# lisvulaczo/lodestar

Measured on AMD Instinct MI355X. Metric: BLS signature sets verified/sec (whole node) at 1/2/4/8 MI355X; p50 batch latency, higher is better.
Workload: dtype u32

## Files before the change

### include/lodestar_bls.h

```cpp
#ifndef LODESTAR_BLS_H
#define LODESTAR_BLS_H

#include <stddef.h>
#include <stdint.h>

#ifdef __cplusplus
extern "C" {
#endif

#define LSG_OK 0
#define LSG_ERR_INVALID_ARG 1
#define LSG_ERR_NO_DEVICE 2
#define LSG_ERR_DEVICE 3
#define LSG_ERR_NOMEM 4
#define LSG_ERR_CLOSED 5
#define LSG_ERR_BUSY 6
#define LSG_ERR_ENTROPY 7

#define LSG_BLST_SUCCESS 0
#define LSG_BLST_BAD_ENCODING 1
#define LSG_BLST_POINT_NOT_ON_CURVE 2
#define LSG_BLST_POINT_NOT_IN_GROUP 3
#define LSG_BLST_AGGR_TYPE_MISMATCH 4
#define LSG_BLST_VERIFY_FAIL 5
// ... 67 lines not shown
int lsg_submit_jobs(lsg_ctx* ctx, const lsg_job* jobs, size_t n_jobs, uint64_t seed, lsg_ticket* ticket);
int lsg_wait_jobs(lsg_ctx* ctx, lsg_ticket ticket, lsg_job_result* results , lsg_stats* stats);
int lsg_jobs_partial(lsg_ctx* ctx, lsg_ticket ticket, uint8_t* out576, int32_t* has_batch);
int lsg_jobs_partial_device(lsg_ctx* ctx, lsg_ticket ticket, void* dev_out576, int32_t* has_batch);
int lsg_wait_jobs_node(lsg_ctx* ctx, lsg_ticket ticket, int32_t node_valid, lsg_job_result* results,
                       lsg_stats* stats);
#define LSG_NO_GROUP 0xffffffffu
int lsg_submit_jobs_grouped(lsg_ctx* ctx, const lsg_job* jobs, size_t n_jobs, uint64_t seed,
                            const uint32_t* set_group, size_t n_groups, lsg_ticket* ticket);
int lsg_wait_jobs_grouped(lsg_ctx* ctx, lsg_ticket ticket, lsg_job_result* results, lsg_stats* stats,
                          uint8_t* agg96 , uint32_t* agg_n );
int lsg_set_coalesce(lsg_ctx* ctx, uint32_t max_sets, int32_t max_inflight);
int lsg_assign_jobs(const uint32_t* job_sets, size_t n_jobs, int32_t n_devices, int32_t* owner);
int lsg_pipeline_slots(lsg_ctx* ctx, int32_t* n);
int lsg_poll(lsg_ctx* ctx, lsg_ticket ticket, int32_t* done);
int lsg_verify_jobs(lsg_ctx* ctx, const lsg_job* jobs, size_t n_jobs, uint64_t seed, lsg_job_result* results,
                    lsg_stats* stats);

int lsg_verify_sets(lsg_ctx* ctx, const lsg_set* sets, size_t n_sets, uint64_t seed, lsg_job_result* result);

int lsg_aggregate_pubkeys(lsg_ctx* ctx, const uint8_t* pks, uint32_t pk_len, size_t n, uint8_t* out96,
                          int32_t* err_code);
int lsg_aggregate_pubkeys_multi(lsg_ctx* ctx, const lsg_set* sets, size_t n_sets, uint8_t* out96, int32_t* err);

int lsg_hash_to_g2(lsg_ctx* ctx, const uint8_t* msgs, uint32_t msg_len, size_t n, const uint8_t* dst,
                   uint32_t dst_len, uint8_t* out192);

int lsg_sig_decode(lsg_ctx* ctx, const uint8_t* sigs, uint32_t sig_len, size_t n, uint8_t* out192, int32_t* err);

int lsg_batch_partial(lsg_ctx* ctx, const lsg_set* sets, size_t n_sets, uint64_t seed, uint8_t* out576,
                      int32_t* set_err, int32_t* any_error);
int lsg_final_verify(lsg_ctx* ctx, const uint8_t* partials576, size_t n_partials, int32_t* valid);
int lsg_final_submit(lsg_ctx* ctx, const uint8_t* partials576, size_t n_partials, lsg_ticket* ticket);
int lsg_final_submit_device(lsg_ctx* ctx, const void* dev_partials576, size_t n_partials, lsg_ticket* ticket);
int lsg_final_wait(lsg_ctx* ctx, lsg_ticket ticket, int32_t* valid);
int lsg_final_submit_groups(lsg_ctx* ctx, const uint8_t* partials576, size_t n_groups, size_t per_group,
                            lsg_ticket* ticket);
int lsg_final_wait_groups(lsg_ctx* ctx, lsg_ticket ticket, int32_t* valid );

int lsg_pubkey_table_set(lsg_ctx* ctx, size_t first_index, const uint8_t* pks, uint32_t pk_len, size_t n,
                         int32_t* err);
int lsg_pubkey_table_size(lsg_ctx* ctx, size_t* n);

int lsg_committees_set(lsg_ctx* ctx, uint32_t first_id, const uint32_t* indices,
                       const uint32_t* offsets , size_t n_committees,
                       int32_t* err );
int lsg_committees_clear(lsg_ctx* ctx, uint32_t first_id, size_t n);
int lsg_committee_count(lsg_ctx* ctx, size_t* n);

typedef struct {
  uint64_t lookups, hits, pending, inserts, evictions, bypassed, full;
  uint32_t entries, capacity;
} lsg_msg_cache_stats;
int lsg_msg_cache_set(lsg_ctx* ctx, size_t capacity);
int lsg_msg_cache_clear(lsg_ctx* ctx);
int lsg_msg_cache_get_stats(lsg_ctx* ctx, lsg_msg_cache_stats* out);

int lsg_pubkey_validate(lsg_ctx* ctx, const uint8_t* pks, uint32_t pk_len, size_t n, uint8_t* out96, int32_t* err);

int lsg_aggregate_signatures(lsg_ctx* ctx, const uint8_t* sigs, uint32_t sig_len, const uint32_t* offsets,
                             size_t n_groups, uint8_t* out96, int32_t* err);

int lsg_signing_roots(lsg_ctx* ctx, const uint8_t* roots32, size_t n, const uint8_t* domain32, uint32_t domain_stride,
                      uint8_t* out32);
int lsg_attestation_signing_roots(lsg_ctx* ctx, const uint8_t* data128, size_t n, const uint8_t* domain32,
                                  uint32_t domain_stride, uint8_t* out32);
int lsg_deposit_signing_roots(lsg_ctx* ctx, const uint8_t* msgs88, size_t n, const uint8_t* domain32,
                              uint32_t domain_stride, uint8_t* out32);
int lsg_object_signing_roots(lsg_ctx* ctx, const uint8_t* objs, uint32_t obj_len, size_t n, const uint8_t* domain32,
                             uint32_t domain_stride, uint8_t* out32);

int lsg_verify_deposits(lsg_ctx* ctx, const uint8_t* data184, size_t n, const uint8_t* domain32, uint64_t seed,
                        uint8_t* valid, int32_t* err);

int lsg_sign(lsg_ctx* ctx, const uint8_t* sks32, const uint8_t* msgs, uint32_t msg_len, size_t n, uint8_t* out96);
int lsg_sk_to_pk(lsg_ctx* ctx, const uint8_t* sks32, size_t n, uint8_t* out96);

int lsg_check_fp2_mul(lsg_ctx* ctx, const uint32_t* in, size_t n, uint32_t* out);
int lsg_check_fp_sqr(lsg_ctx* ctx, const uint32_t* in, size_t n, uint32_t* out);
int lsg_check_fp2_sqr(lsg_ctx* ctx, const uint32_t* in, size_t n, uint32_t* out);
int lsg_check_sums(lsg_ctx* ctx, const uint32_t* in, size_t n, uint32_t* out);
int lsg_check_fp2_lanes(lsg_ctx* ctx, const uint32_t* in, size_t n, uint32_t* out);
int lsg_check_g2_lanes(lsg_ctx* ctx, const uint32_t* in, size_t n, uint32_t* out);
int lsg_check_canon(lsg_ctx* ctx, const uint32_t* in, size_t n, const uint8_t* bytes48, size_t nb, uint32_t* out,
                    uint32_t* out_limbs);
int lsg_check_fp2_roots(lsg_ctx* ctx, const uint32_t* in, size_t n, uint32_t* out);
int lsg_check_batch_inv(lsg_ctx* ctx, const uint32_t* in, size_t n, uint32_t* out);
int lsg_check_map_uniform(lsg_ctx* ctx, const uint8_t* ub256, size_t n, uint8_t* out192);
int lsg_check_batch_partial_rnd(lsg_ctx* ctx, const lsg_set* sets, size_t n_sets,
                                const uint64_t* rnd , uint8_t* out576,
                                int32_t* set_err, int32_t* any_error);

int lsg_probe_fp_mul_rate(lsg_ctx* ctx, double* fp_mul_per_s, double* mad_per_s);

int lsg_probe_mad_peak(lsg_ctx* ctx, double* mad_per_s);

int lsg_last_kernel_times(lsg_ctx* ctx, const char** names, double* ms, int max);

#ifdef __cplusplus
}
#endif
#endif
```

### lodestar_amd/_native.py

```python
import ctypes
import os
import struct
import threading

HERE = os.path.dirname(os.path.abspath(__file__))
LIB_PATH = os.environ.get("LSG_LIB", os.path.join(HERE, "liblodestar_bls.so"))
AB_LIB_PATH = os.path.join(HERE, "liblodestar_bls_ab.so")

LSG_OK = 0
LSG_ERR_INVALID_ARG = 1
LSG_ERR_NO_DEVICE = 2
LSG_ERR_BUSY = 6
LSG_ERR_ENTROPY = 7

LSG_INVALID = 0
LSG_VALID = 1
LSG_ERROR = 2

LSG_JOB_BATCHABLE = 1
LSG_JOB_PRIORITY = 2
LSG_JOB_VALIDATE_KEYS = 4

BLST_NAMES = {
    0: "BLST_SUCCESS", 1: "BLST_BAD_ENCODING", 2: "BLST_POINT_NOT_ON_CURVE", 3: "BLST_POINT_NOT_IN_GROUP",
# ... 66 lines not shown
        k = len(self.committees)
        return struct.pack("=I%dI" % k, k, *self.committees) + self.bits


def _key_form(pks):
    if isinstance(pks, PkBits):
        return LSG_PK_BITS, pks.n_bits, pks.tobytes()
    if isinstance(pks, PkBitsMulti):
        return LSG_PK_BITS_MULTI, pks.n_bits, pks.tobytes()
    if isinstance(pks, PkIndices):
        return LSG_PK_INDEX, len(pks), pks.tobytes()
    pk_len = len(pks[0]) if pks else 96
    if any(len(p) != pk_len for p in pks):
        raise ValueError("all pubkeys of one set must share one encoding length")
    if pk_len in (LSG_PK_BITS, LSG_PK_BITS_MULTI):
        pk_len = 0
    return pk_len, len(pks), b"".join(pks)


class MsgObject:

    def __init__(self, obj, domain):
        self.obj = bytes(obj)
        self.domain = bytes(domain)

    def __len__(self):
        return len(self.obj) + len(self.domain)

    def tobytes(self):
        return self.obj + self.domain


def _msg_form(msg):
    if isinstance(msg, MsgObject):
        b = msg.tobytes()
        return b, len(b) | LSG_MSG_OBJECT
    return msg, len(msg)


class LsgSet(ctypes.Structure):
    _fields_ = [
        ("pks", ctypes.c_void_p), ("pk_len", ctypes.c_uint32), ("n_pks", ctypes.c_uint32),
        ("msg", ctypes.c_void_p), ("msg_len", ctypes.c_uint32),
        ("sig", ctypes.c_void_p), ("sig_len", ctypes.c_uint32),
    ]


class LsgJob(ctypes.Structure):
    _fields_ = [("sets", ctypes.POINTER(LsgSet)), ("n_sets", ctypes.c_uint32), ("flags", ctypes.c_uint32)]


class LsgJobResult(ctypes.Structure):
    _fields_ = [("status", ctypes.c_int32), ("err_code", ctypes.c_int32)]


class LsgStats(ctypes.Structure):
    _fields_ = [
        ("batch_retries", ctypes.c_uint32), ("batch_sigs_success", ctypes.c_uint32),
        ("start_ns", ctypes.c_uint64), ("end_ns", ctypes.c_uint64),
        ("n_final_exps", ctypes.c_uint32), ("submit_us", ctypes.c_uint32),
        ("key_error", ctypes.c_int32), ("key_error_job", ctypes.c_uint32),
    ]


class LsgMsgCacheStats(ctypes.Structure):
    _fields_ = [(k, ctypes.c_uint64) for k in ("lookups", "hits", "pending", "inserts", "evictions", "bypassed",
                                                "full")] + [("entries", ctypes.c_uint32), ("capacity", ctypes.c_uint32)]


_lib = None
_lib_lock = threading.Lock()

EXPORTS = [
    "lsg_init", "lsg_init_devices", "lsg_destroy", "lsg_device_count", "lsg_last_error", "lsg_device_name",
    "lsg_reserve", "lsg_allocation_count", "lsg_verify_jobs", "lsg_verify_sets",
    "lsg_aggregate_pubkeys", "lsg_hash_to_g2", "lsg_sig_decode", "lsg_batch_partial", "lsg_final_verify",
    "lsg_probe_fp_mul_rate", "lsg_last_kernel_times", "lsg_sign", "lsg_sk_to_pk",
    "lsg_submit_jobs", "lsg_wait_jobs", "lsg_wait_jobs_node", "lsg_jobs_partial", "lsg_assign_jobs", "lsg_poll",
    "lsg_final_submit", "lsg_final_wait", "lsg_pipeline_slots", "lsg_probe_mad_peak",
    "lsg_pubkey_table_set", "lsg_pubkey_table_size", "lsg_pubkey_validate",
    "lsg_final_submit_groups", "lsg_final_wait_groups", "lsg_aggregate_signatures",
    "lsg_signing_roots", "lsg_attestation_signing_roots", "lsg_jobs_partial_device", "lsg_final_submit_device",
    "lsg_set_coalesce", "lsg_aggregate_pubkeys_multi", "lsg_check_fp2_mul",
    "lsg_check_fp_sqr", "lsg_check_fp2_sqr", "lsg_check_sums", "lsg_check_fp2_lanes", "lsg_check_g2_lanes",
    "lsg_check_canon", "lsg_check_fp2_roots", "lsg_check_batch_inv", "lsg_check_map_uniform",
    "lsg_check_batch_partial_rnd",
    "lsg_deposit_signing_roots", "lsg_verify_deposits",
    "lsg_committees_set", "lsg_committees_clear", "lsg_committee_count",
    "lsg_object_signing_roots",
    "lsg_submit_jobs_grouped", "lsg_wait_jobs_grouped",
    "lsg_msg_cache_set", "lsg_msg_cache_clear", "lsg_msg_cache_get_stats",
]


def load_library(path=LIB_PATH):
    global _lib
    with _lib_lock:
        if _lib is not None and path == LIB_PATH:
            return _lib
        if not os.path.exists(path):
            raise NativeUnavailable(f"{path} not built (run python -c 'import __graft_entry__; __graft_entry__.build()')")
        lib = ctypes.CDLL(path)
        vp, u32, u64, i32, sz = ctypes.c_void_p, ctypes.c_uint32, ctypes.c_uint64, ctypes.c_int32, ctypes.c_size_t
        pi32 = ctypes.POINTER(ctypes.c_int32)
        lib.lsg_init.argtypes = [ctypes.c_int, ctypes.POINTER(vp)]
        lib.lsg_init_devices.argtypes = [ctypes.POINTER(ctypes.c_int), ctypes.c_int, ctypes.POINTER(vp)]
        lib.lsg_device_count.argtypes = [vp, pi32]
        lib.lsg_reserve.argtypes = [vp, sz, sz, sz, i32]
        lib.lsg_allocation_count.argtypes = [vp, ctypes.POINTER(u64)]
        lib.lsg_wait_jobs_node.argtypes = [vp, u64, i32, ctypes.POINTER(LsgJobResult), ctypes.POINTER(LsgStats)]
        lib.lsg_jobs_partial.argtypes = [vp, u64, ctypes.c_char_p, pi32]
        lib.lsg_jobs_partial_device.argtypes = [vp, u64, vp, pi32]
        lib.lsg_final_submit_device.argtypes = [vp, vp, sz, ctypes.POINTER(u64)]
        lib.lsg_assign_jobs.argtypes = [ctypes.POINTER(u32), sz, i32, pi32]
        lib.lsg_destroy.argtypes = [vp]
        lib.lsg_last_error.argtypes = [vp]
        lib.lsg_last_error.restype = ctypes.c_char_p
        lib.lsg_device_name.argtypes = [vp, ctypes.c_char_p, sz]
        lib.lsg_verify_jobs.argtypes = [vp, ctypes.POINTER(LsgJob), sz, u64, ctypes.POINTER(LsgJobResult),
                                        ctypes.POINTER(LsgStats)]
        lib.lsg_verify_sets.argtypes = [vp, ctypes.POINTER(LsgSet), sz, u64, ctypes.POINTER(LsgJobResult)]
        lib.lsg_aggregate_pubkeys.argtypes = [vp, ctypes.c_char_p, u32, sz, ctypes.c_char_p, pi32]
        lib.lsg_aggregate_pubkeys_multi.argtypes = [vp, ctypes.POINTER(LsgSet), sz, ctypes.c_char_p, pi32]
        lib.lsg_hash_to_g2.argtypes = [vp, ctypes.c_char_p, u32, sz, ctypes.c_char_p, u32, ctypes.c_char_p]
        lib.lsg_sig_decode.argtypes = [vp, ctypes.c_char_p, u32, sz, ctypes.c_char_p, pi32]
        lib.lsg_batch_partial.argtypes = [vp, ctypes.POINTER(LsgSet), sz, u64, ctypes.c_char_p, pi32, pi32]
        lib.lsg_final_verify.argtypes = [vp, ctypes.c_char_p, sz, pi32]
        lib.lsg_probe_fp_mul_rate.argtypes = [vp, ctypes.POINTER(ctypes.c_double), ctypes.POINTER(ctypes.c_double)]
        lib.lsg_last_kernel_times.argtypes = [vp, ctypes.POINTER(ctypes.c_char_p), ctypes.POINTER(ctypes.c_double),
                                              ctypes.c_int]
        lib.lsg_sign.argtypes = [vp, ctypes.c_char_p, ctypes.c_char_p, u32, sz, ctypes.c_char_p]
        lib.lsg_sk_to_pk.argtypes = [vp, ctypes.c_char_p, sz, ctypes.c_char_p]
        pu64 = ctypes.POINTER(u64)
        lib.lsg_submit_jobs.argtypes = [vp, ctypes.POINTER(LsgJob), sz, u64, pu64]
        lib.lsg_wait_jobs.argtypes = [vp, u64, ctypes.POINTER(LsgJobResult), ctypes.POINTER(LsgStats)]
        lib.lsg_submit_jobs_grouped.argtypes = [vp, ctypes.POINTER(LsgJob), sz, u64, ctypes.POINTER(u32), sz, pu64]
        lib.lsg_wait_jobs_grouped.argtypes = [vp, u64, ctypes.POINTER(LsgJobResult), ctypes.POINTER(LsgStats),
                                              ctypes.c_char_p, ctypes.POINTER(u32)]
        lib.lsg_poll.argtypes = [vp, u64, pi32]
        lib.lsg_pubkey_table_set.argtypes = [vp, sz, ctypes.c_char_p, u32, sz, pi32]
        lib.lsg_pubkey_table_size.argtypes = [vp, ctypes.POINTER(sz)]
        lib.lsg_committees_set.argtypes = [vp, u32, ctypes.POINTER(u32), ctypes.POINTER(u32), sz, pi32]
        lib.lsg_committees_clear.argtypes = [vp, u32, sz]
        lib.lsg_committee_count.argtypes = [vp, ctypes.POINTER(sz)]
        lib.lsg_msg_cache_set.argtypes = [vp, sz]
        lib.lsg_msg_cache_clear.argtypes = [vp]
        lib.lsg_msg_cache_get_stats.argtypes = [vp, ctypes.POINTER(LsgMsgCacheStats)]
        lib.lsg_final_submit_groups.argtypes = [vp, ctypes.c_char_p, sz, sz, pu64]
        lib.lsg_final_wait_groups.argtypes = [vp, u64, pi32]
        lib.lsg_pubkey_validate.argtypes = [vp, ctypes.c_char_p, u32, sz, ctypes.c_char_p, pi32]
        lib.lsg_signing_roots.argtypes = [vp, ctypes.c_char_p, sz, ctypes.c_char_p, u32, ctypes.c_char_p]
        lib.lsg_attestation_signing_roots.argtypes = [vp, ctypes.c_char_p, sz, ctypes.c_char_p, u32, ctypes.c_char_p]
        lib.lsg_deposit_signing_roots.argtypes = [vp, ctypes.c_char_p, sz, ctypes.c_char_p, u32, ctypes.c_char_p]
        lib.lsg_object_signing_roots.argtypes = [vp, ctypes.c_char_p, u32, sz, ctypes.c_char_p, u32, ctypes.c_char_p]
        lib.lsg_verify_deposits.argtypes = [vp, ctypes.c_char_p, sz, ctypes.c_char_p, u64, ctypes.c_char_p, pi32]
        lib.lsg_aggregate_signatures.argtypes = [vp, ctypes.c_char_p, u32, ctypes.POINTER(u32), sz,
                                                 ctypes.c_char_p, pi32]
        lib.lsg_final_submit.argtypes = [vp, ctypes.c_char_p, sz, pu64]
        lib.lsg_final_wait.argtypes = [vp, u64, pi32]
        lib.lsg_pipeline_slots.argtypes = [vp, pi32]
        lib.lsg_set_coalesce.argtypes = [vp, u32, i32]
        lib.lsg_check_fp2_mul.argtypes = [vp, ctypes.c_char_p, sz, ctypes.c_char_p]
        lib.lsg_check_fp_sqr.argtypes = [vp, ctypes.c_char_p, sz, ctypes.c_char_p]
        lib.lsg_check_fp2_sqr.argtypes = [vp, ctypes.c_char_p, sz, ctypes.c_char_p]
        lib.lsg_check_sums.argtypes = [vp, ctypes.c_char_p, sz, ctypes.c_char_p]
        lib.lsg_check_fp2_lanes.argtypes = [vp, ctypes.c_char_p, sz, ctypes.c_char_p]
        lib.lsg_check_g2_lanes.argtypes = [vp, ctypes.c_char_p, sz, ctypes.c_char_p]
        lib.lsg_check_canon.argtypes = [vp, ctypes.c_char_p, sz, ctypes.c_char_p, sz, ctypes.c_char_p, ctypes.c_char_p]
        lib.lsg_check_fp2_roots.argtypes = [vp, ctypes.c_char_p, sz, ctypes.c_char_p]
        lib.lsg_check_batch_inv.argtypes = [vp, ctypes.c_char_p, sz, ctypes.c_char_p]
        lib.lsg_check_map_uniform.argtypes = [vp, ctypes.c_char_p, sz, ctypes.c_char_p]
        lib.lsg_check_batch_partial_rnd.argtypes = [vp, ctypes.POINTER(LsgSet), sz, ctypes.POINTER(u64),
                                                    ctypes.c_char_p, pi32, pi32]
        lib.lsg_probe_mad_peak.argtypes = [vp, ctypes.POINTER(ctypes.c_double)]
        for name in EXPORTS:
            if name != "lsg_last_error":
                getattr(lib, name).restype = ctypes.c_int
        if path == LIB_PATH:
            _lib = lib
        return lib


class SetBuffer:

    def __init__(self, sets):
        self._keep = []
        sets = list(sets)
        self.arr = (LsgSet * max(len(sets), 1))()
        for i, (pks, msg, sig) in enumerate(sets):
            pk_len, n_pks, pkb = _key_form(pks)
            msg, msg_len = _msg_form(msg)
            for b in (pkb, msg, sig):
                self._keep.append(b)
            s = self.arr[i]
            s.pks = ctypes.cast(ctypes.c_char_p(pkb), ctypes.c_void_p) if pkb else None
            s.pk_len = pk_len
            s.n_pks = n_pks
            s.msg = ctypes.cast(ctypes.c_char_p(msg), ctypes.c_void_p) if msg else None
            s.msg_len = msg_len
            s.sig = ctypes.cast(ctypes.c_char_p(sig), ctypes.c_void_p) if sig else None
            s.sig_len = len(sig)
        self.n = len(sets)


def assign_jobs(job_sizes, n_devices):
    lib = load_library()
    n = len(job_sizes)
    sizes = (ctypes.c_uint32 * max(n, 1))(*job_sizes)
    owner = (ctypes.c_int32 * max(n, 1))()
    rc = lib.lsg_assign_jobs(sizes, n, int(n_devices), owner)
    if rc != LSG_OK:
        raise ValueError(f"lsg_assign_jobs failed ({rc})")
    return list(owner[:n])


class PreparedJobs:

    def __init__(self, jobs):
        import numpy as np
        flat = [st for sets, _ in jobs for st in sets]
        n = len(flat)
        pk_parts, pk_len, n_pks = [], np.zeros(max(n, 1), np.uint32), np.zeros(max(n, 1), np.uint32)
        for i, (pks, _m, _s) in enumerate(flat):
            pk_len[i], n_pks[i], b = _key_form(pks)
            pk_parts.append(b)

        def pack(parts):
            lens = np.array([len(p) for p in parts] or [0], np.uint64)
            offs = np.zeros_like(lens)
            if len(parts) > 1:
                offs[1:] = np.cumsum(lens)[:-1]
            buf = np.frombuffer(b"".join(parts) + b"\0", dtype=np.uint8).copy()
            return buf, offs, lens

        self._pk, pk_off, _ = pack(pk_parts)
        forms = [_msg_form(m) for _, m, _ in flat]
        self._msg, msg_off, msg_len = pack([b for b, _ in forms])
        msg_word = np.array([w for _, w in forms] or [0], np.uint32)
        self._sig, sig_off, sig_len = pack([s for _, _, s in flat])
        self.sets = (LsgSet * max(n, 1))()
        dt = np.dtype({"names": ["pks", "pk_len", "n_pks", "msg", "msg_len", "sig", "sig_len"],
                       "formats": [np.uint64, np.uint32, np.uint32, np.uint64, np.uint32, np.uint64, np.uint32],
                       "offsets": [LsgSet.pks.offset, LsgSet.pk_len.offset, LsgSet.n_pks.offset, LsgSet.msg.offset,
                                   LsgSet.msg_len.offset, LsgSet.sig.offset, LsgSet.sig_len.offset],
                       "itemsize": ctypes.sizeof(LsgSet)})
        v = np.frombuffer(self.sets, dtype=dt)
        if n:
            has_keys = (n_pks[:n] > 0) | (pk_len[:n] == LSG_PK_BITS_MULTI)
            v["pks"][:n] = np.where(has_keys, self._pk.ctypes.data + pk_off[:n], 0)
            v["pk_len"][:n] = pk_len[:n]
# ... 384 lines not shown

    def final_submit_groups(self, groups):
        ng = len(groups)
        pg = len(groups[0]) if groups else 0
        if any(len(g) != pg for g in groups):
            raise ValueError("every group needs the same number of partials")
        t = ctypes.c_uint64()
        rc = self.lib.lsg_final_submit_groups(self.h, b"".join(b"".join(g) for g in groups), ng, pg, ctypes.byref(t))
        if rc == LSG_ERR_BUSY:
            return None
        self._check(rc, "lsg_final_submit_groups")
        t_ng = ng
        return (t.value, t_ng)

    def final_wait_groups(self, ticket):
        t, ng = ticket
        v = (ctypes.c_int32 * max(ng, 1))()
        self._check(self.lib.lsg_final_wait_groups(self.h, t, v), "lsg_final_wait_groups")
        return [bool(x) for x in v[:ng]]

    def sign(self, sks, msgs):
        if not sks:
            return []
        ml = len(msgs[0])
        out = ctypes.create_string_buffer(96 * len(sks))
        skb = b"".join(int(k).to_bytes(32, "big") for k in sks)
        self._check(self.lib.lsg_sign(self.h, skb, b"".join(msgs), ml, len(sks), out), "lsg_sign")
        raw = out.raw
        return [raw[96 * i:96 * i + 96] for i in range(len(sks))]

    def sk_to_pk(self, sks):
        if not sks:
            return []
        out = ctypes.create_string_buffer(96 * len(sks))
        skb = b"".join(int(k).to_bytes(32, "big") for k in sks)
        self._check(self.lib.lsg_sk_to_pk(self.h, skb, len(sks), out), "lsg_sk_to_pk")
        raw = out.raw
        return [raw[96 * i:96 * i + 96] for i in range(len(sks))]

    def check_fp2_mul(self, words):
        n = len(words) // 56
        assert len(words) == 56 * n
        out = ctypes.create_string_buffer(4 * 28 * n)
        src = struct.pack(f"<{len(words)}I", *words)
        self._check(self.lib.lsg_check_fp2_mul(self.h, src, n, out), "lsg_check_fp2_mul")
        return list(struct.unpack(f"<{28 * n}I", out.raw))

    def _check_sqr(self, fn, words, per_item):
        n = len(words) // per_item
        assert len(words) == per_item * n
        out = ctypes.create_string_buffer(4 * per_item * n)
        src = struct.pack(f"<{len(words)}I", *words)
        self._check(getattr(self.lib, fn)(self.h, src, n, out), fn)
        return list(struct.unpack(f"<{per_item * n}I", out.raw))

    def check_fp_sqr(self, words):
        return self._check_sqr("lsg_check_fp_sqr", words, 14)

    def check_fp2_sqr(self, words):
        return self._check_sqr("lsg_check_fp2_sqr", words, 28)

    def check_sums(self, words):
        n = len(words) // (12 * 14)
        assert len(words) == 12 * 14 * n
        out = ctypes.create_string_buffer(4 * 42 * 14 * n)
        src = struct.pack(f"<{len(words)}I", *words)
        self._check(self.lib.lsg_check_sums(self.h, src, n, out), "lsg_check_sums")
        return list(struct.unpack(f"<{42 * 14 * n}I", out.raw))

    def _check_lanes(self, fn, words):
        n = len(words) // (12 * 14)
        assert len(words) == 12 * 14 * n
        out = ctypes.create_string_buffer(4 * 24 * 14 * n)
        src = struct.pack(f"<{len(words)}I", *words)
        self._check(getattr(self.lib, fn)(self.h, src, n, out), fn)
        return list(struct.unpack(f"<{24 * 14 * n}I", out.raw))

    def check_fp2_lanes(self, words):
        return self._check_lanes("lsg_check_fp2_lanes", words)

    def check_g2_lanes(self, words):
        return self._check_lanes("lsg_check_g2_lanes", words)

    def check_canon(self, words, strings=()):
        n, nb = len(words) // 14, len(strings)
        assert len(words) == 14 * n and all(len(b) == 48 for b in strings)
        out = ctypes.create_string_buffer(4 * 54 * max(n, 1))
        limbs = ctypes.create_string_buffer(4 * 14 * max(nb, 1))
        src = struct.pack(f"<{len(words)}I", *words)
        self._check(self.lib.lsg_check_canon(self.h, src, n, b"".join(strings), nb, out, limbs), "lsg_check_canon")
        return (list(struct.unpack(f"<{54 * n}I", out.raw[:4 * 54 * n])),
                list(struct.unpack(f"<{14 * nb}I", limbs.raw[:4 * 14 * nb])))

    def check_fp2_roots(self, words):
        n = len(words) // 28
        assert len(words) == 28 * n
        out = ctypes.create_string_buffer(4 * 58 * n)
        src = struct.pack(f"<{len(words)}I", *words)
        self._check(self.lib.lsg_check_fp2_roots(self.h, src, n, out), "lsg_check_fp2_roots")
        return list(struct.unpack(f"<{58 * n}I", out.raw))

    def check_batch_inv(self, words):
        return self._check_sqr("lsg_check_batch_inv", words, 14)

    def check_map_uniform(self, items):
        n = len(items)
        assert all(len(b) == 256 for b in items)
        if not n:
            return []
        out = ctypes.create_string_buffer(192 * n)
        self._check(self.lib.lsg_check_map_uniform(self.h, b"".join(items), n, out), "lsg_check_map_uniform")
        raw = out.raw
        return [raw[192 * i:192 * i + 192] for i in range(n)]

    def batch_partial_rnd(self, sets, rnd):
        b = SetBuffer(sets)
        assert len(rnd) == b.n
        r = (ctypes.c_uint64 * max(b.n, 1))(*[int(x) for x in rnd])
        out = ctypes.create_string_buffer(576)
        errs = (ctypes.c_int32 * max(b.n, 1))()
        anyerr = ctypes.c_int32()
        self._check(self.lib.lsg_check_batch_partial_rnd(self.h, b.arr, b.n, r, out, errs, ctypes.byref(anyerr)),
                    "lsg_check_batch_partial_rnd")
        return out.raw, [errs[i] for i in range(b.n)], bool(anyerr.value)

    def probe_fp_mul_rate(self):
        a, b = ctypes.c_double(), ctypes.c_double()
        self._check(self.lib.lsg_probe_fp_mul_rate(self.h, ctypes.byref(a), ctypes.byref(b)), "lsg_probe_fp_mul_rate")
        return a.value, b.value

    def last_kernel_times(self, max_entries=1024):
        names = (ctypes.c_char_p * max_entries)()
        ms = (ctypes.c_double * max_entries)()
        n = self.lib.lsg_last_kernel_times(self.h, names, ms, max_entries)
        return [(names[i].decode(), ms[i]) for i in range(n)]
```

### lodestar_amd/csrc/lsg_curve.hpp

```cpp
#pragma once
#include "lsg_tower.hpp"

LSG_INL fp_t fadd(const fp_t& a, const fp_t& b) { return fp_add(a, b); }
LSG_INL fp2_t fadd(const fp2_t& a, const fp2_t& b) { return fp2_add(a, b); }
LSG_INL fp_t fsub(const fp_t& a, const fp_t& b) { return fp_sub(a, b); }
LSG_INL fp2_t fsub(const fp2_t& a, const fp2_t& b) { return fp2_sub(a, b); }
LSG_INL fp_t fmul(const fp_t& a, const fp_t& b) { return fp_mul(a, b); }
LSG_INL fp2_t fmul(const fp2_t& a, const fp2_t& b) { return fp2_mul(a, b); }
LSG_INL fp_t fsqr(const fp_t& a) { return fp_sqr(a); }
LSG_INL fp2_t fsqr(const fp2_t& a) { return fp2_sqr(a); }
LSG_INL fp_t fneg(const fp_t& a) { return fp_neg(a); }
LSG_INL fp2_t fneg(const fp2_t& a) { return fp2_neg(a); }
LSG_INL fps_t<1, 0> fsum(const fp_t& a) { return fps(a); }
LSG_INL fp2s_t<1, 0> fsum(const fp2_t& a) { return fp2s(a); }
template <int K, int P, int N>
LSG_INL fps_t<K * P, K * N> fsum_mulk(const fps_t<P, N>& a) { return fps_mulk<K>(a); }
template <int K, int P0, int N0, int P1, int N1>
LSG_INL fp2s_t<K * P0, K * N0, K * P1, K * N1> fsum_mulk(const fp2s_t<P0, N0, P1, N1>& a) { return fp2s_mulk<K>(a); }
template <int K> LSG_INL fp_t fmulk(const fp_t& a) { return fp_mulk<K>(a); }
template <int K> LSG_INL fp2_t fmulk(const fp2_t& a) { return fp2_mulk<K>(a); }
template <class F> LSG_INL F fsub2(const F& a, const F& b, const F& c) { return (fsum(a) - b - c).carry(); }
LSG_INL fp_t fmul_b3(const fp_t& a) { return fp_mul12(a); }
LSG_INL fp2_t fmul_b3(const fp2_t& a) { return fp2_mul_b3(a); }
LSG_INL bool fis_zero(const fp_t& a) { return fp_is_zero(a); }
LSG_INL bool fis_zero(const fp2_t& a) { return fp2_is_zero(a); }
LSG_INL bool feq(const fp_t& a, const fp_t& b) { return fp_eq(a, b); }
LSG_INL bool feq(const fp2_t& a, const fp2_t& b) { return fp2_eq(a, b); }
LSG_INL fp_t fselect(bool c, const fp_t& a, const fp_t& b) { return fp_select(c, a, b); }
LSG_INL fp2_t fselect(bool c, const fp2_t& a, const fp2_t& b) { return fp2_select(c, a, b); }
LSG_INL fp_t finv(const fp_t& a) { return fp_inv(a); }
LSG_INL fp2_t finv(const fp2_t& a) { return fp2_inv(a); }
template <class F> LSG_INL F fzero();
template <> LSG_INL fp_t fzero<fp_t>() { return fp_zero(); }
template <> LSG_INL fp2_t fzero<fp2_t>() { return fp2_zero(); }
template <class F> LSG_INL F fone();
template <> LSG_INL fp_t fone<fp_t>() { return FP_ONE; }
template <> LSG_INL fp2_t fone<fp2_t>() { return fp2_one(); }
#ifdef LSG_PAIR_MODE
#include "lsg_fp2_lanes.hpp"
#endif
#ifdef LSG_FP2_LANES
template <> LSG_INL fp2v_t fzero<fp2v_t>() { return fp2v_from_const(fpc_t{}, fpc_t{}); }
template <> LSG_INL fp2v_t fone<fp2v_t>() { return fp2v_from_const(FP_ONE, fpc_t{}); }
#endif

template <class F>
struct aff_t {
  F x, y;
};
template <class F>
struct proj_t {
  F X, Y, Z;
};
typedef aff_t<fp_t> g1a_t;
typedef aff_t<fp2_t> g2a_t;
typedef proj_t<fp_t> g1p_t;
typedef proj_t<fp2_t> g2p_t;

template <class F>
LSG_INL proj_t<F> proj_inf() {
  proj_t<F> r;
  r.X = fzero<F>();
  r.Y = fone<F>();
  r.Z = fzero<F>();
  return r;
}

template <class F>
LSG_INL proj_t<F> proj_from_aff(const aff_t<F>& a) {
  proj_t<F> r;
  r.X = a.x;
  r.Y = a.y;
  r.Z = fone<F>();
  return r;
}

template <class F>
LSG_INL bool proj_is_inf(const proj_t<F>& a) {
  return fis_zero(a.Z);
}

template <class F>
LSG_INL proj_t<F> proj_neg(const proj_t<F>& a) {
  proj_t<F> r = a;
  r.Y = fneg(a.Y);
  return r;
}

template <class F>
LSG_INL proj_t<F> proj_add(const proj_t<F>& p, const proj_t<F>& q) {
  F t0 = fmul(p.X, q.X);
  F t1 = fmul(p.Y, q.Y);
  F t2 = fmul(p.Z, q.Z);
  F t3 = fsub2(fmul(fadd(p.X, p.Y), fadd(q.X, q.Y)), t0, t1);
  F t4 = fsub2(fmul(fadd(p.Y, p.Z), fadd(q.Y, q.Z)), t1, t2);
  F Y3 = fsub2(fmul(fadd(p.X, p.Z), fadd(q.X, q.Z)), t0, t2);
  F X3;
  t0 = fmulk<3>(t0);
  t2 = fmul_b3(t2);
  F Z3 = fadd(t1, t2);
  t1 = fsub(t1, t2);
  Y3 = fmul_b3(Y3);
  X3 = fmul(t4, Y3);
  t2 = fmul(t3, t1);
  X3 = fsub(t2, X3);
  Y3 = fmul(Y3, t0);
// ... 535 lines not shown
```

### lodestar_amd/csrc/lsg_fp2_lanes.hpp

```cpp
#pragma once

constexpr int LSG_VL = 14;

#if LSG_PAIR_G == 2
#define LSG_LANES_HIDE(x) asm volatile("" : "+v"(x))
#else
#define LSG_LANES_HIDE(x) ((void)0)
#endif

LSG_PFN void lanes_carry64(int64_t* t) {
#pragma unroll
  for (int j = 0; j < LSG_VL - 1; j++) {
    t[j + 1] += t[j] >> 29;
    t[j] &= (int64_t)LSG_M29;
  }
}
LSG_PFN void lanes_reduce_step(int64_t* t, const uint32_t* p, int i) {
  uint32_t m = ((uint32_t)t[0] * LSG_N0P) & LSG_M29;
  LSG_LANES_HIDE(m);
#pragma unroll
  for (int j = 0; j < LSG_VL; j++) t[j] += (int64_t)(int32_t)m * (int32_t)p[j];
  const int64_t c = t[0] >> 29;
#pragma unroll
  for (int j = 0; j < LSG_VL - 1; j++) t[j] = t[j + 1];
  t[0] += c;
  t[LSG_VL - 1] = 0;
  if (i == 6) lanes_carry64(t);
}
LSG_PFN void lanes_tail(int64_t* t, uint32_t* r) {
  lanes_carry64(t);
#pragma unroll
  for (int j = 0; j < LSG_VL; j++) r[j] = (uint32_t)t[j];
}
template <class OTHER>
LSG_PFN void lanes_sop_pass(uint32_t* r, const uint32_t* P, const uint32_t* Q, const uint32_t* b, const OTHER& other) {
  uint32_t p[LSG_VL];
#pragma unroll
  for (int j = 0; j < LSG_VL; j++) p[j] = LSG_P[j];
  int64_t t[LSG_VL];
#pragma unroll
  for (int j = 0; j < LSG_VL; j++) t[j] = 0;
#pragma unroll
  for (int i = 0; i < LSG_VL; i++) {
    uint32_t bo = b[i], bs = other(i, b[i]);
    LSG_LANES_HIDE(bo);
    LSG_LANES_HIDE(bs);
#pragma unroll
    for (int j = 0; j < LSG_VL; j++) t[j] += (int64_t)(int32_t)P[j] * (int32_t)bo;
#pragma unroll
    for (int j = 0; j < LSG_VL; j++) t[j] += (int64_t)(int32_t)Q[j] * (int32_t)bs;
    lanes_reduce_step(t, p, i);
  }
  lanes_tail(t, r);
}
LSG_PFN void lanes_mul_pass(uint32_t* r, const uint32_t* V, const uint32_t* s) {
  uint32_t p[LSG_VL];
#pragma unroll
  for (int j = 0; j < LSG_VL; j++) p[j] = LSG_P[j];
  int64_t t[LSG_VL];
#pragma unroll
  for (int j = 0; j < LSG_VL; j++) t[j] = 0;
#pragma unroll
  for (int i = 0; i < LSG_VL; i++) {
    uint32_t si = s[i];
    LSG_LANES_HIDE(si);
#pragma unroll
    for (int j = 0; j < LSG_VL; j++) t[j] += (int64_t)(int32_t)V[j] * (int32_t)si;
    lanes_reduce_step(t, p, i);
  }
  lanes_tail(t, r);
}
LSG_PFN void lanes_mul_operand(uint32_t& P, uint32_t& Q, uint32_t own, uint32_t partner, bool odd) {
  P = odd ? partner : own;
  Q = odd ? own : 0u - partner;
}
LSG_PFN void lanes_sqr_operand(uint32_t& V, uint32_t& s, uint32_t own, uint32_t partner, bool odd) {
  V = odd ? own : own + partner;
  s = odd ? partner + partner : own - partner;
}

#if LSG_PAIR_G == 2 && !defined(LSG_NO_FP2_LANES)
#define LSG_FP2_LANES 1
struct fp2v_t {
  uint32_t l[LSG_VL];
};
LSG_PFN bool lanes_odd() { return pair_h() != 0u; }
LSG_PFN uint32_t lanes_swap(uint32_t x) {
  return (uint32_t)__builtin_amdgcn_update_dpp(0, (int)x, 0xB1, 0xf, 0xf, true);
}

typedef uint32_t lanes8_t __attribute__((ext_vector_type(8)));
typedef uint32_t lanes4_t __attribute__((ext_vector_type(4)));
typedef uint32_t lanes2_t __attribute__((ext_vector_type(2)));
#define LSG_LANES_PARAMS(x) lanes8_t x##_a, lanes4_t x##_b, lanes2_t x##_c
#define LSG_LANES_ARGS(v) lanes_pack8(v), lanes_pack4(v), lanes_pack2(v)
#define LSG_LANES_UNPACK(x) lanes_unpack(x##_a, x##_b, x##_c)
LSG_PFN lanes8_t lanes_pack8(const fp2v_t& a) {
  return lanes8_t{a.l[0], a.l[1], a.l[2], a.l[3], a.l[4], a.l[5], a.l[6], a.l[7]};
}
LSG_PFN lanes4_t lanes_pack4(const fp2v_t& a) { return lanes4_t{a.l[8], a.l[9], a.l[10], a.l[11]}; }
LSG_PFN lanes2_t lanes_pack2(const fp2v_t& a) { return lanes2_t{a.l[12], a.l[13]}; }
LSG_PFN fp2v_t lanes_unpack(const lanes8_t& a, const lanes4_t& b, const lanes2_t& c) {
  fp2v_t r;
#pragma unroll
  for (int k = 0; k < 8; k++) r.l[k] = a[k];
#pragma unroll
  for (int k = 0; k < 4; k++) r.l[8 + k] = b[k];
  r.l[12] = c[0];
  r.l[13] = c[1];
  return r;
}

LSG_PLEAF fp2v_t lanes_fp2_mul_v(LSG_LANES_PARAMS(va), LSG_LANES_PARAMS(vb)) {
  const fp2v_t a = LSG_LANES_UNPACK(va), b = LSG_LANES_UNPACK(vb);
  const bool odd = lanes_odd();
  uint32_t P[LSG_VL], Q[LSG_VL];
#pragma unroll
  for (int k = 0; k < LSG_VL; k++) {
    lanes_mul_operand(P[k], Q[k], a.l[k], lanes_swap(a.l[k]), odd);
    LSG_LANES_HIDE(P[k]);
    LSG_LANES_HIDE(Q[k]);
  }
  fp2v_t r;
  lanes_sop_pass(r.l, P, Q, b.l, [](int, uint32_t x) { return lanes_swap(x); });
  return r;
}
LSG_PLEAF fp2v_t lanes_fp2_sqr_v(LSG_LANES_PARAMS(va)) {
  const fp2v_t a = LSG_LANES_UNPACK(va);
  const bool odd = lanes_odd();
  uint32_t V[LSG_VL], s[LSG_VL];
#pragma unroll
  for (int k = 0; k < LSG_VL; k++) {
    lanes_sqr_operand(V[k], s[k], a.l[k], lanes_swap(a.l[k]), odd);
    LSG_LANES_HIDE(V[k]);
    LSG_LANES_HIDE(s[k]);
  }
  fp2v_t r;
  lanes_mul_pass(r.l, V, s);
  return r;
}

LSG_PFN fp2v_t fp2v_from_pair(const fp2_t& a) {
  const bool odd = lanes_odd();
  fp2v_t r;
#pragma unroll
  for (int k = 0; k < LSG_PL; k++) {
    const uint32_t s = lanes_swap(odd ? a.c0.l[k] : a.c1.l[k]);
    r.l[k] = odd ? s : a.c0.l[k];
    r.l[LSG_PL + k] = odd ? a.c1.l[k] : s;
  }
  return r;
}
LSG_PFN fp2_t fp2v_to_pair(const fp2v_t& a) {
  const bool odd = lanes_odd();
  fp2_t r;
#pragma unroll
  for (int k = 0; k < LSG_PL; k++) {
    const uint32_t s = lanes_swap(odd ? a.l[k] : a.l[LSG_PL + k]);
    r.c0.l[k] = odd ? s : a.l[k];
    r.c1.l[k] = odd ? a.l[LSG_PL + k] : s;
  }
  return r;
}
LSG_PFN fp2v_t fp2v_from_const(const fpc_t& c0, const fpc_t& c1) {
  const bool odd = lanes_odd();
  fp2v_t r;
#pragma unroll
  for (int k = 0; k < LSG_VL; k++) r.l[k] = odd ? c1.l[k] : c0.l[k];
  return r;
}

LSG_PFN fp2v_t lanes_carry(const fp2v_t& a) {
  fp2v_t o;
  o.l[0] = a.l[0] & LSG_M29;
#pragma unroll
  for (int k = 1; k < LSG_VL - 1; k++) o.l[k] = (a.l[k] & LSG_M29) + (uint32_t)((int32_t)a.l[k - 1] >> 29);
  o.l[LSG_VL - 1] = a.l[LSG_VL - 1] + (uint32_t)((int32_t)a.l[LSG_VL - 2] >> 29);
  return o;
}
template <int P, int N>
struct fp2vs_t {
  uint32_t l[LSG_VL];
  LSG_PFN fp2v_t carry() const {
    static_assert(fps_carry_ok(P, N), "lazy sum too long for one carry round: carry a group first (P <= 3, N <= 3)");
    fp2v_t a;
#pragma unroll
    for (int k = 0; k < LSG_VL; k++) a.l[k] = l[k];
    return lanes_carry(a);
  }
  template <int K>
  LSG_PFN fp2v_t carry_mul() const {
    static_assert(fps_carry_mul_ok(K, P, N), "small multiple of this sum does not come out carried: carry() first");
    constexpr int m = fps_mulk_m(K), s = fps_mulk_s(K), sh = 29 - s;
    constexpr uint32_t lowm = (1u << sh) - 1;
    uint32_t t[LSG_VL];
#pragma unroll
    for (int k = 0; k < LSG_VL; k++) t[k] = m == 3 ? l[k] + (l[k] << 1) : l[k];
    fp2v_t o;
    o.l[0] = (t[0] & lowm) << s;
#pragma unroll
    for (int k = 1; k < LSG_VL - 1; k++) o.l[k] = ((t[k] & lowm) << s) + (uint32_t)((int32_t)t[k - 1] >> sh);
    o.l[LSG_VL - 1] = (t[LSG_VL - 1] << s) + (uint32_t)((int32_t)t[LSG_VL - 2] >> sh);
    return o;
  }
};
LSG_PFN fp2vs_t<1, 0> fsum(const fp2v_t& a) {
  fp2vs_t<1, 0> r;
#pragma unroll
  for (int k = 0; k < LSG_VL; k++) r.l[k] = a.l[k];
  return r;
}
template <int P, int N, int Q, int M>
LSG_PFN fp2vs_t<P + Q, N + M> operator+(const fp2vs_t<P, N>& a, const fp2vs_t<Q, M>& b) {
  fp2vs_t<P + Q, N + M> r;
#pragma unroll
  for (int k = 0; k < LSG_VL; k++) r.l[k] = a.l[k] + b.l[k];
  return r;
}
template <int P, int N, int Q, int M>
LSG_PFN fp2vs_t<P + M, N + Q> operator-(const fp2vs_t<P, N>& a, const fp2vs_t<Q, M>& b) {
  fp2vs_t<P + M, N + Q> r;
#pragma unroll
  for (int k = 0; k < LSG_VL; k++) r.l[k] = a.l[k] - b.l[k];
  return r;
}
template <int P, int N>
LSG_PFN fp2vs_t<N, P> operator-(const fp2vs_t<P, N>& a) {
  fp2vs_t<N, P> r;
#pragma unroll
  for (int k = 0; k < LSG_VL; k++) r.l[k] = 0u - a.l[k];
  return r;
}
template <int P, int N>
LSG_PFN fp2vs_t<P + 1, N> operator+(const fp2vs_t<P, N>& a, const fp2v_t& b) { return a + fsum(b); }
template <int P, int N>
LSG_PFN fp2vs_t<P, N + 1> operator-(const fp2vs_t<P, N>& a, const fp2v_t& b) { return a - fsum(b); }
template <int K, int P, int N>
LSG_PFN fp2vs_t<K * P, K * N> fsum_mulk(const fp2vs_t<P, N>& a) {
  static_assert(K >= 1 && K <= 3, "uncarried small multiples up to 3");
  fp2vs_t<K * P, K * N> r;
#pragma unroll
  for (int k = 0; k < LSG_VL; k++) r.l[k] = a.l[k] * (uint32_t)K;
  return r;
}

LSG_PFN fp2v_t fmul(const fp2v_t& a, const fp2v_t& b) { return lanes_fp2_mul_v(LSG_LANES_ARGS(a), LSG_LANES_ARGS(b)); }
LSG_PFN fp2v_t fsqr(const fp2v_t& a) { return lanes_fp2_sqr_v(LSG_LANES_ARGS(a)); }
LSG_PFN fp2v_t fadd(const fp2v_t& a, const fp2v_t& b) { return (fsum(a) + b).carry(); }
LSG_PFN fp2v_t fsub(const fp2v_t& a, const fp2v_t& b) { return (fsum(a) - b).carry(); }
LSG_PFN fp2v_t fneg(const fp2v_t& a) { return (-fsum(a)).carry(); }
template <int K>
LSG_PFN fp2v_t fmulk(const fp2v_t& a) { return fsum(a).template carry_mul<K>(); }
LSG_PFN fp2v_t fmul_b3(const fp2v_t& a) {
  const bool odd = lanes_odd();
  fp2vs_t<2, 1> x;
#pragma unroll
  for (int k = 0; k < LSG_VL; k++) {
    const uint32_t o = lanes_swap(a.l[k]);
    x.l[k] = odd ? a.l[k] + o : a.l[k] - o;
  }
  return fmulk<12>(x.carry());
}
LSG_PFN fp2v_t fselect(bool c, const fp2v_t& a, const fp2v_t& b) {
  fp2v_t r;
#pragma unroll
  for (int k = 0; k < LSG_VL; k++) r.l[k] = c ? a.l[k] : b.l[k];
  return r;
}
LSG_PFN bool fis_zero(const fp2v_t& a) { return fp2_is_zero(fp2v_to_pair(a)); }
#endif
```

### lodestar_amd/csrc/lsg_host.hip

```cpp
#include <hip/hip_runtime.h>
#include <rccl/rccl.h>
#include <stdio.h>
#include <stdlib.h>
#include <errno.h>
#include <string.h>
#include <sys/random.h>
#include <time.h>

#include <algorithm>
#include <atomic>
#include <condition_variable>
#include <chrono>
#include <mutex>
#include <shared_mutex>
#include <thread>
#include <unordered_map>
#include <string>
#include <vector>

#include "../../include/lodestar_bls.h"
#include "lsg_launch.h"
#include "lsg_layout.h"
#include "lsg_serial.h"
#include "lsg_ab.h"
// ... 403 lines not shown
    s->own_streams = false;
  } else {
    for (int k = 0; k < 2; k++) LSG_HIP(s, hipStreamCreateWithFlags(&s->st_norm[k], hipStreamNonBlocking));
    s->st[0] = s->st_norm[0];
    s->st[1] = s->st_norm[1];
  }
  hipEvent_t* evs[] = {&s->ev_in, &s->ev_sig, &s->ev_grp, &s->ev_part, &s->ev_done, &s->ev_node, &s->ev_xp};
  for (hipEvent_t* e : evs) LSG_HIP(s, hipEventCreateWithFlags(e, hipEventDisableTiming));
  if (blocking_waits()) {
    for (hipEvent_t* e : {&s->ev_part, &s->ev_done}) {
      LSG_HIP(s, hipEventDestroy(*e));
      LSG_HIP(s, hipEventCreateWithFlags(e, hipEventDisableTiming | hipEventBlockingSync));
    }
  }
  LSG_RC(ensure(s, s->d_dst, 256));
  LSG_HIP(s, hipMemcpy(s->d_dst.p, DST_POP, DST_POP_LEN, hipMemcpyHostToDevice));
  return LSG_OK;
}

void slot_destroy(Slot* s) {
  if (!s->d) return;
  for (int k = 0; k < 2; k++)
    if (s->st[k]) (void)hipStreamSynchronize(s->st[k]);
  DevBuf* bufs[] = {&s->d_sig,  &s->d_siglen, &s->d_msg,  &s->d_msgoff, &s->d_msglen, &s->d_pk,    &s->d_pklen,
                    &s->d_rnd,  &s->d_mode,   &s->d_dst,  &s->d_ub,     &s->d_sigaff, &s->d_siginf, &s->d_seterr,
                    &s->d_pkp,  &s->d_pkerr,  &s->d_agg,  &s->d_P,      &s->d_pinf,   &s->d_H,     &s->d_hinf,
                    &s->d_rs,   &s->d_rs2,    &s->d_fall, &s->d_fall2,  &s->d_Pp,     &s->d_zP,    &s->d_zPi,
                    &s->d_U,    &s->d_nrm,    &s->d_nrmi, &s->d_Hp,     &s->d_zN,     &s->d_zNi,   &s->binv_lv[0],
                    &s->binv_lv[1], &s->binv_iv[0], &s->binv_iv[1], &s->d_lines, &s->d_S, &s->d_F, &s->d_verdict,
                    &s->d_Sb,   &s->d_fgb,    &s->d_Fb,   &s->d_bkt,    &s->d_bits,   &s->d_aux,   &s->d_gath,
                    &s->d_nodeF, &s->d_nodeV, &s->d_plan, &s->d_mid, &s->d_Hm, &s->d_hinfm,
                    &s->d_mmask, &s->d_PmP, &s->d_Pm, &s->d_pinfm, &s->d_errm, &s->d_xport,
                    &s->d_agga, &s->d_aggi, &s->d_aggpre, &s->d_aggtot, &s->d_aggflag, &s->d_cbits,
                    &s->d_gplan, &s->d_gsum, &s->d_gagg, &s->d_gtmp[0], &s->d_gtmp[1], &s->d_Hx, &s->d_hinfx};
  for (DevBuf* b : bufs) free_dev(*b);
  for (auto& u : s->seg_tmp)
    for (DevBuf& b : u) free_dev(b);
  HostBuf* hb[] = {&s->h_arena, &s->h_err, &s->h_pinf, &s->h_pkerr, &s->h_verdict, &s->h_blob, &s->h_plan, &s->h_nodeV,
                   &s->h_xport, &s->h_cbits, &s->h_gplan, &s->h_gagg};
  for (HostBuf* b : hb) free_host(*b);
  for (Timer& t : s->timers) {
    (void)hipEventDestroy(t.a);
    (void)hipEventDestroy(t.b);
  }
  s->timers.clear();
  hipEvent_t evs[] = {s->ev_in, s->ev_sig, s->ev_grp, s->ev_part, s->ev_done, s->ev_node, s->ev_xp};
  for (hipEvent_t e : evs)
    if (e) (void)hipEventDestroy(e);
  if (s->own_streams) {
    for (int k = 0; k < 2; k++) {
      if (s->st_prio[k]) (void)hipStreamSynchronize(s->st_prio[k]);
      if (s->st_norm[k]) (void)hipStreamSynchronize(s->st_norm[k]);
    }
    for (int k = 0; k < 2; k++) {
      if (s->st_norm[k]) (void)hipStreamDestroy(s->st_norm[k]);
      s->st_norm[k] = s->st_prio[k] = s->st[k] = nullptr;
    }
  }
  s->d = nullptr;
}

int slot_streams(Slot* s, bool prio) {
  if (!s->own_streams) return LSG_OK;
  if (prio && !s->st_prio[0]) {
    Dev* d = s->d;
    for (int k = 0; k < 2; k++) LSG_RC(prio_stream(d->c, d, &d->s_pp[k]));
    s->st_prio[0] = d->s_pp[0];
    s->st_prio[1] = d->s_pp[1];
  }
  hipStream_t* p = prio ? s->st_prio : s->st_norm;
  s->st[0] = p[0];
  s->st[1] = p[1];
  return LSG_OK;
}

int slot_ready(Dev* d, Slot* s, int index) {
  if (s->d) return LSG_OK;
  const int rc = slot_create(d, s, index, nullptr);
  if (rc) slot_destroy(s);
  return rc;
}

bool miller_fused() { return lsg_ab_long("LSG_MILLER_FUSED", 1) != 0; }

size_t slp_items_max();
int miller_k_for(size_t n_sets) {
  if (miller_fused()) return n_sets <= slp_items_max() ? 1 : 4;
  const long v = lsg_ab_long("LSG_MILLER_K", 0);
  if (v == 1 || v == 2 || v == 4) return (int)v;
  return n_sets >= 8192 ? 4 : (n_sets >= 1024 ? 2 : 1);
}

bool agg_tree_on() { return lsg_ab_long("LSG_AGG_TREE", 0) != 0; }

Switches read_switches() {
  Switches w;
  w.package_group = lsg_ab_long("LSG_PACKAGE_GROUP", 1) != 0;
  w.sub_groups = lsg_ab_long("LSG_SUB_GROUPS", 1) != 0;
  w.nb_merge = lsg_ab_long("LSG_NB_MERGE", 1) != 0;
  w.msg_agg = lsg_ab_long("LSG_MSG_AGG", 1) != 0;
  w.msm_min_group = (size_t)std::max(1L, lsg_ab_long("LSG_MSM_MIN_GROUP", 256));
  w.b0_min = (size_t)std::max(0L, lsg_ab_long("LSG_B0_MIN", 64));
  w.b0_run = (size_t)std::max(2L, lsg_ab_long("LSG_B0_RUN", 4));
  w.seg_fold_wide = (int)lsg_ab_long("LSG_SEG_FOLD_WIDE", SEG_FOLD_WIDE);
  w.slp_items = slp_items_max();
  return w;
}
SegPlan slot_seg(Slot* s, int op, const std::vector<int32_t>& seg_off, const std::vector<int32_t>& seg_len, bool has_idx,
                 size_t idx_off, int32_t dst_base) {
  return plan_seg(s->plan, op, seg_off, seg_len, has_idx, idx_off, dst_base,
                  (int)lsg_ab_long("LSG_SEG_FOLD_WIDE", SEG_FOLD_WIDE));
}

void binv_sizes(size_t n, size_t* lv, size_t* iv);
size_t binv_lv_words(size_t n) {
  size_t a, b;
  binv_sizes(n, &a, &b);
  return a;
}
size_t binv_iv_words(size_t n) {
  size_t a, b;
  binv_sizes(n, &a, &b);
  return b;
}

int size_inputs(Slot* s, size_t n, size_t np, size_t mb) {
  const size_t nn = std::max(n, (size_t)1), pp = std::max(np, (size_t)1);
  auto al = [](size_t x) { return (x + 7) & ~(size_t)7; };
  const size_t arena = al(192 * nn) + al(4 * nn) * 4 + al(4 * pp) + al(8 * nn) + al(96 * pp) + al(std::max(mb, (size_t)1)) + nn;
  LSG_RC(ensure_host(s, s->h_arena, arena));
  LSG_RC(ensure(s, s->d_sig, 192 * nn));
  LSG_RC(ensure(s, s->d_siglen, 4 * nn));
  LSG_RC(ensure(s, s->d_msg, std::max(mb, (size_t)1)));
  LSG_RC(ensure(s, s->d_msgoff, 4 * nn));
  LSG_RC(ensure(s, s->d_msglen, 4 * nn));
  LSG_RC(ensure(s, s->d_pk, 96 * pp));
  LSG_RC(ensure(s, s->d_pklen, 4 * pp));
  LSG_RC(ensure(s, s->d_rnd, 8 * nn));
  LSG_RC(ensure(s, s->d_mode, nn));
  LSG_RC(ensure(s, s->d_mid, 4 * nn));
  return LSG_OK;
}

int size_state(Slot* s, size_t n, size_t np, size_t ng, size_t n_msm, int pkg = 0) {
  const size_t nn = std::max(n, (size_t)1), pp = std::max(np, (size_t)1), gg = std::max(ng, (size_t)1);
  const size_t g_msm = std::max(n_msm, (size_t)1);
  struct {
    DevBuf* b;
    size_t bytes;
  } dev[] = {{&s->d_ub, 256 * nn},
             {&s->d_sigaff, 4 * W_G2A * nn},
             {&s->d_siginf, nn},
             {&s->d_seterr, 4 * nn},
             {&s->d_pkp, 4 * W_G1P * pp},
             {&s->d_pkerr, 4 * pp},
             {&s->d_agg, 4 * W_G1P * nn},
             {&s->d_P, 4 * W_G1A * nn},
             {&s->d_pinf, nn},
             {&s->d_H, 4 * W_G2A * nn},
             {&s->d_hinf, nn},
             {&s->d_rs, 4 * W_G2P * nn},
             {&s->d_Pp, 4 * W_G1P * nn},
             {&s->d_zP, 4 * W_FP * nn},
             {&s->d_zPi, 4 * W_FP * nn},
             {&s->d_U, 4 * W_H2CU * nn},
             {&s->d_nrm, 4 * W_FP * 2 * nn},
// ... 475 lines not shown
  if (s->msg_dedup) s->msg_id.assign(mid, mid + n);
  if (scale && n) {
    if (rnd_in) {
      memcpy(rnd, rnd_in, 8 * n);
    } else if (seed == 0) {
      if (!os_random(rnd, 8 * n)) {
        set_err(s->d->c, "no entropy for the RLC randomizers (getrandom failed)");
        return LSG_ERR_ENTROPY;
      }
      for (size_t i = 0; i < n; i++)
        while (rnd[i] == 0)
          if (!os_random(&rnd[i], 8)) {
            set_err(s->d->c, "no entropy for the RLC randomizers (getrandom failed)");
            return LSG_ERR_ENTROPY;
          }
    } else {
      uint64_t sd = seed;
      for (size_t i = 0; i < n; i++) {
        uint64_t r;
        do r = splitmix64(sd);
        while (r == 0);
        rnd[i] = r;
      }
    }
  } else if (n) {
    memset(rnd, 0, 8 * n);
  }
  if (scale && noscale)
    for (size_t i = 0; i < n; i++)
      if ((*noscale)[i]) rnd[i] = 0;
  memcpy(s->rnd.data(), rnd, 8 * n);
  hipStream_t S = s->st[0];
  struct {
    DevBuf* d;
    size_t off, len;
  } cp[] = {{&s->d_sig, o_sig, 192 * nn},      {&s->d_siglen, o_siglen, 4 * nn}, {&s->d_msg, o_msg, std::max(mc ? mo : msg_total, (size_t)1)},
            {&s->d_msgoff, o_msgoff, 4 * nn}, {&s->d_msglen, o_msglen, 4 * nn}, {&s->d_pk, o_pk, ks * np},
            {&s->d_pklen, o_pklen, 4 * np},   {&s->d_rnd, o_rnd, 8 * nn}};
  for (auto& x : cp) LSG_HIP(s, hipMemcpyAsync(x.d->p, A + x.off, x.len, hipMemcpyHostToDevice, S));
  if (s->msg_dedup) LSG_HIP(s, hipMemcpyAsync(s->d_mid.p, A + o_mid, 4 * n, hipMemcpyHostToDevice, S));
  if (bw) LSG_HIP(s, hipMemcpyAsync(s->d_cbits.p, cbits, 4 * bw, hipMemcpyHostToDevice, S));
  return LSG_OK;
}

int run_pk_bits(Slot* s, uint32_t* dst) {
  if (s->bits_sets.empty()) return LSG_OK;
  Dev* d = s->d;
  KL(s, "k_pk_agg_bits", lsgk::pk_agg_bits(S_(s), (int)s->bplan.n_pairs, PL(s, s->bplan.pair_off), PL(s, s->bplan.plan_off),
                                           P_<uint32_t>(s->d_cbits), P_<uint32_t>(d->d_cm_idx), P_<uint32_t>(d->d_cm_off),
                                           P_<uint32_t>(d->d_cm_sum), P_<uint32_t>(d->d_pktab), P_<uint8_t>(d->d_pktab_ok),
                                           (uint32_t)d->pktab_n, dst));
  return LSG_OK;
}
int run_pk_multi(Slot* s, uint32_t* dst) {
  if (s->multi_sets.empty()) return LSG_OK;
  Dev* d = s->d;
  KL(s, "k_pk_agg_bits_multi",
     lsgk::pk_agg_bits_multi(S_(s), (int)s->mplan.n_pairs, PL(s, s->mplan.pair_off), PL(s, s->mplan.set_off),
                             PL(s, s->mplan.part_off), P_<uint32_t>(s->d_cbits), P_<uint32_t>(d->d_cm_idx),
                             P_<uint32_t>(d->d_cm_off), P_<uint32_t>(d->d_cm_sum), P_<uint32_t>(d->d_pktab),
                             P_<uint8_t>(d->d_pktab_ok), (uint32_t)d->pktab_n, dst));
  return LSG_OK;
}

int launch_accum(Slot* s, size_t n_items, size_t item_off, uint32_t* fall, bool single = false) {
  const int ni = (int)n_items;
  const int32_t* items = PL(s, item_off);
  if (ni > 0 && (single || s->K == 1) && miller_fused() && (size_t)ni <= std::max(slp_items_max(), (size_t)8192) &&
      slp_items_max() > 0) {
    KL(s, "k_slp_items1", lsg_slp_miller_items1(S_(s), ni, items, P_<uint32_t>(s->d_P), P_<uint8_t>(s->d_pinf),
                                                P_<uint8_t>(s->d_hinf), P_<int32_t>(s->d_seterr), P_<uint32_t>(s->d_H),
                                                fall));
    return LSG_OK;
  }
  if (single && ni > 0) {
    LSG_RC(ensure(s, s->d_lines, 4 * (size_t)ML_STEPS * W_LINE * n_items));
    KL(s, "k_miller_lines_list", lsgk::miller_lines_list(S_(s), ni, items, P_<uint32_t>(s->d_H), P_<uint32_t>(s->d_lines)));
    KL(s, "k_miller_accum_list",
       lsgk::miller_accum_list(S_(s), ni, items, P_<uint32_t>(s->d_P), P_<uint8_t>(s->d_pinf), P_<uint8_t>(s->d_hinf),
                               P_<int32_t>(s->d_seterr), P_<uint32_t>(s->d_lines), fall));
    return LSG_OK;
  }
  if (miller_fused()) {
    KL(s, "k_miller_fused", lsgk::miller_fused(S_(s), ni, items, items + ni, P_<uint32_t>(s->d_P), P_<uint8_t>(s->d_pinf),
                                              P_<uint8_t>(s->d_hinf), P_<int32_t>(s->d_seterr), P_<uint32_t>(s->d_H),
                                              fall));
    return LSG_OK;
  }
  KL(s, "k_miller_accum",
     lsgk::miller_accum(S_(s), s->K, ni, items, items + ni, P_<uint32_t>(s->d_P), P_<uint8_t>(s->d_pinf),
                        P_<uint8_t>(s->d_hinf), P_<int32_t>(s->d_seterr), (int)s->n_sets, P_<uint32_t>(s->d_lines),
                        fall));
  return LSG_OK;
}

#define SERIAL_LABEL(name) (lsg_serial_mode() == LSG_SERIAL_SLP ? "slp_" #name : "k_row_" #name)

int launch_phase(Slot* s, const PhasePlan& Ph, const uint32_t* rs, uint32_t* fall, bool export_blobs,
                 const uint32_t* rs_msm = nullptr) {
  if (!rs_msm) rs_msm = rs;
  const size_t ng = Ph.groups.size();
  if (ng == 0) return LSG_OK;
  LSG_RC(size_state(s, s->n_sets, s->n_pks, ng, Ph.n_msm, 2));
  s->cur = 1;
  if (Ph.n_msm) {
    LSG_RC(run_seg(s, 1, "msm_buckets", Ph.buckets, rs_msm, P_<uint32_t>(s->d_bkt)));
    LSG_RC(run_seg(s, 1, "msm_bits", Ph.bits, P_<uint32_t>(s->d_bkt), P_<uint32_t>(s->d_bits)));
    KL(s, "k_g2p_to_canon", lsgk::g2p_to_canon(S_(s), (int)(MSM_BITS * Ph.n_msm), P_<uint32_t>(s->d_bits),
                                               P_<uint8_t>(s->d_Sb)));
    KL(s, SERIAL_LABEL(horner_miller),
       lsg_row_horner_miller(S_(s), (int)Ph.n_msm, P_<uint8_t>(s->d_Sb), P_<uint8_t>(s->d_fgb)));
  }
  if (Ph.n_msm < ng) {
    const int nsm = (int)(ng - Ph.n_msm);
    LSG_RC(run_seg(s, 1, "sig_sums", Ph.sums, rs, P_<uint32_t>(s->d_S)));
    uint8_t* sb = P_<uint8_t>(s->d_Sb) + (size_t)288 * MSM_BITS * Ph.n_msm;
    KL(s, "k_g2p_to_canon", lsgk::g2p_to_canon(S_(s), nsm, P_<uint32_t>(s->d_S) + W_G2P * Ph.n_msm, sb));
    KL(s, SERIAL_LABEL(miller_neg_g1),
       lsg_row_miller_neg_g1(S_(s), nsm, sb, P_<uint8_t>(s->d_fgb) + 576 * Ph.n_msm));
  }
  KL(s, "k_blobs_to_fp12", lsgk::blobs_to_fp12(S_(s), (int)ng, P_<uint8_t>(s->d_fgb), fall + W_F12 * Ph.term_base));
  LSG_HIP(s, hipEventRecord(s->ev_grp, s->st[1]));
  s->cur = 0;
  LSG_HIP(s, hipStreamWaitEvent(s->st[0], s->ev_grp, 0));
  LSG_RC(run_seg(s, 2, "fp12_product", Ph.prod, fall, P_<uint32_t>(s->d_F)));
  KL(s, "k_fp12_to_canon", lsgk::fp12_to_canon(S_(s), (int)ng, P_<uint32_t>(s->d_F), P_<uint8_t>(s->d_Fb)));
  if (export_blobs) LSG_HIP(s, hipMemcpyAsync(s->h_blob.p, s->d_Fb.p, 576 * ng, hipMemcpyDeviceToHost, s->st[0]));
  LSG_HIP(s, hipEventRecord(s->ev_part, s->st[0]));
  return LSG_OK;
}

int launch_fe_range(Slot* s, size_t g0, size_t g1) {
  if (g1 <= g0) return LSG_OK;
  s->cur = 0;
  const size_t ng = g1 - g0;
  KL(s, SERIAL_LABEL(final_exp),
     lsg_row_final_exp(S_(s), (int)ng, P_<uint8_t>(s->d_Fb) + 576 * g0, P_<int32_t>(s->d_verdict) + g0));
  LSG_HIP(s, hipMemcpyAsync(H_<int32_t>(s->h_verdict) + g0, P_<int32_t>(s->d_verdict) + g0, 4 * ng,
                            hipMemcpyDeviceToHost, s->st[0]));
  return LSG_OK;
}
int launch_fe(Slot* s, size_t ng) { return launch_fe_range(s, 0, ng); }

int launch_agg_tree(Slot* s, const AggPlan& P, uint32_t* agg);

int launch_set_stages(Slot* s, const SegPlan* pkagg, const PhasePlan& Ph, uint32_t* fall) {
  const size_t n_items = Ph.agg_g >= 0 ? Ph.n_set_items : Ph.n_items, item_off = Ph.item_off;
  const int n = (int)s->n_sets, np = (int)s->n_pks;
  if (n == 0) return LSG_OK;
  Dev* d = s->d;
  LSG_HIP(s, hipEventRecord(s->ev_in, s->st[0]));
  s->cur = 1;
  LSG_HIP(s, hipStreamWaitEvent(s->st[1], s->ev_in, 0));
  if (!s->single_keys && s->agg.tree) {
    LSG_RC(launch_agg_tree(s, s->agg, P_<uint32_t>(s->d_agg)));
  } else if (s->single_keys) {
    if (np > 0)
      KL(s, "k_pk_decode", lsgk::pk_decode(S_(s), np, P_<uint8_t>(s->d_pk), s->pk_stride, P_<uint32_t>(s->d_pklen),
                                           P_<uint32_t>(s->d_agg), P_<int32_t>(s->d_pkerr), P_<uint32_t>(d->d_pktab),
                                           P_<uint8_t>(d->d_pktab_ok), (uint32_t)d->pktab_n));
  } else if (!s->pk_all_bits) {
    LSG_RC(run_pk_seg(s, *pkagg, P_<uint32_t>(s->d_agg)));
  }
  LSG_RC(run_pk_bits(s, P_<uint32_t>(s->d_agg)));
  LSG_RC(run_pk_multi(s, P_<uint32_t>(s->d_agg)));
  if (s->n_kv)
    KL(s, "k_pk_keyvalidate", lsgk::pk_keyvalidate(S_(s), (int)s->n_kv, PL(s, s->kv_off), P_<uint8_t>(s->d_pk),
                                                   P_<uint32_t>(s->d_pklen), P_<int32_t>(s->d_pkp)));
  KL(s, "k_pk_scale", lsgk::pk_scale(S_(s), n, P_<uint32_t>(s->d_agg), P_<uint64_t>(s->d_rnd), P_<uint32_t>(s->d_Pp),
// ... 2462 lines not shown
int lsg_sign(lsg_ctx* c, const uint8_t* sks32, const uint8_t* msgs, uint32_t msg_len, size_t n, uint8_t* out96) {
  if (!c || !out96 || (n && (!sks32 || !msgs)) || msg_marked(msg_len)) return LSG_ERR_INVALID_ARG;
  LSG_ENTER(c);
  Slot* s = &c->dev[0]->util;
  timer_reset(s);
  if (n == 0) return LSG_OK;
  LSG_RC(util_hash(s, msgs, msg_len, n, DST_POP, DST_POP_LEN));
  LSG_RC(ensure(s, s->d_aux, 96 * n));
  LSG_RC(ensure(s, s->d_Fb, 32 * n));
  LSG_HIP(s, hipMemcpyAsync(s->d_Fb.p, sks32, 32 * n, hipMemcpyHostToDevice, s->st[0]));
  KL(s, "k_sign", lsgk::sign(S_(s), (int)n, P_<uint8_t>(s->d_Fb), P_<uint32_t>(s->d_H), P_<uint8_t>(s->d_aux)));
  LSG_HIP(s, hipMemcpyAsync(out96, s->d_aux.p, 96 * n, hipMemcpyDeviceToHost, s->st[0]));
  LSG_HIP(s, hipStreamSynchronize(s->st[0]));
  return LSG_OK;
}

int lsg_sk_to_pk(lsg_ctx* c, const uint8_t* sks32, size_t n, uint8_t* out96) {
  if (!c || !out96 || (n && !sks32)) return LSG_ERR_INVALID_ARG;
  LSG_ENTER(c);
  Slot* s = &c->dev[0]->util;
  timer_reset(s);
  if (n == 0) return LSG_OK;
  LSG_RC(ensure(s, s->d_aux, 96 * n));
  LSG_RC(ensure(s, s->d_Fb, 32 * n));
  LSG_HIP(s, hipMemcpyAsync(s->d_Fb.p, sks32, 32 * n, hipMemcpyHostToDevice, s->st[0]));
  KL(s, "k_sk_to_pk", lsgk::sk_to_pk(S_(s), (int)n, P_<uint8_t>(s->d_Fb), P_<uint8_t>(s->d_aux)));
  LSG_HIP(s, hipMemcpyAsync(out96, s->d_aux.p, 96 * n, hipMemcpyDeviceToHost, s->st[0]));
  LSG_HIP(s, hipStreamSynchronize(s->st[0]));
  return LSG_OK;
}

int lsg_check_fp2_mul(lsg_ctx* c, const uint32_t* in, size_t n, uint32_t* out) {
  if (!c || (n && (!in || !out)) || n > 0x7fffffffull / (4 * W_FP)) return LSG_ERR_INVALID_ARG;
  LSG_ENTER(c);
  if (n == 0) return LSG_OK;
  Slot* s = &c->dev[0]->util;
  timer_reset(s);
  LSG_RC(ensure(s, s->d_aux, 4 * 4 * W_FP * n));
  LSG_RC(ensure(s, s->d_Fb, 4 * 2 * W_FP * n));
  LSG_HIP(s, hipMemcpyAsync(s->d_aux.p, in, 4 * 4 * W_FP * n, hipMemcpyHostToDevice, s->st[0]));
  KL(s, "k_check_fp2_mul", lsgk::check_fp2_mul(S_(s), (int)n, P_<uint32_t>(s->d_aux), P_<uint32_t>(s->d_Fb)));
  LSG_HIP(s, hipMemcpyAsync(out, s->d_Fb.p, 4 * 2 * W_FP * n, hipMemcpyDeviceToHost, s->st[0]));
  LSG_HIP(s, hipStreamSynchronize(s->st[0]));
  return LSG_OK;
}

static int check_sqr(lsg_ctx* c, const uint32_t* in, size_t n, uint32_t* out, int E) {
  if (!c || (n && (!in || !out)) || n > 0x7fffffffull / (4 * W_FP)) return LSG_ERR_INVALID_ARG;
  LSG_ENTER(c);
  if (n == 0) return LSG_OK;
  Slot* s = &c->dev[0]->util;
  timer_reset(s);
  const size_t bytes = 4 * (size_t)E * W_FP * n;
  LSG_RC(ensure(s, s->d_aux, bytes));
  LSG_RC(ensure(s, s->d_Fb, bytes));
  LSG_HIP(s, hipMemcpyAsync(s->d_aux.p, in, bytes, hipMemcpyHostToDevice, s->st[0]));
  if (E == 1)
    KL(s, "k_check_fp_sqr", lsgk::check_fp_sqr(S_(s), (int)n, P_<uint32_t>(s->d_aux), P_<uint32_t>(s->d_Fb)));
  else
    KL(s, "k_check_fp2_sqr", lsgk::check_fp2_sqr(S_(s), (int)n, P_<uint32_t>(s->d_aux), P_<uint32_t>(s->d_Fb)));
  LSG_HIP(s, hipMemcpyAsync(out, s->d_Fb.p, bytes, hipMemcpyDeviceToHost, s->st[0]));
  LSG_HIP(s, hipStreamSynchronize(s->st[0]));
  return LSG_OK;
}
int lsg_check_fp_sqr(lsg_ctx* c, const uint32_t* in, size_t n, uint32_t* out) { return check_sqr(c, in, n, out, 1); }
int lsg_check_fp2_sqr(lsg_ctx* c, const uint32_t* in, size_t n, uint32_t* out) { return check_sqr(c, in, n, out, 2); }

int lsg_check_sums(lsg_ctx* c, const uint32_t* in, size_t n, uint32_t* out) {
  constexpr size_t EIN = 12, EOUT = 42;
  if (!c || (n && (!in || !out)) || n > 0x7fffffffull / (4 * W_FP * EOUT)) return LSG_ERR_INVALID_ARG;
  LSG_ENTER(c);
  if (n == 0) return LSG_OK;
  Slot* s = &c->dev[0]->util;
  timer_reset(s);
  LSG_RC(ensure(s, s->d_aux, 4 * EIN * W_FP * n));
  LSG_RC(ensure(s, s->d_Fb, 4 * EOUT * W_FP * n));
  LSG_HIP(s, hipMemcpyAsync(s->d_aux.p, in, 4 * EIN * W_FP * n, hipMemcpyHostToDevice, s->st[0]));
  KL(s, "k_check_sums", lsgk::check_sums(S_(s), (int)n, P_<uint32_t>(s->d_aux), P_<uint32_t>(s->d_Fb)));
  LSG_HIP(s, hipMemcpyAsync(out, s->d_Fb.p, 4 * EOUT * W_FP * n, hipMemcpyDeviceToHost, s->st[0]));
  LSG_HIP(s, hipStreamSynchronize(s->st[0]));
  return LSG_OK;
}

static int check_lanes(lsg_ctx* c, const uint32_t* in, size_t n, uint32_t* out, bool g2) {
  const size_t EIN = g2 ? lsgk::CHECK_G2L_IN : lsgk::CHECK_LANES_IN, EOUT = g2 ? lsgk::CHECK_G2L_OUT : lsgk::CHECK_LANES_OUT;
  if (!c || (n && (!in || !out)) || n > 0x7fffffffull / (4 * W_FP * EOUT)) return LSG_ERR_INVALID_ARG;
  LSG_ENTER(c);
  if (n == 0) return LSG_OK;
  Slot* s = &c->dev[0]->util;
  timer_reset(s);
  LSG_RC(ensure(s, s->d_aux, 4 * EIN * W_FP * n));
  LSG_RC(ensure(s, s->d_Fb, 4 * EOUT * W_FP * n));
  LSG_HIP(s, hipMemcpyAsync(s->d_aux.p, in, 4 * EIN * W_FP * n, hipMemcpyHostToDevice, s->st[0]));
  if (g2)
    KL(s, "k_check_g2_lanes", lsgk::check_g2_lanes(S_(s), (int)n, P_<uint32_t>(s->d_aux), P_<uint32_t>(s->d_Fb)));
  else
    KL(s, "k_check_fp2_lanes", lsgk::check_fp2_lanes(S_(s), (int)n, P_<uint32_t>(s->d_aux), P_<uint32_t>(s->d_Fb)));
  LSG_HIP(s, hipMemcpyAsync(out, s->d_Fb.p, 4 * EOUT * W_FP * n, hipMemcpyDeviceToHost, s->st[0]));
  LSG_HIP(s, hipStreamSynchronize(s->st[0]));
  return LSG_OK;
}
int lsg_check_fp2_lanes(lsg_ctx* c, const uint32_t* in, size_t n, uint32_t* out) { return check_lanes(c, in, n, out, false); }
int lsg_check_g2_lanes(lsg_ctx* c, const uint32_t* in, size_t n, uint32_t* out) { return check_lanes(c, in, n, out, true); }

int lsg_check_canon(lsg_ctx* c, const uint32_t* in, size_t n, const uint8_t* bytes48, size_t nb, uint32_t* out,
                    uint32_t* out_limbs) {
  constexpr size_t WOUT = lsgk::CHECK_CANON_OUT;
  if (!c || (n && (!in || !out)) || (nb && (!bytes48 || !out_limbs)) || n > 0x7fffffffull / (4 * WOUT) ||
      nb > 0x7fffffffull / (4 * W_FP))
    return LSG_ERR_INVALID_ARG;
  LSG_ENTER(c);
  Slot* s = &c->dev[0]->util;
  timer_reset(s);
  if (n) {
    LSG_RC(ensure(s, s->d_aux, 4 * W_FP * n));
    LSG_RC(ensure(s, s->d_Fb, 4 * WOUT * n));
    LSG_HIP(s, hipMemcpyAsync(s->d_aux.p, in, 4 * W_FP * n, hipMemcpyHostToDevice, s->st[0]));
    KL(s, "k_check_canon", lsgk::check_canon(S_(s), (int)n, P_<uint32_t>(s->d_aux), P_<uint32_t>(s->d_Fb)));
    LSG_HIP(s, hipMemcpyAsync(out, s->d_Fb.p, 4 * WOUT * n, hipMemcpyDeviceToHost, s->st[0]));
    LSG_HIP(s, hipStreamSynchronize(s->st[0]));
  }
  if (nb) {
    LSG_RC(ensure(s, s->d_aux, 48 * nb));
    LSG_RC(ensure(s, s->d_Fb, 4 * W_FP * nb));
    LSG_HIP(s, hipMemcpyAsync(s->d_aux.p, bytes48, 48 * nb, hipMemcpyHostToDevice, s->st[0]));
    KL(s, "k_check_from_bytes", lsgk::check_from_bytes(S_(s), (int)nb, P_<uint8_t>(s->d_aux), P_<uint32_t>(s->d_Fb)));
    LSG_HIP(s, hipMemcpyAsync(out_limbs, s->d_Fb.p, 4 * W_FP * nb, hipMemcpyDeviceToHost, s->st[0]));
    LSG_HIP(s, hipStreamSynchronize(s->st[0]));
  }
  return LSG_OK;
}

int lsg_check_fp2_roots(lsg_ctx* c, const uint32_t* in, size_t n, uint32_t* out) {
  constexpr size_t WOUT = lsgk::CHECK_ROOTS_OUT;
  if (!c || (n && (!in || !out)) || n > 0x7fffffffull / (4 * WOUT)) return LSG_ERR_INVALID_ARG;
  LSG_ENTER(c);
  if (n == 0) return LSG_OK;
  Slot* s = &c->dev[0]->util;
  timer_reset(s);
  LSG_RC(ensure(s, s->d_aux, 4 * 2 * W_FP * n));
  LSG_RC(ensure(s, s->d_Fb, 4 * WOUT * n));
  LSG_HIP(s, hipMemcpyAsync(s->d_aux.p, in, 4 * 2 * W_FP * n, hipMemcpyHostToDevice, s->st[0]));
  KL(s, "k_check_fp2_roots", lsgk::check_fp2_roots(S_(s), (int)n, P_<uint32_t>(s->d_aux), P_<uint32_t>(s->d_Fb)));
  LSG_HIP(s, hipMemcpyAsync(out, s->d_Fb.p, 4 * WOUT * n, hipMemcpyDeviceToHost, s->st[0]));
  LSG_HIP(s, hipStreamSynchronize(s->st[0]));
  return LSG_OK;
}

int lsg_check_batch_inv(lsg_ctx* c, const uint32_t* in, size_t n, uint32_t* out) {
  if (!c || (n && (!in || !out)) || n > 0x7fffffffull / (4 * W_FP)) return LSG_ERR_INVALID_ARG;
  LSG_ENTER(c);
  if (n == 0) return LSG_OK;
  Slot* s = &c->dev[0]->util;
  timer_reset(s);
  LSG_RC(ensure(s, s->d_aux, 4 * W_FP * n));
  LSG_RC(ensure(s, s->d_Fb, 4 * W_FP * n));
  LSG_HIP(s, hipMemcpyAsync(s->d_aux.p, in, 4 * W_FP * n, hipMemcpyHostToDevice, s->st[0]));
  LSG_RC(batch_inv(s, 0, "binv_check", P_<uint32_t>(s->d_aux), n, P_<uint32_t>(s->d_Fb)));
  LSG_HIP(s, hipMemcpyAsync(out, s->d_Fb.p, 4 * W_FP * n, hipMemcpyDeviceToHost, s->st[0]));
  LSG_HIP(s, hipStreamSynchronize(s->st[0]));
  keep_times(s);
  return LSG_OK;
}

int lsg_check_map_uniform(lsg_ctx* c, const uint8_t* ub256, size_t n, uint8_t* out192) {
  if (!c || (n && (!ub256 || !out192)) || n > 0x7fffffffull / 256) return LSG_ERR_INVALID_ARG;
  LSG_ENTER(c);
  if (n == 0) return LSG_OK;
  Slot* s = &c->dev[0]->util;
  timer_reset(s);
  LSG_RC(size_state(s, n, 0, 1, 0));
  LSG_RC(ensure(s, s->d_aux, 192 * n));
  LSG_HIP(s, hipMemcpyAsync(s->d_ub.p, ub256, 256 * n, hipMemcpyHostToDevice, s->st[0]));
  const int nn = (int)n;
  LSG_RC(launch_hash(s, nn, P_<uint32_t>(s->d_H), P_<uint8_t>(s->d_hinf)));
  KL(s, "k_g2a_to_bytes",
     lsgk::g2a_to_bytes(S_(s), nn, P_<uint32_t>(s->d_H), P_<uint8_t>(s->d_hinf), P_<uint8_t>(s->d_aux)));
  LSG_HIP(s, hipMemcpyAsync(out192, s->d_aux.p, 192 * n, hipMemcpyDeviceToHost, s->st[0]));
  LSG_HIP(s, hipStreamSynchronize(s->st[0]));
  keep_times(s);
  return LSG_OK;
}

int lsg_probe_fp_mul_rate(lsg_ctx* c, double* fp_mul_per_s, double* mad_per_s) {
  if (!c || !fp_mul_per_s || !mad_per_s) return LSG_ERR_INVALID_ARG;
  LSG_ENTER(c);
// ... 74 lines not shown
```

### lodestar_amd/csrc/lsg_k_miller.hip

```cpp
#include "lsg_kcommon.hpp"

constexpr int W_LINE_LANE = (int)(sizeof(line_t) / 4);
LSG_DEVI void line_store(uint32_t* __restrict__ lines, size_t n, size_t i, int st, const line_t& L) {
  uint32_t w[W_LINE_LANE];
  __builtin_memcpy(w, &L, sizeof(line_t));
  uint32_t* p = lines + (((size_t)st * W_LINE_LANE) * n + i) * LSG_GROUP + (threadIdx.x % LSG_GROUP);
#pragma unroll
  for (int k = 0; k < W_LINE_LANE; k++) p[(size_t)k * n * LSG_GROUP] = w[k];
}
LSG_DEVI line_t line_load(const uint32_t* __restrict__ lines, size_t n, size_t i, int st) {
  uint32_t w[W_LINE_LANE];
  const uint32_t* p = lines + (((size_t)st * W_LINE_LANE) * n + i) * LSG_GROUP + (threadIdx.x % LSG_GROUP);
#pragma unroll
  for (int k = 0; k < W_LINE_LANE; k++) w[k] = p[(size_t)k * n * LSG_GROUP];
  line_t L;
  __builtin_memcpy(&L, w, sizeof(line_t));
  return L;
}

__global__ void LSG_KERNEL_ATTR k_miller_lines(int n, const uint32_t* __restrict__ H, uint32_t* __restrict__ lines) {
  LANE_ITEM(n);
  (void)lead;
  const g2a_t Q = lane_load<g2a_t>(H, item);
  miller_lines(Q, [&](int st, const line_t& L) { line_store(lines, (size_t)n, item, st, L); });
}

#ifndef LSG_ACCUM_WAVES
#define LSG_ACCUM_WAVES 1
#endif
template <int K>
__global__ void LSG_KERNEL_ATTR_W(LSG_ACCUM_WAVES)
    k_miller_accum(int n_items, const int32_t* __restrict__ item_first, const int32_t* __restrict__ item_cnt,
                   const uint32_t* __restrict__ P, const uint8_t* __restrict__ pinf, const uint8_t* __restrict__ hinf,
                   const int32_t* __restrict__ err, int n_sets, const uint32_t* __restrict__ lines,
                   uint32_t* __restrict__ f) {
  LANE_ITEM(n_items);
  (void)lead;
  const int first = item_first[item], cnt = item_cnt[item];
  g1a_t Pk[K];
  bool use[K];
  int idx[K];
#pragma unroll
  for (int k = 0; k < K; k++) {
    const int i = first + (k < cnt ? k : cnt - 1);
    idx[k] = i;
    use[k] = k < cnt && err[i] == 0 && !pinf[i] && !hinf[i];
    Pk[k] = lane_load<g1a_t>(P, i);
  }
  lane_store(f, item, miller_accum_multi<K>(Pk, use, [&](int k, int st) {
               return line_load(lines, (size_t)n_sets, (size_t)idx[k], st);
             }));
}

__global__ void LSG_KERNEL_ATTR k_miller_lines_list(int n, const int32_t* __restrict__ list, const uint32_t* __restrict__ H,
                                                    uint32_t* __restrict__ lines) {
  LANE_ITEM(n);
  (void)lead;
  const g2a_t Q = lane_load<g2a_t>(H, (size_t)list[item]);
  miller_lines(Q, [&](int st, const line_t& L) { line_store(lines, (size_t)n, item, st, L); });
}
__global__ void LSG_KERNEL_ATTR_W(LSG_ACCUM_WAVES)
    k_miller_accum_list(int n, const int32_t* __restrict__ list, const uint32_t* __restrict__ P,
                        const uint8_t* __restrict__ pinf, const uint8_t* __restrict__ hinf, const int32_t* __restrict__ err,
                        const uint32_t* __restrict__ lines, uint32_t* __restrict__ f) {
  LANE_ITEM(n);
  (void)lead;
  const int i = list[item];
  g1a_t Pk[1] = {lane_load<g1a_t>(P, (size_t)i)};
  bool use[1] = {err[i] == 0 && !pinf[i] && !hinf[i]};
  lane_store(f, item, miller_accum_multi<1>(Pk, use, [&](int, int st) { return line_load(lines, (size_t)n, item, st); }));
}

constexpr int MF_ITEMS = 32;
constexpr int MF_F = 0, MF_L = 12, MF_V = 36, MF_T = 66, MF_COMPS = 90;
constexpr size_t MF_LDS_BYTES = (size_t)MF_COMPS * 7 * 64 * 4;

LSG_DEVI uint32_t* mf_slot(uint32_t* lds, int c) { return lds + (size_t)c * 7 * 64 + (threadIdx.x & 63); }
LSG_DEVI void mf_put(uint32_t* lds, int c, const fp_t& v) {
  uint32_t* p = mf_slot(lds, c);
#pragma unroll
  for (int k = 0; k < LSG_PL; k++) p[k * 64] = v.l[k];
}
LSG_DEVI fp_t mf_get(uint32_t* lds, int c) {
  const uint32_t* p = mf_slot(lds, c);
  fp_t v;
#pragma unroll
  for (int k = 0; k < LSG_PL; k++) v.l[k] = p[k * 64];
  return v;
}
LSG_DEVI void mf_put2(uint32_t* lds, int c, const fp2_t& v) {
  mf_put(lds, c, v.c0);
  mf_put(lds, c + 1, v.c1);
}
LSG_DEVI fp2_t mf_get2(uint32_t* lds, int c) { return fp2_t(mf_get(lds, c), mf_get(lds, c + 1)); }
#define MF_FC(j) (MF_F + 2 * (j))
#define MF_LC(k, j) (MF_L + 6 * (k) + 2 * (j))
#define MF_VC(p) ((p) < 15 ? MF_V + 2 * (p) : ((p) == 15 ? MF_LC(1, 2) : MF_LC(3, 2)))

LSG_DEVI void mf_sqr(uint32_t* lds, int w) {
  {
    fp6_t x, y;
    const fp6_t a = fp6_make(mf_get2(lds, MF_FC(0)), mf_get2(lds, MF_FC(1)), mf_get2(lds, MF_FC(2)));
    const fp6_t b = fp6_make(mf_get2(lds, MF_FC(3)), mf_get2(lds, MF_FC(4)), mf_get2(lds, MF_FC(5)));
    if (w < 2) {
      x = a;
      y = b;
    } else {
      x = fp6_add(a, b);
      y = fp6_add(a, fp6_mul_v(b));
    }
    fp2_t p0, p1, p2;
    if ((w & 1) == 0) {
      p0 = fp2_mul(x.c0, y.c0);
      p1 = fp2_mul(x.c1, y.c1);
      p2 = fp2_mul(x.c2, y.c2);
    } else {
      p0 = fp2_mul(fp2_add(x.c1, x.c2), fp2_add(y.c1, y.c2));
      p1 = fp2_mul(fp2_add(x.c0, x.c1), fp2_add(y.c0, y.c1));
      p2 = fp2_mul(fp2_add(x.c0, x.c2), fp2_add(y.c0, y.c2));
    }
    mf_put2(lds, MF_VC(3 * w), p0);
    mf_put2(lds, MF_VC(3 * w + 1), p1);
    mf_put2(lds, MF_VC(3 * w + 2), p2);
  }
  __syncthreads();
  auto V = [&](int p) { return mf_get2(lds, MF_VC(p)); };
  fp2_t o0, o1, o2;
  if (w == 0) {
    o0 = mfc_sqr<0>(V);
    o1 = mfc_sqr<1>(V);
    o2 = mfc_sqr<2>(V);
  } else if (w == 1) {
    o0 = mfc_sqr<3>(V);
  } else if (w == 2) {
    o0 = mfc_sqr<4>(V);
  } else {
    o0 = mfc_sqr<5>(V);
  }
  if (w == 0) {
    mf_put2(lds, MF_FC(3), o0);
    mf_put2(lds, MF_FC(4), o1);
    mf_put2(lds, MF_FC(5), o2);
  } else {
    mf_put2(lds, MF_FC(w - 1), o0);
  }
}

LSG_DEVI void mf_pair_lines(uint32_t* lds, int w) {
  const int pi = w >> 1, h = w & 1;
  {
    const fp2_t a0 = mf_get2(lds, MF_LC(2 * pi, 0)), a1 = mf_get2(lds, MF_LC(2 * pi, 1)),
                a2 = mf_get2(lds, MF_LC(2 * pi, 2));
    const fp2_t b0 = mf_get2(lds, MF_LC(2 * pi + 1, 0)), b1 = mf_get2(lds, MF_LC(2 * pi + 1, 1)),
                b2 = mf_get2(lds, MF_LC(2 * pi + 1, 2));
    if (h == 0) {
      mf_put2(lds, MF_VC(6 * pi), fp2_mul(a0, b0));
      mf_put2(lds, MF_VC(6 * pi + 1), fp2_mul(a2, b2));
      mf_put2(lds, MF_VC(6 * pi + 2), fp2_mul(a1, b1));
    } else {
      mf_put2(lds, MF_VC(6 * pi + 3), fp2_mul(fp2_add(a0, a1), fp2_add(b0, b1)));
      mf_put2(lds, MF_VC(6 * pi + 4), fp2_mul(fp2_add(a0, a2), fp2_add(b0, b2)));
      mf_put2(lds, MF_VC(6 * pi + 5), fp2_mul(fp2_add(a1, a2), fp2_add(b1, b2)));
    }
  }
  __syncthreads();
  auto V = [&](int p) { return mf_get2(lds, MF_VC(6 * pi + p)); };
  if (h == 0) {
    mf_put2(lds, MF_LC(2 * pi, 0), mfc_pair<0>(V));
    mf_put2(lds, MF_LC(2 * pi, 1), mfc_pair<1>(V));
    mf_put2(lds, MF_LC(2 * pi, 2), V(2));
  } else {
    mf_put2(lds, MF_LC(2 * pi + 1, 0), mfc_pair<2>(V));
    mf_put2(lds, MF_LC(2 * pi + 1, 1), mfc_pair<3>(V));
  }
  __syncthreads();
}

LSG_DEVI void mf_mul_pair(uint32_t* lds, int w, int k) {
  {
    const fp2_t m0 = mf_get2(lds, MF_LC(2 * k, 0)), m1 = mf_get2(lds, MF_LC(2 * k, 1)), m2 = mf_get2(lds, MF_LC(2 * k, 2));
    if (w == 0) {
      const fp2_t a0 = mf_get2(lds, MF_FC(0)), a1 = mf_get2(lds, MF_FC(1)), a2 = mf_get2(lds, MF_FC(2));
      mf_put2(lds, MF_VC(0), fp2_mul(a0, m0));
      mf_put2(lds, MF_VC(1), fp2_mul(a1, m1));
      mf_put2(lds, MF_VC(2), fp2_mul(a2, m2));
      mf_put2(lds, MF_VC(3), fp2_mul(fp2_add(a0, a1), fp2_add(m0, m1)));
      mf_put2(lds, MF_VC(4), fp2_mul(fp2_add(a1, a2), fp2_add(m1, m2)));
    } else if (w == 1) {
      const fp2_t m4 = mf_get2(lds, MF_LC(2 * k + 1, 0)), m5 = mf_get2(lds, MF_LC(2 * k + 1, 1));
      const fp2_t b0 = mf_get2(lds, MF_FC(3)), b1 = mf_get2(lds, MF_FC(4));
      mf_put2(lds, MF_VC(5), fp2_mul(fp2_add(mf_get2(lds, MF_FC(0)), mf_get2(lds, MF_FC(2))), fp2_add(m0, m2)));
      mf_put2(lds, MF_VC(6), fp2_mul(b0, m4));
      mf_put2(lds, MF_VC(7), fp2_mul(b1, m5));
      mf_put2(lds, MF_VC(8), fp2_mul(fp2_add(b0, b1), fp2_add(m4, m5)));
    } else if (w == 2) {
      const fp2_t m4 = mf_get2(lds, MF_LC(2 * k + 1, 0)), m5 = mf_get2(lds, MF_LC(2 * k + 1, 1));
      const fp2_t b2 = mf_get2(lds, MF_FC(5));
      mf_put2(lds, MF_VC(9), fp2_mul(b2, m4));
      mf_put2(lds, MF_VC(10), fp2_mul(b2, m5));
      const fp2_t s0 = fp2_add(mf_get2(lds, MF_FC(0)), mf_get2(lds, MF_FC(3)));
      const fp2_t s1 = fp2_add(mf_get2(lds, MF_FC(1)), mf_get2(lds, MF_FC(4)));
      mf_put2(lds, MF_VC(11), fp2_mul(s0, m0));
      mf_put2(lds, MF_VC(12), fp2_mul(s1, fp2_add(m1, m4)));
    } else {
      const fp2_t m4 = mf_get2(lds, MF_LC(2 * k + 1, 0)), m5 = mf_get2(lds, MF_LC(2 * k + 1, 1));
      const fp2_t s0 = fp2_add(mf_get2(lds, MF_FC(0)), mf_get2(lds, MF_FC(3)));
      const fp2_t s1 = fp2_add(mf_get2(lds, MF_FC(1)), mf_get2(lds, MF_FC(4)));
      const fp2_t s2 = fp2_add(mf_get2(lds, MF_FC(2)), mf_get2(lds, MF_FC(5)));
      const fp2_t q1 = fp2_add(m1, m4), q2 = fp2_add(m2, m5);
      mf_put2(lds, MF_VC(13), fp2_mul(s2, q2));
      mf_put2(lds, MF_VC(14), fp2_mul(fp2_add(s0, s1), fp2_add(m0, q1)));
      mf_put2(lds, MF_VC(15), fp2_mul(fp2_add(s1, s2), fp2_add(q1, q2)));
      mf_put2(lds, MF_VC(16), fp2_mul(fp2_add(s0, s2), fp2_add(m0, q2)));
    }
  }
  __syncthreads();
  auto V = [&](int p) { return mf_get2(lds, MF_VC(p)); };
  fp2_t o0, o1;
  int j0, j1 = -1;
  if (w == 0) {
    o0 = mfc_mul<0>(V);
    o1 = mfc_mul<1>(V);
    j0 = 0;
    j1 = 1;
  } else if (w == 1) {
    o0 = mfc_mul<2>(V);
    o1 = mfc_mul<3>(V);
    j0 = 2;
    j1 = 3;
  } else if (w == 2) {
    o0 = mfc_mul<4>(V);
    j0 = 4;
  } else {
    o0 = mfc_mul<5>(V);
    j0 = 5;
  }
  mf_put2(lds, MF_FC(j0), o0);
  if (j1 >= 0) mf_put2(lds, MF_FC(j1), o1);
  __syncthreads();
}

#ifndef LSG_MF_STAGED
#define LSG_MF_STAGED 1
#endif
LSG_DEVI void mf_put_line(uint32_t* lds, int wl, bool use, const fp2_t& l00, const fp2_t& l01P, const fp2_t& l11P) {
  mf_put2(lds, MF_LC(wl, 0), fp2_select(use, l00, fp2_one()));
  mf_put2(lds, MF_LC(wl, 1), fp2_select(use, l01P, fp2_zero()));
  mf_put2(lds, MF_LC(wl, 2), fp2_select(use, l11P, fp2_zero()));
}
LSG_DEVI void mf_dbl_line(uint32_t* lds, int wl, bool use, const uint32_t* __restrict__ P, size_t sl) {
  const int tb = MF_T + 6 * wl;
  fp2_t t0, t1, t2, v1;
  {
    const fp2_t X = mf_get2(lds, tb), Y = mf_get2(lds, tb + 2), Z = mf_get2(lds, tb + 4);
    t0 = fp2_sqr(Y);
    t1 = fp2_mul(Y, Z);
    t2 = fp2_mul_b3(fp2_sqr(Z));
    const fp2_t XX = fp2_sqr(X);
    v1 = fp2_mul(X, Y);
    const g1a_t Pk = lane_load<g1a_t>(P, sl);
    mf_put_line(lds, wl, use, fp2_sub(t2, t0), fp2_mul_fp(fp2_mulk<3>(XX), Pk.x),
                fp2_mul_fp((-fp2s(t1)).carry_mul<2>(), Pk.y));
  }
  fp2_t Z3 = fp2_mulk<8>(t0);
  fp2_t X3 = fp2_mul(t2, Z3);
  fp2_t Y3 = fp2_add(t0, t2);
  mf_put2(lds, tb + 4, fp2_mul(t1, Z3));
  const fp2_t s0 = (fp2s(t0) - fp2s_mulk<3>(fp2s(t2))).carry();
  Y3 = fp2_mul(s0, Y3);
  mf_put2(lds, tb + 2, fp2_add(X3, Y3));
  X3 = fp2_mul(s0, v1);
  mf_put2(lds, tb, fp2_mulk<2>(X3));
}
LSG_DEVI void mf_add_line(uint32_t* lds, int wl, bool use, const uint32_t* __restrict__ P, const uint32_t* __restrict__ H,
                          size_t sl) {
  const int tb = MF_T + 6 * wl;
  fp2_t theta, delta;
  {
    const g2a_t Q = lane_load<g2a_t>(H, sl);
    const fp2_t Z = mf_get2(lds, tb + 4);
    theta = fp2_sub(mf_get2(lds, tb + 2), fp2_mul(Q.y, Z));
    delta = fp2_sub(mf_get2(lds, tb), fp2_mul(Q.x, Z));
    const fp2_t l00 = fp2_sub(fp2_mul(delta, Q.y), fp2_mul(theta, Q.x));
    const g1a_t Pk = lane_load<g1a_t>(P, sl);
    mf_put_line(lds, wl, use, l00, fp2_mul_fp(theta, Pk.x), fp2_mul_fp(fp2_neg(delta), Pk.y));
  }
  const fp2_t C = fp2_sqr(theta);
  const fp2_t D = fp2_sqr(delta);
  const fp2_t E = fp2_mul(D, delta);
  const fp2_t F = fp2_mul(mf_get2(lds, tb + 4), C);
  const fp2_t G = fp2_mul(mf_get2(lds, tb), D);
  const fp2_t Hs = (fp2s(E) + F - fp2s_mulk<2>(fp2s(G))).carry();
  mf_put2(lds, tb, fp2_mul(delta, Hs));
  const fp2_t Y3 = fp2_sub(fp2_mul(theta, fp2_sub(G, Hs)), fp2_mul(E, mf_get2(lds, tb + 2)));
  mf_put2(lds, tb + 2, Y3);
  mf_put2(lds, tb + 4, fp2_mul(E, mf_get2(lds, tb + 4)));
}

#ifndef LSG_MF_PRIO
#define LSG_MF_PRIO 2
#endif
#ifndef LSG_MF_WAVES
#define LSG_MF_WAVES 2
#endif
__global__ void __launch_bounds__(256) __attribute__((amdgpu_waves_per_eu(LSG_MF_WAVES)))
k_miller_fused(int n_items, const int32_t* __restrict__ item_first, const int32_t* __restrict__ item_cnt,
               const uint32_t* __restrict__ P, const uint8_t* __restrict__ pinf, const uint8_t* __restrict__ hinf,
               const int32_t* __restrict__ err, const uint32_t* __restrict__ H, uint32_t* __restrict__ f_out) {
  extern __shared__ uint32_t lds[];
#if LSG_MF_PRIO
  __builtin_amdgcn_s_setprio(LSG_MF_PRIO);
#endif
  const int w = __builtin_amdgcn_readfirstlane((int)(threadIdx.x >> 6));
  const size_t it = (size_t)blockIdx.x * MF_ITEMS + ((threadIdx.x & 63) >> 1);
  const bool live = it < (size_t)n_items;
  const size_t itc = live ? it : 0;
  const int first = item_first[itc], cnt = item_cnt[itc];
  const int si = first + (w < cnt ? w : cnt - 1);
  const uint64_t use_mask = __ballot(live && w < cnt && err[si] == 0 && !pinf[si] && !hinf[si]);
  {
    const g2p_t T = proj_from_aff(lane_load<g2a_t>(H, (size_t)si));
    mf_put2(lds, MF_T + 6 * w, T.X);
    mf_put2(lds, MF_T + 6 * w + 2, T.Y);
    mf_put2(lds, MF_T + 6 * w + 4, T.Z);
  }
  auto line_phase = [&](bool add) {
    int wl = w, sl = si;
    asm volatile("" : "+s"(wl), "+v"(sl));
#if LSG_MF_STAGED
    const bool use = (use_mask >> __lane_id()) & 1u;
    if (add)
      mf_add_line(lds, wl, use, P, H, (size_t)sl);
    else
      mf_dbl_line(lds, wl, use, P, (size_t)sl);
#else
    g2p_t T;
    T.X = mf_get2(lds, MF_T + 6 * wl);
    T.Y = mf_get2(lds, MF_T + 6 * wl + 2);
    T.Z = mf_get2(lds, MF_T + 6 * wl + 4);
    line_t L = add ? ml_add_step_raw(T, lane_load<g2a_t>(H, (size_t)sl)) : ml_dbl_step_raw(T);
    mf_put2(lds, MF_T + 6 * wl, T.X);
    mf_put2(lds, MF_T + 6 * wl + 2, T.Y);
    mf_put2(lds, MF_T + 6 * wl + 4, T.Z);
    const g1a_t Pk = lane_load<g1a_t>(P, (size_t)sl);
    L = line_eval(L, Pk.x, Pk.y);
    const bool use = (use_mask >> __lane_id()) & 1u;
    mf_put2(lds, MF_LC(wl, 0), fp2_select(use, L.l00, fp2_one()));
    mf_put2(lds, MF_LC(wl, 1), fp2_select(use, L.l01, fp2_zero()));
    mf_put2(lds, MF_LC(wl, 2), fp2_select(use, L.l11, fp2_zero()));
#endif
    __syncthreads();
    mf_pair_lines(lds, wl);
#pragma unroll 1
    for (int k = 0; k < 2; k++) mf_mul_pair(lds, wl, k);
  };
  if (w < 2) {
    mf_put2(lds, MF_FC(3 * w), w == 0 ? fp2_one() : fp2_zero());
    mf_put2(lds, MF_FC(3 * w + 1), fp2_zero());
    mf_put2(lds, MF_FC(3 * w + 2), fp2_zero());
  }
  const uint64_t xa = ((uint64_t)LSG_X_ABS_HI << 32) | LSG_X_ABS_LO;
  line_phase(false);
  line_phase(true);
#pragma unroll 1
  for (int b = 61; b >= 0; b--) {
    mf_sqr(lds, w);
    line_phase(false);
    if ((xa >> b) & 1u) line_phase(true);
  }
  if (live) {
    uint32_t* o = f_out + it * (size_t)lsgl::W_F12 + pair_h();
#pragma unroll
    for (int j = 0; j < 3; j++) {
      const int c = 3 * w + j;
      fp_t v = mf_get(lds, MF_F + c);
      if (c >= 6) v = fp_neg(v);
#pragma unroll
      for (int k = 0; k < LSG_PL; k++) o[(7 * c + k) * LSG_GROUP] = v.l[k];
    }
  }
}

namespace lsgk {
hipError_t miller_fused(hipStream_t st, int n_items, const int32_t* item_first, const int32_t* item_cnt,
                        const uint32_t* P, const uint8_t* pinf, const uint8_t* hinf, const int32_t* err,
                        const uint32_t* H, uint32_t* f) {
  if (n_items <= 0) return hipSuccess;
  static const hipError_t attr = hipFuncSetAttribute((const void*)k_miller_fused,
                                                     hipFuncAttributeMaxDynamicSharedMemorySize, (int)MF_LDS_BYTES);
  if (attr != hipSuccess) return attr;
  hipLaunchKernelGGL(k_miller_fused, dim3((n_items + MF_ITEMS - 1) / MF_ITEMS), dim3(256), MF_LDS_BYTES, st, n_items, item_first,
                     item_cnt, P, pinf, hinf, err, H, f);
  return hipGetLastError();
}
hipError_t miller_lines_list(hipStream_t st, int n, const int32_t* list, const uint32_t* H, uint32_t* lines) {
  LSG_LAUNCH_ITEMS(k_miller_lines_list, n, st, n, list, H, lines);
}
hipError_t miller_accum_list(hipStream_t st, int n, const int32_t* list, const uint32_t* P, const uint8_t* pinf,
                             const uint8_t* hinf, const int32_t* err, const uint32_t* lines, uint32_t* f) {
  LSG_LAUNCH_ITEMS(k_miller_accum_list, n, st, n, list, P, pinf, hinf, err, lines, f);
}
hipError_t miller_lines(hipStream_t st, int n, const uint32_t* H, uint32_t* lines) {
  LSG_LAUNCH_ITEMS(k_miller_lines, n, st, n, H, lines);
}
hipError_t miller_accum(hipStream_t st, int K, int n_items, const int32_t* item_first, const int32_t* item_cnt,
                        const uint32_t* P, const uint8_t* pinf, const uint8_t* hinf, const int32_t* err, int n_sets,
                        const uint32_t* lines, uint32_t* f) {
  if (K == 1) LSG_LAUNCH_ITEMS(k_miller_accum<1>, n_items, st, n_items, item_first, item_cnt, P, pinf, hinf, err, n_sets, lines, f);
  if (K == 2) LSG_LAUNCH_ITEMS(k_miller_accum<2>, n_items, st, n_items, item_first, item_cnt, P, pinf, hinf, err, n_sets, lines, f);
  LSG_LAUNCH_ITEMS(k_miller_accum<4>, n_items, st, n_items, item_first, item_cnt, P, pinf, hinf, err, n_sets, lines, f);
}
}
```

### lodestar_amd/csrc/lsg_k_reduce.hip

```cpp
#include "lsg_kcommon.hpp"
namespace {
#include "lsg_inv.hpp"
}

template <int OP>
struct seg_op;
template <>
struct seg_op<0> {
  typedef g1p_t T;
  static LSG_DEVI T ident() { return proj_inf<fp_t>(); }
  static LSG_DEVI T op(const T& a, const T& b) { return g1_add(a, b); }
};
template <>
struct seg_op<1> {
  typedef g2p_t T;
  static LSG_DEVI T ident() { return proj_inf<fp2_t>(); }
  static LSG_DEVI T op(const T& a, const T& b) { return g2_add(a, b); }
};
template <>
struct seg_op<2> {
  typedef fp12_t T;
  static LSG_DEVI T ident() { return fp12_one(); }
  static LSG_DEVI T op(const T& a, const T& b) { return fp12_mul(a, b); }
};
// ... 218 lines not shown
  auto put2 = [&](const fp2_t& v) {
    put(v.c0);
    put(v.c1);
  };
  const fp_t a = el(0), b = el(1), c = el(2);
  put((fps(a) + b + c - el(3) - el(4) - el(5)).carry());
  put(fp_mulk<2>(a));
  put(fp_mulk<3>(a));
  put(fp_mulk<4>(a));
  put(fp_mulk<8>(a));
  put(fp_mulk<12>(a));
  put2(fp2_mul_b3(fp2_t(a, b)));
  const jac_t<fp_t> j1 = {a, b, c};
  const jac_t<fp_t> r1 = jac_dbl(j1), n1 = check_jac_dbl_nested(j1);
  put(r1.X), put(r1.Y), put(r1.Z);
  put(n1.X), put(n1.Y), put(n1.Z);
  const jac_t<fp2_t> j2 = {el2(0), el2(1), el2(2)};
  const jac_t<fp2_t> r2 = jac_dbl(j2), n2 = check_jac_dbl_nested(j2);
  put2(r2.X), put2(r2.Y), put2(r2.Z);
  put2(n2.X), put2(n2.Y), put2(n2.Z);
  const g2p_t p = {el2(0), el2(1), el2(2)}, q = {el2(3), el2(4), el2(5)};
  const g2p_t r3 = g2_add(p, q), n3 = check_proj_add_nested(p, q);
  put2(r3.X), put2(r3.Y), put2(r3.Z);
  put2(n3.X), put2(n3.Y), put2(n3.Z);
  put2(mfc_mul<3>(el2));
  const fp2_t t2c = fp2_add(el2(11), fp2_mul_xi(fp2_sub(fp2_sub(el2(15), el2(12)), el2(13))));
  const fp2_t t0c = fp2_add(el2(0), fp2_mul_xi(fp2_sub(fp2_sub(el2(4), el2(1)), el2(2))));
  put2(fp2_sub(fp2_sub(t2c, t0c), fp2_mul_xi(fp2_add(el2(7), el2(9)))));
}

#ifdef LSG_FP2_LANES
__global__ void LSG_KERNEL_ATTR k_check_fp2_lanes(int n, const uint32_t* __restrict__ in, uint32_t* __restrict__ out) {
  LANE_ITEM(n);
  (void)lead;
  auto el2 = [&](int j) {
    return fp2_t(lane_load<fp_t>(in, (size_t)lsgk::CHECK_LANES_IN * item + 2 * j),
                 lane_load<fp_t>(in, (size_t)lsgk::CHECK_LANES_IN * item + 2 * j + 1));
  };
  int o = 0;
  auto put = [&](const fp2v_t& v) {
    const fp2_t w = fp2v_to_pair(v);
    lane_store(out, (size_t)lsgk::CHECK_LANES_OUT * item + (size_t)o, w.c0);
    lane_store(out, (size_t)lsgk::CHECK_LANES_OUT * item + (size_t)o + 1, w.c1);
    o += 2;
  };
  const fp2v_t A = fp2v_from_pair(el2(0)), B = fp2v_from_pair(el2(1)), C = fp2v_from_pair(el2(2));
  const fp2v_t D = fp2v_from_pair(el2(3)), E = fp2v_from_pair(el2(4)), F = fp2v_from_pair(el2(5));
  put(A);
  put(fmul(A, B));
  put(fsqr(A));
  put((fsum(A) + B + C - D - E - F).carry());
  put(fmulk<2>(A));
  put(fmulk<3>(A));
  put(fmulk<4>(A));
  put(fmulk<8>(A));
  put(fmulk<12>(A));
  put(fmul_b3(A));
  put(fneg(A));
  lane_store(out + (size_t)lsgk::CHECK_LANES_OUT * lsgl::W_FP * item + (size_t)o * lsgl::W_FP, 0, A);
}
__global__ void LSG_KERNEL_ATTR k_check_g2_lanes(int n, const uint32_t* __restrict__ in, uint32_t* __restrict__ out) {
  LANE_ITEM(n);
  (void)lead;
  auto el2 = [&](int j) {
    return fp2_t(lane_load<fp_t>(in, (size_t)lsgk::CHECK_G2L_IN * item + 2 * j),
                 lane_load<fp_t>(in, (size_t)lsgk::CHECK_G2L_IN * item + 2 * j + 1));
  };
  int o = 0;
  auto put2 = [&](const fp2_t& w) {
    lane_store(out, (size_t)lsgk::CHECK_G2L_OUT * item + (size_t)o, w.c0);
    lane_store(out, (size_t)lsgk::CHECK_G2L_OUT * item + (size_t)o + 1, w.c1);
    o += 2;
  };
  auto putv = [&](const jac_t<fp2v_t>& r) { put2(fp2v_to_pair(r.X)), put2(fp2v_to_pair(r.Y)), put2(fp2v_to_pair(r.Z)); };
  auto putp = [&](const jac_t<fp2_t>& r) { put2(r.X), put2(r.Y), put2(r.Z); };
  const jac_t<fp2_t> J = {el2(0), el2(1), el2(2)};
  const g2p_t Q = {el2(3), el2(4), el2(5)};
  const jac_t<fp2v_t> Jv = {fp2v_from_pair(J.X), fp2v_from_pair(J.Y), fp2v_from_pair(J.Z)};
  putv(jac_dbl(Jv));
  putp(jac_dbl(J));
  putv(jac_add_proj(Jv, g2v_from_pair(Q)));
  putp(jac_add_proj(J, Q));
}
#endif

constexpr int LSG_CHECK_CANON_OUT = lsgk::CHECK_CANON_OUT;
__global__ void LSG_KERNEL_ATTR k_check_canon(int n, const uint32_t* __restrict__ in, uint32_t* __restrict__ out) {
  LANE_ITEM(n);
  const fp_t a = lane_load<fp_t>(in, item);
  uint32_t* o = out + (size_t)LSG_CHECK_CANON_OUT * item;
  const fp_t c = fp_canonical(a);
  lane_store(o, 0, pair_canon(a));
  lane_store(o + 14, 0, c);
  fp_to_be48((uint8_t*)(o + 28), c);
  fp_to_be48((uint8_t*)(o + 42), a);
  const uint32_t f = (fp_is_zero(a) ? 1u : 0u) | (fp_canon_lt_p(a) ? 2u : 0u) | (fp_canon_gt_half(a) ? 4u : 0u) |
                     (fp_canon_parity(a) ? 8u : 0u);
  o[40 + (lead ? 0 : 1)] = lead ? f : 0u;
}
__global__ void LSG_KERNEL_ATTR k_check_from_bytes(int n, const uint8_t* __restrict__ in, uint32_t* __restrict__ out) {
  LANE_ITEM(n);
  (void)lead;
  lane_store(out, item, fp_from_be_bytes(in + 48 * item, 12));
}
constexpr int LSG_CHECK_ROOTS_OUT = lsgk::CHECK_ROOTS_OUT;
__global__ void LSG_KERNEL_ATTR k_check_fp2_roots(int n, const uint32_t* __restrict__ in, uint32_t* __restrict__ out) {
  LANE_ITEM(n);
  const fp2_t a(lane_load<fp_t>(in, 2 * item), lane_load<fp_t>(in, 2 * item + 1));
  uint32_t* o = out + (size_t)LSG_CHECK_ROOTS_OUT * item;
  fp2_t r;
  const bool ok = fp2_sqrt(r, a);
  lane_store(o, 0, r.c0);
  lane_store(o + 14, 0, r.c1);
  lane_store(o + 28, 0, fp_inv(a.c0));
  lane_store(o + 42, 0, pair_mont_mul(pair_inv_gcd(pair_canon(a.c0)), fp_t(FP_RCUBE)));
  const uint32_t f = (ok ? 1u : 0u) | (fp2_sgn0(a) ? 2u : 0u) | (fp2_lexi_largest(a) ? 4u : 0u) |
                     (fp2_is_zero(a) ? 8u : 0u);
  o[56 + (lead ? 0 : 1)] = lead ? f : 0u;
}

__global__ void LSG_KERNEL_ATTR k_probe_fp_mul(int n, int iters, uint32_t* __restrict__ io) {
  LANE_ITEM(n);
  (void)lead;
  fp_t a = lane_load<fp_t>(io, item), b = fp_t(FP_R2), c = fp_t(FP_R3), d = fp_t(FP_HALF);
  for (int k = 0; k < iters; k++) {
    a = fp_mul(a, b);
    b = fp_mul(b, c);
    c = fp_mul(c, d);
    d = fp_mul(d, a);
  }
  lane_store(io, item, fp_add(fp_add(a, b), fp_add(c, d)));
}

__global__ void __launch_bounds__(256) k_probe_mad(int iters, uint32_t seed, uint64_t* __restrict__ io) {
  const uint32_t t = blockIdx.x * blockDim.x + threadIdx.x;
  uint64_t acc[16];
  uint32_t x[16];
#pragma unroll
  for (int k = 0; k < 16; k++) {
    acc[k] = t + k;
    x[k] = (t * 2654435761u) ^ (seed + 977u * k);
  }
  const uint32_t y = seed | 1u;
  for (int i = 0; i < iters; i++) {
#pragma unroll
    for (int k = 0; k < 16; k++) acc[k] = (uint64_t)x[k] * y + acc[k];
  }
  uint64_t r = 0;
#pragma unroll
  for (int k = 0; k < 16; k++) r ^= acc[k];
  io[t] = r;
}

namespace lsgk {
hipError_t seg_reduce(hipStream_t st, int op, int n_chunks, int ips_log2, const int32_t* chunks, const int32_t* idx,
                      const uint32_t* src, uint32_t* dst, uint32_t* tmp) {
  const size_t items = (size_t)n_chunks << ips_log2;
  if (op == 0) LSG_LAUNCH_ITEMS(k_seg_reduce<0>, items, st, n_chunks, ips_log2, chunks, idx, src, dst, tmp);
  if (op == 1) LSG_LAUNCH_ITEMS(k_seg_reduce<1>, items, st, n_chunks, ips_log2, chunks, idx, src, dst, tmp);
  LSG_LAUNCH_ITEMS(k_seg_reduce<2>, items, st, n_chunks, ips_log2, chunks, idx, src, dst, tmp);
}
hipError_t binv_fold(hipStream_t st, int n, int zero_to_one, const uint32_t* in, uint32_t* pre, uint32_t* tot) {
  LSG_LAUNCH_ITEMS(k_binv_fold, (n + LSG_BINV_T - 1) / LSG_BINV_T, st, n, zero_to_one, in, pre, tot);
}
hipError_t binv_block(hipStream_t st, int n, int T, int zero_to_one, const uint32_t* in, uint32_t* pre, uint32_t* out) {
  if (n <= 0) return hipSuccess;
  const size_t chunks = ((size_t)n + T - 1) / T;
  hipLaunchKernelGGL(k_binv_block, dim3(lane_blocks(chunks)), dim3(LSG_TPB), 0, st, n, T, zero_to_one, in, pre, out);
  return hipGetLastError();
}
hipError_t binv_root(hipStream_t st, const uint32_t* top, uint32_t* inv) {
  LSG_LAUNCH_ITEMS(k_binv_root, 1, st, top, inv);
}
hipError_t binv_unfold(hipStream_t st, int n, int zero_to_one, const uint32_t* in, const uint32_t* pre,
                       const uint32_t* tinv, uint32_t* out) {
  LSG_LAUNCH_ITEMS(k_binv_unfold, (n + LSG_BINV_T - 1) / LSG_BINV_T, st, n, zero_to_one, in, pre, tinv, out);
}
hipError_t blobs_to_fp12(hipStream_t st, int n, const uint8_t* blobs, uint32_t* out) {
  LSG_LAUNCH_ITEMS(k_blobs_to_fp12, n, st, n, blobs, out);
}
hipError_t fp12_to_canon(hipStream_t st, int n, const uint32_t* in, uint8_t* out576) {
  LSG_LAUNCH_ITEMS(k_fp12_to_canon, n, st, n, in, out576);
}
hipError_t fp12_pow_u64(hipStream_t st, const uint8_t* in576, uint64_t r, uint8_t* out576) {
  LSG_LAUNCH_ITEMS(k_fp12_pow_u64, 1, st, in576, r, out576);
}
hipError_t check_fp2_mul(hipStream_t st, int n, const uint32_t* in, uint32_t* out) {
  LSG_LAUNCH_ITEMS(k_check_fp2_mul, n, st, n, in, out);
}
hipError_t check_fp_sqr(hipStream_t st, int n, const uint32_t* in, uint32_t* out) {
  LSG_LAUNCH_ITEMS(k_check_fp_sqr, n, st, n, in, out);
}
hipError_t check_fp2_sqr(hipStream_t st, int n, const uint32_t* in, uint32_t* out) {
  LSG_LAUNCH_ITEMS(k_check_fp2_sqr, n, st, n, in, out);
}
hipError_t check_sums(hipStream_t st, int n, const uint32_t* in, uint32_t* out) {
  LSG_LAUNCH_ITEMS(k_check_sums, n, st, n, in, out);
}
#ifdef LSG_FP2_LANES
hipError_t check_fp2_lanes(hipStream_t st, int n, const uint32_t* in, uint32_t* out) {
  LSG_LAUNCH_ITEMS(k_check_fp2_lanes, n, st, n, in, out);
}
hipError_t check_g2_lanes(hipStream_t st, int n, const uint32_t* in, uint32_t* out) {
  LSG_LAUNCH_ITEMS(k_check_g2_lanes, n, st, n, in, out);
}
#else
hipError_t check_fp2_lanes(hipStream_t, int, const uint32_t*, uint32_t*) { return hipErrorNotSupported; }
hipError_t check_g2_lanes(hipStream_t, int, const uint32_t*, uint32_t*) { return hipErrorNotSupported; }
#endif
hipError_t check_canon(hipStream_t st, int n, const uint32_t* in, uint32_t* out) {
  LSG_LAUNCH_ITEMS(k_check_canon, n, st, n, in, out);
}
hipError_t check_from_bytes(hipStream_t st, int n, const uint8_t* in, uint32_t* out) {
  LSG_LAUNCH_ITEMS(k_check_from_bytes, n, st, n, in, out);
}
hipError_t check_fp2_roots(hipStream_t st, int n, const uint32_t* in, uint32_t* out) {
  LSG_LAUNCH_ITEMS(k_check_fp2_roots, n, st, n, in, out);
}
hipError_t probe_fp_mul(hipStream_t st, int items, int iters, uint32_t* io) {
  LSG_LAUNCH_ITEMS(k_probe_fp_mul, items, st, items, iters, io);
}
hipError_t probe_mad(hipStream_t st, int blocks, int iters, uint32_t seed, uint64_t* io) {
  if (blocks <= 0) return hipSuccess;
  hipLaunchKernelGGL(k_probe_mad, dim3(blocks), dim3(256), 0, st, iters, seed, io);
  return hipGetLastError();
}
}
```

### lodestar_amd/csrc/lsg_launch.h

```cpp
#pragma once
#include <hip/hip_runtime.h>
#include <stddef.h>
#include <stdint.h>

constexpr uint32_t LSG_MC_ROW = 0x80000000u;

namespace lsgk {
hipError_t expand_msg(hipStream_t st, int n, const uint8_t* msg, const uint32_t* off, const uint32_t* len,
                      const uint8_t* dst, uint32_t dst_len, uint8_t* ub);
hipError_t h2c_prep(hipStream_t st, int n, const uint8_t* ub, uint32_t* U, uint32_t* norms);
hipError_t h2c_map(hipStream_t st, int n, const uint32_t* U, const uint32_t* ninv, uint32_t* Hp);
hipError_t h2c_clear(hipStream_t st, int n, uint32_t* Hp, uint32_t* zN, uint8_t* hinf, bool pair_form = false);
hipError_t h2c_gather(hipStream_t st, int n, const uint32_t* mid, const uint32_t* Hm, const uint8_t* hinfm, uint32_t* H,
                      uint8_t* hinf);
hipError_t h2c_affine(hipStream_t st, int n, const uint32_t* Hp, const uint32_t* ninv, const uint8_t* hinf,
                      uint32_t* H);
hipError_t h2c_cache_merge(hipStream_t st, int nm, const uint32_t* src, uint32_t n_rows, const uint32_t* rows,
                           const uint8_t* rinf, uint32_t n_miss, const uint32_t* Hx, const uint8_t* hinfx, uint32_t* Hm,
                           uint8_t* hinfm);
hipError_t h2c_cache_store(hipStream_t st, int n, const uint32_t* list, uint32_t n_miss, const uint32_t* Hx,
                           const uint8_t* hinfx, uint32_t n_rows, uint32_t* rows, uint8_t* rinf);
hipError_t signing_root(hipStream_t st, int n, const uint8_t* roots, const uint8_t* domains, uint32_t dstride,
                        uint8_t* out32);
hipError_t attestation_signing_root(hipStream_t st, int n, const uint8_t* data, const uint8_t* domains,
                                    uint32_t dstride, uint8_t* out32);
hipError_t deposit_signing_root(hipStream_t st, int n, const uint8_t* data, uint32_t stride, const uint8_t* domains,
                                uint32_t dstride, uint8_t* out32);
hipError_t object_signing_root(hipStream_t st, int n, const uint8_t* objs, uint32_t obj_len, const uint8_t* domains,
                               uint32_t dstride, uint8_t* out32);
hipError_t msg_roots(hipStream_t st, int n, uint8_t* msg, const uint32_t* off, uint32_t* len);

hipError_t sig_decode(hipStream_t st, int n, const uint8_t* sig, const uint32_t* sig_len, uint32_t* sig_aff,
                      uint8_t* inf, int32_t* err);
hipError_t sig_subgroup(hipStream_t st, int n, const uint32_t* sig_aff, const uint8_t* inf, int32_t* err,
                        bool pair_form = false);
hipError_t sig_prep(hipStream_t st, int n, const uint32_t* sig_aff, const uint8_t* inf, const int32_t* err,
                    const uint8_t* pinf, const uint64_t* rnd, const uint8_t* mode, uint32_t* out);
hipError_t sig_scale_only(hipStream_t st, int n, const uint32_t* sig_aff, const uint8_t* inf, const int32_t* err,
                          const uint8_t* pinf, const uint64_t* rnd, const uint8_t* mode, uint32_t* out);
hipError_t sig_agg_seg(hipStream_t st, int n_chunks, int ips_log2, const int32_t* chunks, const int32_t* gather,
                       const uint32_t* sig_aff, const uint8_t* inf, const int32_t* err, uint32_t* dst, uint32_t* tmp);
hipError_t g2a_to_bytes(hipStream_t st, int n, const uint32_t* pts, const uint8_t* inf, uint8_t* out192);
hipError_t g2p_compress(hipStream_t st, int n, const uint32_t* pts, uint8_t* out96);
hipError_t g2p_to_canon(hipStream_t st, int n, const uint32_t* pts, uint8_t* out288);
hipError_t sign(hipStream_t st, int n, const uint8_t* sks, const uint32_t* H, uint8_t* out96);

hipError_t pk_decode(hipStream_t st, int n, const uint8_t* pk, uint32_t stride, const uint32_t* pk_len, uint32_t* pts,
                     int32_t* err, const uint32_t* tab, const uint8_t* tab_ok, uint32_t tab_n);
hipError_t pk_validate(hipStream_t st, int n, const uint8_t* pk, uint32_t len, uint32_t* pts, int32_t* err);
hipError_t pk_keyvalidate(hipStream_t st, int n, const int32_t* keys, const uint8_t* pk, const uint32_t* pk_len,
                          int32_t* code);
hipError_t pk_keyvalidate_apply(hipStream_t st, int n, const int32_t* sets, const int32_t* code, int32_t* set_err);
hipError_t pk_gather_aff(hipStream_t st, int n, const uint8_t* pk, uint32_t stride, const uint32_t* pk_len, uint32_t* pts,
                         uint8_t* inf, int32_t* err, const uint32_t* tab, const uint8_t* tab_ok, uint32_t tab_n);
hipError_t pk_agg_seg(hipStream_t st, int n_chunks, int ips_log2, const int32_t* chunks, const uint8_t* pk, uint32_t stride,
                      const uint32_t* pk_len, int32_t* err, const uint32_t* tab, const uint8_t* tab_ok, uint32_t tab_n,
                      uint32_t* dst, uint32_t* tmp);
hipError_t pk_agg_bits(hipStream_t st, int n_pairs, const int32_t* pair_set, const int32_t* plan, const uint32_t* bits,
                       const uint32_t* cm_idx, const uint32_t* cm_off, const uint32_t* cm_sum, const uint32_t* tab,
                       const uint8_t* tab_ok, uint32_t tab_n, uint32_t* dst);
hipError_t pk_agg_bits_multi(hipStream_t st, int n_pairs, const int32_t* pair_set, const int32_t* set_plan,
                             const int32_t* part_plan, const uint32_t* bits, const uint32_t* cm_idx, const uint32_t* cm_off,
                             const uint32_t* cm_sum, const uint32_t* tab, const uint8_t* tab_ok, uint32_t tab_n,
                             uint32_t* dst);
struct AggTreeArgs {
  int L = 0, T = 1;
  int64_t n_c0 = 0, N0 = 0;
  const int32_t* blk_set = nullptr;
  const int32_t* set_o0 = nullptr;
  const int32_t* set_len = nullptr;
  const int32_t* set_pk0 = nullptr;
  const uint8_t* pk = nullptr;
  uint32_t stride = 0;
  const uint32_t* pk_len = nullptr;
  int32_t* pk_err = nullptr;
  const uint32_t* tab = nullptr;
  const uint8_t* tab_ok = nullptr;
  uint32_t tab_n = 0;
  uint32_t* pts = nullptr;
  uint8_t* inf = nullptr;
  uint32_t* pre[2] = {nullptr, nullptr};
  uint32_t* cinv[2] = {nullptr, nullptr};
  uint8_t* flag[2] = {nullptr, nullptr};
};
hipError_t agg_leaf(hipStream_t st, const AggTreeArgs& a);
hipError_t agg_step(hipStream_t st, const AggTreeArgs& a, int t);
hipError_t agg_final(hipStream_t st, const AggTreeArgs& a, int n_sets, const int32_t* src, uint32_t* agg);
hipError_t pk_scale(hipStream_t st, int n, const uint32_t* agg, const uint64_t* rnd, uint32_t* Pp, uint32_t* zP,
                    uint8_t* pinf);
hipError_t pk_affine(hipStream_t st, int n, const uint32_t* Pp, const uint32_t* zinv, uint32_t* P);
hipError_t pk_mask(hipStream_t st, int n, const uint32_t* Pp, const int32_t* err, const uint8_t* pinf, uint32_t* out);
hipError_t g1p_affine_inv(hipStream_t st, int n, const uint32_t* Pp, uint32_t* P, uint8_t* pinf);
hipError_t g1p_to_bytes(hipStream_t st, int n, const uint32_t* pts, uint8_t* out96);
hipError_t sk_to_pk(hipStream_t st, int n, const uint8_t* sks, uint8_t* out96);

hipError_t miller_fused(hipStream_t st, int n_items, const int32_t* item_first, const int32_t* item_cnt,
                        const uint32_t* P, const uint8_t* pinf, const uint8_t* hinf, const int32_t* err,
                        const uint32_t* H, uint32_t* f);
hipError_t miller_lines(hipStream_t st, int n, const uint32_t* H, uint32_t* lines);
hipError_t miller_lines_list(hipStream_t st, int n, const int32_t* list, const uint32_t* H, uint32_t* lines);
hipError_t miller_accum_list(hipStream_t st, int n, const int32_t* list, const uint32_t* P, const uint8_t* pinf,
                             const uint8_t* hinf, const int32_t* err, const uint32_t* lines, uint32_t* f);
hipError_t miller_accum(hipStream_t st, int K, int n_items, const int32_t* item_first, const int32_t* item_cnt,
                        const uint32_t* P, const uint8_t* pinf, const uint8_t* hinf, const int32_t* err, int n_sets,
                        const uint32_t* lines, uint32_t* f);

hipError_t seg_reduce(hipStream_t st, int op, int n_chunks, int ips_log2, const int32_t* chunks, const int32_t* idx,
                      const uint32_t* src, uint32_t* dst, uint32_t* tmp);
hipError_t binv_fold(hipStream_t st, int n, int zero_to_one, const uint32_t* in, uint32_t* pre, uint32_t* tot);
hipError_t binv_root(hipStream_t st, const uint32_t* top, uint32_t* inv);
hipError_t binv_block(hipStream_t st, int n, int T, int zero_to_one, const uint32_t* in, uint32_t* pre, uint32_t* out);
hipError_t binv_unfold(hipStream_t st, int n, int zero_to_one, const uint32_t* in, const uint32_t* pre,
                       const uint32_t* tinv, uint32_t* out);
hipError_t blobs_to_fp12(hipStream_t st, int n, const uint8_t* blobs, uint32_t* out);
hipError_t fp12_to_canon(hipStream_t st, int n, const uint32_t* in, uint8_t* out576);
hipError_t fp12_pow_u64(hipStream_t st, const uint8_t* in576, uint64_t r, uint8_t* out576);
hipError_t probe_fp_mul(hipStream_t st, int items, int iters, uint32_t* io);
hipError_t check_fp2_mul(hipStream_t st, int n, const uint32_t* in, uint32_t* out);
hipError_t check_fp_sqr(hipStream_t st, int n, const uint32_t* in, uint32_t* out);
hipError_t check_fp2_sqr(hipStream_t st, int n, const uint32_t* in, uint32_t* out);
hipError_t check_sums(hipStream_t st, int n, const uint32_t* in, uint32_t* out);
constexpr int CHECK_LANES_IN = 12, CHECK_LANES_OUT = 24, CHECK_G2L_IN = 12, CHECK_G2L_OUT = 24;
hipError_t check_fp2_lanes(hipStream_t st, int n, const uint32_t* in, uint32_t* out);
hipError_t check_g2_lanes(hipStream_t st, int n, const uint32_t* in, uint32_t* out);
constexpr int CHECK_CANON_OUT = 54, CHECK_ROOTS_OUT = 58;
hipError_t check_canon(hipStream_t st, int n, const uint32_t* in, uint32_t* out);
hipError_t check_from_bytes(hipStream_t st, int n, const uint8_t* in48, uint32_t* out);
hipError_t check_fp2_roots(hipStream_t st, int n, const uint32_t* in, uint32_t* out);
hipError_t probe_mad(hipStream_t st, int blocks, int iters, uint32_t seed, uint64_t* io);
}
```

### lodestar_amd/csrc/lsg_pairing.hpp

```cpp
#pragma once
#include "lsg_curve.hpp"

struct line_t {
  fp2_t l00, l01, l11;
};

LSG_BIGFN line_t ml_dbl_step_raw(g2p_t& T) {
  fp2_t t0 = fp2_sqr(T.Y);
  fp2_t t1 = fp2_mul(T.Y, T.Z);
  fp2_t t2 = fp2_mul_b3(fp2_sqr(T.Z));
  fp2_t XX = fp2_sqr(T.X);
  line_t L;
  L.l00 = fp2_sub(t2, t0);
  L.l01 = fp2_mulk<3>(XX);
  L.l11 = (-fp2s(t1)).carry_mul<2>();
  fp2_t Z3 = fp2_mulk<8>(t0);
  fp2_t X3 = fp2_mul(t2, Z3);
  fp2_t Y3 = fp2_add(t0, t2);
  Z3 = fp2_mul(t1, Z3);
  fp2_t s0 = (fp2s(t0) - fp2s_mulk<3>(fp2s(t2))).carry();
  Y3 = fp2_mul(s0, Y3);
  Y3 = fp2_add(X3, Y3);
  fp2_t v1 = fp2_mul(T.X, T.Y);
  X3 = fp2_mulk<2>(fp2_mul(s0, v1));
  T.X = X3;
  T.Y = Y3;
  T.Z = Z3;
  return L;
}

LSG_BIGFN line_t ml_add_step_raw(g2p_t& T, g2a_t Q) {
  fp2_t theta = fp2_sub(T.Y, fp2_mul(Q.y, T.Z));
  fp2_t delta = fp2_sub(T.X, fp2_mul(Q.x, T.Z));
  line_t L;
  L.l00 = fp2_sub(fp2_mul(delta, Q.y), fp2_mul(theta, Q.x));
  L.l01 = theta;
  L.l11 = fp2_neg(delta);
  fp2_t C = fp2_sqr(theta);
  fp2_t D = fp2_sqr(delta);
  fp2_t E = fp2_mul(D, delta);
  fp2_t F = fp2_mul(T.Z, C);
  fp2_t G = fp2_mul(T.X, D);
  fp2_t H = (fp2s(E) + F - fp2s_mulk<2>(fp2s(G))).carry();
  fp2_t X3 = fp2_mul(delta, H);
  fp2_t Y3 = fp2_sub(fp2_mul(theta, fp2_sub(G, H)), fp2_mul(E, T.Y));
  fp2_t Z3 = fp2_mul(E, T.Z);
  T.X = X3;
  T.Y = Y3;
  T.Z = Z3;
  return L;
}

LSG_INL line_t line_eval(line_t L, const fp_t& xP, const fp_t& yP) {
  L.l01 = fp2_mul_fp(L.l01, xP);
  L.l11 = fp2_mul_fp(L.l11, yP);
  return L;
}

template <int J, class G>
LSG_INL fp2_t mfc_sqr(const G& V) {
  if constexpr (J == 0) {
    return fp6_kar_s0(V(0), V(1), V(2), V(3)).template carry_mul<2>();
  } else if constexpr (J == 1) {
    return fp6_kar_s1(V(0), V(1), V(2), V(4)).template carry_mul<2>();
  } else if constexpr (J == 2) {
    return fp6_kar_s2(V(0), V(1), V(2), V(5)).template carry_mul<2>();
  } else if constexpr (J == 3) {
    const fp2_t d = (fp6_kar_s0(V(6), V(7), V(8), V(9)) - fp6_kar_s0(V(0), V(1), V(2), V(3))).carry();
    const fp2_t t2 = fp6_kar_s2(V(0), V(1), V(2), V(5)).carry();
    return (fp2s(d) - fp2s_mul_xi(t2)).carry();
  } else if constexpr (J == 4) {
    const fp2_t d = ((fp2s(V(10)) - V(6) - V(7)) - (fp2s(V(4)) - V(0) - V(1))).carry();
    const fp2_t e = (fp2s(d) + fp2s_mul_xi(fp2s(V(8)) - V(2))).carry();
    return (fp2s(e) - fp6_kar_s0(V(0), V(1), V(2), V(3))).carry();
  } else {
    const fp2_t d = ((fp2s(V(11)) - V(6) - V(8)) - (fp2s(V(5)) - V(0) - V(2))).carry();
    const fp2_t t1 = fp6_kar_s1(V(0), V(1), V(2), V(4)).carry();
    return (fp2s(d) + V(7) - V(1) - t1).carry();
  }
}
template <int J, class G>
LSG_INL fp2_t mfc_pair(const G& V) {
  if constexpr (J == 0) {
    return (fp2s(V(0)) + fp2s_mul_xi(V(1))).carry();
  } else if constexpr (J == 1) {
    return fp2_sub2(V(3), V(0), V(2));
  } else if constexpr (J == 2) {
    return fp2_sub2(V(4), V(0), V(1));
  } else {
    return fp2_sub2(V(5), V(2), V(1));
  }
}
template <int J, class G>
LSG_INL fp2_t mfc_mul(const G& V) {
  if constexpr (J == 0) {
    const fp2_t g = (fp2s(V(4)) - V(1) - V(2) + V(8)).carry();
    const fp2_t h = (fp2s(g) - V(6) - V(7)).carry();
    return (fp2s(V(0)) + fp2s_mul_xi(h)).carry();
  } else if constexpr (J == 1) {
    const fp2_t h = (fp2s(V(2)) + V(7) + V(9)).carry();
    return ((fp2s(V(3)) - V(0) - V(1)) + fp2s_mul_xi(h)).carry();
  } else if constexpr (J == 2) {
    const fp2_t n0 = (fp2s(V(6)) + fp2s_mul_xi(V(10))).carry();
    return (fp2s(V(5)) - V(0) - V(2) + V(1) + n0).carry();
  } else if constexpr (J == 3) {
    const fp2_t g = (fp2s(V(15)) - V(12) - V(13) + V(1) + V(2)).carry();
    const fp2_t h = (fp2s(g) - V(4) - V(7) - V(9)).carry();
    return (fp2s(V(11)) - V(0) + fp2s_mul_xi(h)).carry();
  } else if constexpr (J == 4) {
    const fp2_t a = ((fp2s(V(14)) - V(11) - V(12)) - (fp2s(V(3)) - V(0) - V(1))).carry();
    const fp2_t b = fp2_sub2(V(13), V(2), V(10));
    return (fp2s(a) - V(6) + fp2s_mul_xi(b)).carry();
  } else {
    const fp2_t g = (fp2s(V(11)) + V(13) + V(5) - V(16) - V(12) - V(0)).carry();
    return (fp2s(V(2)) + V(6) + V(7) - V(1) - V(8) - g).carry();
  }
}

#ifdef LSG_ROW_SPLIT
LSG_INL line_t ml_dbl_step_rows(g2p_t& T, const fp_t& xP, const fp_t& yP) {
  fp_t x[16], y[16], z[16];
  kar_prep(x, y, 0, T.Y, T.Y);
  kar_prep(x, y, 3, T.Y, T.Z);
  kar_prep(x, y, 6, T.Z, T.Z);
  kar_prep(x, y, 9, T.X, T.X);
  kar_prep(x, y, 12, T.X, T.Y);
  fp_mul_list<15>(z, x, y);
  const fp2_t t0 = kar_fin(z, 0), t1 = kar_fin(z, 3), t2 = fp2_mul_b3(kar_fin(z, 6)), XX = kar_fin(z, 9),
              v1 = kar_fin(z, 12);
  line_t L;
  L.l00 = fp2_sub(t2, t0);
  const fp2_t l01 = fp2_add(fp2_add(XX, XX), XX), l11 = fp2_neg(fp2_add(t1, t1));
  const fp2_t z8 = fp2_dbl(fp2_dbl(fp2_dbl(t0)));
  const fp2_t y3 = fp2_add(t0, t2);
  const fp2_t s0 = fp2_sub(t0, fp2_add(fp2_add(t2, t2), t2));
  kar_prep(x, y, 0, t2, z8);
  kar_prep(x, y, 3, t1, z8);
  kar_prep(x, y, 6, s0, y3);
  kar_prep(x, y, 9, s0, v1);
  x[12] = l01.c0;
  y[12] = xP;
  x[13] = l01.c1;
  y[13] = xP;
  x[14] = l11.c0;
  y[14] = yP;
  x[15] = l11.c1;
  y[15] = yP;
  fp_mul_list<16>(z, x, y);
  const fp2_t X3 = kar_fin(z, 0);
  T.X = fp2_dbl(kar_fin(z, 9));
  T.Y = fp2_add(X3, kar_fin(z, 6));
  T.Z = kar_fin(z, 3);
  L.l01 = fp2_t(z[12], z[13]);
  L.l11 = fp2_t(z[14], z[15]);
  return L;
}
LSG_INL line_t ml_add_step_rows(g2p_t& T, const g2a_t& Q, const fp_t& xP, const fp_t& yP) {
  fp_t x[13], y[13], z[13];
  kar_prep(x, y, 0, Q.y, T.Z);
  kar_prep(x, y, 3, Q.x, T.Z);
  fp_mul_list<6>(z, x, y);
  const fp2_t theta = fp2_sub(T.Y, kar_fin(z, 0)), delta = fp2_sub(T.X, kar_fin(z, 3));
  kar_prep(x, y, 0, delta, Q.y);
  kar_prep(x, y, 3, theta, Q.x);
  kar_prep(x, y, 6, theta, theta);
  kar_prep(x, y, 9, delta, delta);
  fp_mul_list<12>(z, x, y);
  line_t L;
  L.l00 = fp2_sub(kar_fin(z, 0), kar_fin(z, 3));
  const fp2_t C = kar_fin(z, 6), D = kar_fin(z, 9), l11 = fp2_neg(delta);
  kar_prep(x, y, 0, D, delta);
  kar_prep(x, y, 3, T.Z, C);
  kar_prep(x, y, 6, T.X, D);
  x[9] = theta.c0;
  y[9] = xP;
  x[10] = theta.c1;
  y[10] = xP;
  x[11] = l11.c0;
  y[11] = yP;
  x[12] = l11.c1;
  y[12] = yP;
  fp_mul_list<13>(z, x, y);
  const fp2_t E = kar_fin(z, 0), F = kar_fin(z, 3), G = kar_fin(z, 6);
  L.l01 = fp2_t(z[9], z[10]);
  L.l11 = fp2_t(z[11], z[12]);
  const fp2_t H = fp2_sub(fp2_add(E, F), fp2_add(G, G));
  kar_prep(x, y, 0, delta, H);
  kar_prep(x, y, 3, theta, fp2_sub(G, H));
  kar_prep(x, y, 6, E, T.Y);
  kar_prep(x, y, 9, E, T.Z);
  fp_mul_list<12>(z, x, y);
  T.X = kar_fin(z, 0);
  T.Y = fp2_sub(kar_fin(z, 3), kar_fin(z, 6));
  T.Z = kar_fin(z, 9);
  return L;
}
LSG_INL line_t ml_dbl_step(g2p_t& T, fp_t xP, fp_t yP) { return ml_dbl_step_rows(T, xP, yP); }
LSG_INL line_t ml_add_step(g2p_t& T, g2a_t Q, fp_t xP, fp_t yP) { return ml_add_step_rows(T, Q, xP, yP); }
// ... 148 lines not shown
```

Measured before the change: 3.687 million.

## Run fused Miller-loop Fp12 arithmetic in lane-split Fp2 form

Templates the fused Miller kernel's Fp12 square, line-pair and multiply stages on the field type so they can run on the lane-split fp2v_t representation, where each Fp2 is spread across two lanes. This adds lane versions of mul-by-xi, mul-by-Fp, Fp6 helpers and LDS get/put, and makes this path the default behind the LSG_MF_LANES switch. The aim is to halve the per-thread work and register pressure of the Fp2 multiplies in the hot Miller loop. The cost is extra lane swaps and a different LDS access pattern. A check kernel is added to validate the lane arithmetic against the pair form.

```diff
diff --git a/include/lodestar_bls.h b/include/lodestar_bls.h
--- a/include/lodestar_bls.h
+++ b/include/lodestar_bls.h
@@ -173,6 +173,7 @@
 int lsg_check_sums(lsg_ctx* ctx, const uint32_t* in, size_t n, uint32_t* out);
 int lsg_check_fp2_lanes(lsg_ctx* ctx, const uint32_t* in, size_t n, uint32_t* out);
 int lsg_check_g2_lanes(lsg_ctx* ctx, const uint32_t* in, size_t n, uint32_t* out);
+int lsg_check_mf_lanes(lsg_ctx* ctx, const uint32_t* in, size_t n, uint32_t* out);
 int lsg_check_canon(lsg_ctx* ctx, const uint32_t* in, size_t n, const uint8_t* bytes48, size_t nb, uint32_t* out,
                     uint32_t* out_limbs);
 int lsg_check_fp2_roots(lsg_ctx* ctx, const uint32_t* in, size_t n, uint32_t* out);
diff --git a/lodestar_amd/_native.py b/lodestar_amd/_native.py
--- a/lodestar_amd/_native.py
+++ b/lodestar_amd/_native.py
@@ -172,7 +172,7 @@
     "lsg_final_submit_groups", "lsg_final_wait_groups", "lsg_aggregate_signatures",
     "lsg_signing_roots", "lsg_attestation_signing_roots", "lsg_jobs_partial_device", "lsg_final_submit_device",
     "lsg_set_coalesce", "lsg_aggregate_pubkeys_multi", "lsg_check_fp2_mul",
-    "lsg_check_fp_sqr", "lsg_check_fp2_sqr", "lsg_check_sums", "lsg_check_fp2_lanes", "lsg_check_g2_lanes",
+    "lsg_check_fp_sqr", "lsg_check_fp2_sqr", "lsg_check_sums", "lsg_check_fp2_lanes", "lsg_check_g2_lanes", "lsg_check_mf_lanes",
     "lsg_check_canon", "lsg_check_fp2_roots", "lsg_check_batch_inv", "lsg_check_map_uniform",
     "lsg_check_batch_partial_rnd",
     "lsg_deposit_signing_roots", "lsg_verify_deposits",
@@ -256,6 +256,7 @@
         lib.lsg_check_sums.argtypes = [vp, ctypes.c_char_p, sz, ctypes.c_char_p]
         lib.lsg_check_fp2_lanes.argtypes = [vp, ctypes.c_char_p, sz, ctypes.c_char_p]
         lib.lsg_check_g2_lanes.argtypes = [vp, ctypes.c_char_p, sz, ctypes.c_char_p]
+        lib.lsg_check_mf_lanes.argtypes = [vp, ctypes.c_char_p, sz, ctypes.c_char_p]
         lib.lsg_check_canon.argtypes = [vp, ctypes.c_char_p, sz, ctypes.c_char_p, sz, ctypes.c_char_p, ctypes.c_char_p]
         lib.lsg_check_fp2_roots.argtypes = [vp, ctypes.c_char_p, sz, ctypes.c_char_p]
         lib.lsg_check_batch_inv.argtypes = [vp, ctypes.c_char_p, sz, ctypes.c_char_p]
@@ -806,6 +807,9 @@
     def check_g2_lanes(self, words):
         return self._check_lanes("lsg_check_g2_lanes", words)
 
+    def check_mf_lanes(self, words):
+        return self._check_lanes("lsg_check_mf_lanes", words)
+
     def check_canon(self, words, strings=()):
         n, nb = len(words) // 14, len(strings)
         assert len(words) == 14 * n and all(len(b) == 48 for b in strings)
diff --git a/lodestar_amd/csrc/lsg_curve.hpp b/lodestar_amd/csrc/lsg_curve.hpp
--- a/lodestar_amd/csrc/lsg_curve.hpp
+++ b/lodestar_amd/csrc/lsg_curve.hpp
@@ -22,6 +22,11 @@
 template <class F> LSG_INL F fsub2(const F& a, const F& b, const F& c) { return (fsum(a) - b - c).carry(); }
 LSG_INL fp_t fmul_b3(const fp_t& a) { return fp_mul12(a); }
 LSG_INL fp2_t fmul_b3(const fp2_t& a) { return fp2_mul_b3(a); }
+template <int P0, int N0, int P1, int N1>
+LSG_INL auto fsum_mul_xi(const fp2s_t<P0, N0, P1, N1>& a) { return fp2s_mul_xi(a); }
+LSG_INL fp2s_t<1, 1, 2, 0> fsum_mul_xi(const fp2_t& a) { return fp2s_mul_xi(a); }
+LSG_INL fp2_t fmul_xi(const fp2_t& a) { return fp2_mul_xi(a); }
+LSG_INL fp2_t fmul_fp(const fp2_t& a, const fp_t& k) { return fp2_mul_fp(a, k); }
 LSG_INL bool fis_zero(const fp_t& a) { return fp_is_zero(a); }
 LSG_INL bool fis_zero(const fp2_t& a) { return fp2_is_zero(a); }
 LSG_INL bool feq(const fp_t& a, const fp_t& b) { return fp_eq(a, b); }
diff --git a/lodestar_amd/csrc/lsg_fp2_lanes.hpp b/lodestar_amd/csrc/lsg_fp2_lanes.hpp
--- a/lodestar_amd/csrc/lsg_fp2_lanes.hpp
+++ b/lodestar_amd/csrc/lsg_fp2_lanes.hpp
@@ -78,6 +78,7 @@
   V = odd ? own : own + partner;
   s = odd ? partner + partner : own - partner;
 }
+LSG_PFN uint32_t lanes_xi_operand(uint32_t own, uint32_t partner, bool odd) { return odd ? own + partner : own - partner; }
 
 #if LSG_PAIR_G == 2 && !defined(LSG_NO_FP2_LANES)
 #define LSG_FP2_LANES 1
@@ -140,6 +141,18 @@
   return r;
 }
 
+struct fpv_t {
+  uint32_t l[LSG_VL];
+};
+LSG_PLEAF fp2v_t lanes_fp2_mul_fp_v(LSG_LANES_PARAMS(va), LSG_LANES_PARAMS(vk)) {
+  fp2v_t a = LSG_LANES_UNPACK(va), k = LSG_LANES_UNPACK(vk);
+#pragma unroll
+  for (int j = 0; j < LSG_VL; j++) LSG_LANES_HIDE(a.l[j]);
+  fp2v_t r;
+  lanes_mul_pass(r.l, a.l, k.l);
+  return r;
+}
+
 LSG_PFN fp2v_t fp2v_from_pair(const fp2_t& a) {
   const bool odd = lanes_odd();
   fp2v_t r;
@@ -159,6 +172,17 @@
     const uint32_t s = lanes_swap(odd ? a.l[k] : a.l[LSG_PL + k]);
     r.c0.l[k] = odd ? s : a.l[k];
     r.c1.l[k] = odd ? a.l[LSG_PL + k] : s;
+  }
+  return r;
+}
+LSG_PFN fpv_t fpv_from_pair(const fp_t& a) {
+  const bool odd = lanes_odd();
+  fpv_t r;
+#pragma unroll
+  for (int k = 0; k < LSG_PL; k++) {
+    const uint32_t s = lanes_swap(a.l[k]);
+    r.l[k] = odd ? s : a.l[k];
+    r.l[LSG_PL + k] = odd ? a.l[k] : s;
   }
   return r;
 }
@@ -243,6 +267,17 @@
   for (int k = 0; k < LSG_VL; k++) r.l[k] = a.l[k] * (uint32_t)K;
   return r;
 }
+
+constexpr int lanes_max(int a, int b) { return a > b ? a : b; }
+template <int P, int N>
+LSG_PFN fp2vs_t<lanes_max(P + N, 2 * P), lanes_max(P + N, 2 * N)> fsum_mul_xi(const fp2vs_t<P, N>& a) {
+  const bool odd = lanes_odd();
+  fp2vs_t<lanes_max(P + N, 2 * P), lanes_max(P + N, 2 * N)> r;
+#pragma unroll
+  for (int k = 0; k < LSG_VL; k++) r.l[k] = lanes_xi_operand(a.l[k], lanes_swap(a.l[k]), odd);
+  return r;
+}
+LSG_PFN fp2vs_t<2, 1> fsum_mul_xi(const fp2v_t& a) { return fsum_mul_xi(fsum(a)); }
 
 LSG_PFN fp2v_t fmul(const fp2v_t& a, const fp2v_t& b) { return lanes_fp2_mul_v(LSG_LANES_ARGS(a), LSG_LANES_ARGS(b)); }
 LSG_PFN fp2v_t fsqr(const fp2v_t& a) { return lanes_fp2_sqr_v(LSG_LANES_ARGS(a)); }
@@ -251,15 +286,13 @@
 LSG_PFN fp2v_t fneg(const fp2v_t& a) { return (-fsum(a)).carry(); }
 template <int K>
 LSG_PFN fp2v_t fmulk(const fp2v_t& a) { return fsum(a).template carry_mul<K>(); }
-LSG_PFN fp2v_t fmul_b3(const fp2v_t& a) {
-  const bool odd = lanes_odd();
-  fp2vs_t<2, 1> x;
-#pragma unroll
-  for (int k = 0; k < LSG_VL; k++) {
-    const uint32_t o = lanes_swap(a.l[k]);
-    x.l[k] = odd ? a.l[k] + o : a.l[k] - o;
-  }
-  return fmulk<12>(x.carry());
+LSG_PFN fp2v_t fmul_b3(const fp2v_t& a) { return fmulk<12>(fsum_mul_xi(a).carry()); }
+LSG_PFN fp2v_t fmul_xi(const fp2v_t& a) { return fsum_mul_xi(a).carry(); }
+LSG_PFN fp2v_t fmul_fp(const fp2v_t& a, const fpv_t& k) {
+  fp2v_t kv;
+#pragma unroll
+  for (int j = 0; j < LSG_VL; j++) kv.l[j] = k.l[j];
+  return lanes_fp2_mul_fp_v(LSG_LANES_ARGS(a), LSG_LANES_ARGS(kv));
 }
 LSG_PFN fp2v_t fselect(bool c, const fp2v_t& a, const fp2v_t& b) {
   fp2v_t r;
@@ -268,4 +301,22 @@
   return r;
 }
 LSG_PFN bool fis_zero(const fp2v_t& a) { return fp2_is_zero(fp2v_to_pair(a)); }
+
+struct fp6v_t {
+  fp2v_t c0, c1, c2;
+};
+LSG_PFN fp6v_t fp6_make(const fp2v_t& a, const fp2v_t& b, const fp2v_t& c) { return fp6v_t{a, b, c}; }
+LSG_PFN fp6v_t fp6_add(const fp6v_t& a, const fp6v_t& b) {
+  return fp6v_t{fadd(a.c0, b.c0), fadd(a.c1, b.c1), fadd(a.c2, b.c2)};
+}
+LSG_PFN fp6v_t fp6_mul_v(const fp6v_t& a) { return fp6v_t{fmul_xi(a.c2), a.c0, a.c1}; }
+LSG_PFN fp2vs_t<3, 1> fp6_kar_s0(const fp2v_t& v0, const fp2v_t& v1, const fp2v_t& v2, const fp2v_t& m0) {
+  return fsum(v0) + fsum_mul_xi((fsum(m0) - v1 - v2).carry());
+}
+LSG_PFN fp2vs_t<3, 3> fp6_kar_s1(const fp2v_t& v0, const fp2v_t& v1, const fp2v_t& v2, const fp2v_t& m1) {
+  return (fsum(m1) - v0 - v1) + fsum_mul_xi(v2);
+}
+LSG_PFN fp2vs_t<2, 2> fp6_kar_s2(const fp2v_t& v0, const fp2v_t& v1, const fp2v_t& v2, const fp2v_t& m2) {
+  return (fsum(m2) - v0 - v2) + v1;
+}
 #endif
diff --git a/lodestar_amd/csrc/lsg_host.hip b/lodestar_amd/csrc/lsg_host.hip
--- a/lodestar_amd/csrc/lsg_host.hip
+++ b/lodestar_amd/csrc/lsg_host.hip
@@ -509,6 +509,7 @@
 }
 
 bool miller_fused() { return lsg_ab_long("LSG_MILLER_FUSED", 1) != 0; }
+static bool mf_lanes_on() { return lsg_ab_long("LSG_MF_LANES", 1) != 0; }
 
 size_t slp_items_max();
 int miller_k_for(size_t n_sets) {
@@ -1150,9 +1151,14 @@
     return LSG_OK;
   }
   if (miller_fused()) {
-    KL(s, "k_miller_fused", lsgk::miller_fused(S_(s), ni, items, items + ni, P_<uint32_t>(s->d_P), P_<uint8_t>(s->d_pinf),
-                                              P_<uint8_t>(s->d_hinf), P_<int32_t>(s->d_seterr), P_<uint32_t>(s->d_H),
-                                              fall));
+    if (mf_lanes_on())
+      KL(s, "k_miller_fused", lsgk::miller_fused(S_(s), ni, items, items + ni, P_<uint32_t>(s->d_P), P_<uint8_t>(s->d_pinf),
+                                                P_<uint8_t>(s->d_hinf), P_<int32_t>(s->d_seterr), P_<uint32_t>(s->d_H),
+                                                fall));
+    else
+      KL(s, "k_miller_fused_pair",
+         lsgk::miller_fused(S_(s), ni, items, items + ni, P_<uint32_t>(s->d_P), P_<uint8_t>(s->d_pinf),
+                            P_<uint8_t>(s->d_hinf), P_<int32_t>(s->d_seterr), P_<uint32_t>(s->d_H), fall, true));
     return LSG_OK;
   }
   KL(s, "k_miller_accum",
@@ -3781,7 +3787,7 @@
   return LSG_OK;
 }
 
-static int check_lanes(lsg_ctx* c, const uint32_t* in, size_t n, uint32_t* out, bool g2) {
+static int check_lanes(lsg_ctx* c, const uint32_t* in, size_t n, uint32_t* out, bool g2, bool mf = false) {
   const size_t EIN = g2 ? lsgk::CHECK_G2L_IN : lsgk::CHECK_LANES_IN, EOUT = g2 ? lsgk::CHECK_G2L_OUT : lsgk::CHECK_LANES_OUT;
   if (!c || (n && (!in || !out)) || n > 0x7fffffffull / (4 * W_FP * EOUT)) return LSG_ERR_INVALID_ARG;
   LSG_ENTER(c);
@@ -3793,6 +3799,8 @@
   LSG_HIP(s, hipMemcpyAsync(s->d_aux.p, in, 4 * EIN * W_FP * n, hipMemcpyHostToDevice, s->st[0]));
   if (g2)
     KL(s, "k_check_g2_lanes", lsgk::check_g2_lanes(S_(s), (int)n, P_<uint32_t>(s->d_aux), P_<uint32_t>(s->d_Fb)));
+  else if (mf)
+    KL(s, "k_check_mf_lanes", lsgk::check_mf_lanes(S_(s), (int)n, P_<uint32_t>(s->d_aux), P_<uint32_t>(s->d_Fb)));
   else
     KL(s, "k_check_fp2_lanes", lsgk::check_fp2_lanes(S_(s), (int)n, P_<uint32_t>(s->d_aux), P_<uint32_t>(s->d_Fb)));
   LSG_HIP(s, hipMemcpyAsync(out, s->d_Fb.p, 4 * EOUT * W_FP * n, hipMemcpyDeviceToHost, s->st[0]));
@@ -3801,6 +3809,9 @@
 }
 int lsg_check_fp2_lanes(lsg_ctx* c, const uint32_t* in, size_t n, uint32_t* out) { return check_lanes(c, in, n, out, false); }
 int lsg_check_g2_lanes(lsg_ctx* c, const uint32_t* in, size_t n, uint32_t* out) { return check_lanes(c, in, n, out, true); }
+int lsg_check_mf_lanes(lsg_ctx* c, const uint32_t* in, size_t n, uint32_t* out) {
+  return check_lanes(c, in, n, out, false, true);
+}
 
 int lsg_check_canon(lsg_ctx* c, const uint32_t* in, size_t n, const uint8_t* bytes48, size_t nb, uint32_t* out,
                     uint32_t* out_limbs) {
diff --git a/lodestar_amd/csrc/lsg_k_miller.hip b/lodestar_amd/csrc/lsg_k_miller.hip
--- a/lodestar_amd/csrc/lsg_k_miller.hip
+++ b/lodestar_amd/csrc/lsg_k_miller.hip
@@ -92,40 +92,79 @@
   mf_put(lds, c, v.c0);
   mf_put(lds, c + 1, v.c1);
 }
-LSG_DEVI fp2_t mf_get2(uint32_t* lds, int c) { return fp2_t(mf_get(lds, c), mf_get(lds, c + 1)); }
+template <class F>
+LSG_DEVI F mf_get2(uint32_t* lds, int c);
+template <>
+LSG_DEVI fp2_t mf_get2<fp2_t>(uint32_t* lds, int c) {
+  return fp2_t(mf_get(lds, c), mf_get(lds, c + 1));
+}
+template <class F>
+struct mf_layout;
+template <>
+struct mf_layout<fp2_t> {
+  static LSG_DEVI const fp_t& fp_in(const fp_t& a) { return a; }
+  static LSG_DEVI fp_t fp_out(uint32_t* lds, int c) { return mf_get(lds, c); }
+  static LSG_DEVI fp2_t one() { return fp2_one(); }
+};
+#ifdef LSG_FP2_LANES
+LSG_DEVI void mf_put2(uint32_t* lds, int c, const fp2v_t& v) {
+  uint32_t* p = mf_slot(lds, c);
+#pragma unroll
+  for (int k = 0; k < LSG_VL; k++) p[k * 64] = v.l[k];
+}
+template <>
+LSG_DEVI fp2v_t mf_get2<fp2v_t>(uint32_t* lds, int c) {
+  const uint32_t* p = mf_slot(lds, c);
+  fp2v_t v;
+#pragma unroll
+  for (int k = 0; k < LSG_VL; k++) v.l[k] = p[k * 64];
+  return v;
+}
+template <>
+struct mf_layout<fp2v_t> {
+  static LSG_DEVI fpv_t fp_in(const fp_t& a) { return fpv_from_pair(a); }
+  static LSG_DEVI fp2v_t one() {
+    uint32_t odd = pair_h();
+    asm volatile("" : "+v"(odd));
+    fp2v_t r;
+#pragma unroll
+    for (int k = 0; k < LSG_VL; k++) r.l[k] = odd ? 0u : fpc_t(FP_ONE).l[k];
+    return r;
+  }
+  static LSG_DEVI fp_t fp_out(uint32_t* lds, int c) {
+    const uint32_t* p = lds + (size_t)((c & ~1) + (int)pair_h()) * 7 * 64 + ((threadIdx.x & 62) | (c & 1));
+    fp_t v;
+#pragma unroll
+    for (int k = 0; k < LSG_PL; k++) v.l[k] = p[k * 64];
+    return v;
+  }
+};
+#endif
 #define MF_FC(j) (MF_F + 2 * (j))
 #define MF_LC(k, j) (MF_L + 6 * (k) + 2 * (j))
 #define MF_VC(p) ((p) < 15 ? MF_V + 2 * (p) : ((p) == 15 ? MF_LC(1, 2) : MF_LC(3, 2)))
 
+template <class F>
 LSG_DEVI void mf_sqr(uint32_t* lds, int w) {
   {
-    fp6_t x, y;
-    const fp6_t a = fp6_make(mf_get2(lds, MF_FC(0)), mf_get2(lds, MF_FC(1)), mf_get2(lds, MF_FC(2)));
-    const fp6_t b = fp6_make(mf_get2(lds, MF_FC(3)), mf_get2(lds, MF_FC(4)), mf_get2(lds, MF_FC(5)));
-    if (w < 2) {
-      x = a;
-      y = b;
-    } else {
+    const auto a = fp6_make(mf_get2<F>(lds, MF_FC(0)), mf_get2<F>(lds, MF_FC(1)), mf_get2<F>(lds, MF_FC(2)));
+    const auto b = fp6_make(mf_get2<F>(lds, MF_FC(3)), mf_get2<F>(lds, MF_FC(4)), mf_get2<F>(lds, MF_FC(5)));
+    auto x = a, y = b;
+    if (w >= 2) {
       x = fp6_add(a, b);
       y = fp6_add(a, fp6_mul_v(b));
     }
-    fp2_t p0, p1, p2;
-    if ((w & 1) == 0) {
-      p0 = fp2_mul(x.c0, y.c0);
-      p1 = fp2_mul(x.c1, y.c1);
-      p2 = fp2_mul(x.c2, y.c2);
-    } else {
-      p0 = fp2_mul(fp2_add(x.c1, x.c2), fp2_add(y.c1, y.c2));
-      p1 = fp2_mul(fp2_add(x.c0, x.c1), fp2_add(y.c0, y.c1));
-      p2 = fp2_mul(fp2_add(x.c0, x.c2), fp2_add(y.c0, y.c2));
+    if (w & 1) {
+      x = fp6_make(fadd(x.c1, x.c2), fadd(x.c0, x.c1), fadd(x.c0, x.c2));
+      y = fp6_make(fadd(y.c1, y.c2), fadd(y.c0, y.c1), fadd(y.c0, y.c2));
     }
-    mf_put2(lds, MF_VC(3 * w), p0);
-    mf_put2(lds, MF_VC(3 * w + 1), p1);
-    mf_put2(lds, MF_VC(3 * w + 2), p2);
+    mf_put2(lds, MF_VC(3 * w), fmul(x.c0, y.c0));
+    mf_put2(lds, MF_VC(3 * w + 1), fmul(x.c1, y.c1));
+    mf_put2(lds, MF_VC(3 * w + 2), fmul(x.c2, y.c2));
   }
   __syncthreads();
-  auto V = [&](int p) { return mf_get2(lds, MF_VC(p)); };
-  fp2_t o0, o1, o2;
+  auto V = [&](int p) { return mf_get2<F>(lds, MF_VC(p)); };
+  F o0, o1, o2;
   if (w == 0) {
     o0 = mfc_sqr<0>(V);
     o1 = mfc_sqr<1>(V);
@@ -146,25 +185,26 @@
   }
 }
 
+template <class F>
 LSG_DEVI void mf_pair_lines(uint32_t* lds, int w) {
   const int pi = w >> 1, h = w & 1;
   {
-    const fp2_t a0 = mf_get2(lds, MF_LC(2 * pi, 0)), a1 = mf_get2(lds, MF_LC(2 * pi, 1)),
-                a2 = mf_get2(lds, MF_LC(2 * pi, 2));
-    const fp2_t b0 = mf_get2(lds, MF_LC(2 * pi + 1, 0)), b1 = mf_get2(lds, MF_LC(2 * pi + 1, 1)),
-                b2 = mf_get2(lds, MF_LC(2 * pi + 1, 2));
+    const F a0 = mf_get2<F>(lds, MF_LC(2 * pi, 0)), a1 = mf_get2<F>(lds, MF_LC(2 * pi, 1)),
+                a2 = mf_get2<F>(lds, MF_LC(2 * pi, 2));
+    const F b0 = mf_get2<F>(lds, MF_LC(2 * pi + 1, 0)), b1 = mf_get2<F>(lds, MF_LC(2 * pi + 1, 1)),
+                b2 = mf_get2<F>(lds, MF_LC(2 * pi + 1, 2));
     if (h == 0) {
-      mf_put2(lds, MF_VC(6 * pi), fp2_mul(a0, b0));
-      mf_put2(lds, MF_VC(6 * pi + 1), fp2_mul(a2, b2));
-      mf_put2(lds, MF_VC(6 * pi + 2), fp2_mul(a1, b1));
+      mf_put2(lds, MF_VC(6 * pi), fmul(a0, b0));
+      mf_put2(lds, MF_VC(6 * pi + 1), fmul(a2, b2));
+      mf_put2(lds, MF_VC(6 * pi + 2), fmul(a1, b1));
     } else {
-      mf_put2(lds, MF_VC(6 * pi + 3), fp2_mul(fp2_add(a0, a1), fp2_add(b0, b1)));
-      mf_put2(lds, MF_VC(6 * pi + 4), fp2_mul(fp2_add(a0, a2), fp2_add(b0, b2)));
-      mf_put2(lds, MF_VC(6 * pi + 5), fp2_mul(fp2_add(a1, a2), fp2_add(b1, b2)));
+      mf_put2(lds, MF_VC(6 * pi + 3), fmul(fadd(a0, a1), fadd(b0, b1)));
+      mf_put2(lds, MF_VC(6 * pi + 4), fmul(fadd(a0, a2), fadd(b0, b2)));
+      mf_put2(lds, MF_VC(6 * pi + 5), fmul(fadd(a1, a2), fadd(b1, b2)));
     }
   }
   __syncthreads();
-  auto V = [&](int p) { return mf_get2(lds, MF_VC(6 * pi + p)); };
+  auto V = [&](int p) { return mf_get2<F>(lds, MF_VC(6 * pi + p)); };
   if (h == 0) {
     mf_put2(lds, MF_LC(2 * pi, 0), mfc_pair<0>(V));
     mf_put2(lds, MF_LC(2 * pi, 1), mfc_pair<1>(V));
@@ -176,47 +216,48 @@
   __syncthreads();
 }
 
+template <class F>
 LSG_DEVI void mf_mul_pair(uint32_t* lds, int w, int k) {
   {
-    const fp2_t m0 = mf_get2(lds, MF_LC(2 * k, 0)), m1 = mf_get2(lds, MF_LC(2 * k, 1)), m2 = mf_get2(lds, MF_LC(2 * k, 2));
+    const F m0 = mf_get2<F>(lds, MF_LC(2 * k, 0)), m1 = mf_get2<F>(lds, MF_LC(2 * k, 1)), m2 = mf_get2<F>(lds, MF_LC(2 * k, 2));
     if (w == 0) {
-      const fp2_t a0 = mf_get2(lds, MF_FC(0)), a1 = mf_get2(lds, MF_FC(1)), a2 = mf_get2(lds, MF_FC(2));
-      mf_put2(lds, MF_VC(0), fp2_mul(a0, m0));
-      mf_put2(lds, MF_VC(1), fp2_mul(a1, m1));
-      mf_put2(lds, MF_VC(2), fp2_mul(a2, m2));
-      mf_put2(lds, MF_VC(3), fp2_mul(fp2_add(a0, a1), fp2_add(m0, m1)));
-      mf_put2(lds, MF_VC(4), fp2_mul(fp2_add(a1, a2), fp2_add(m1, m2)));
+      const F a0 = mf_get2<F>(lds, MF_FC(0)), a1 = mf_get2<F>(lds, MF_FC(1)), a2 = mf_get2<F>(lds, MF_FC(2));
+      mf_put2(lds, MF_VC(0), fmul(a0, m0));
+      mf_put2(lds, MF_VC(1), fmul(a1, m1));
+      mf_put2(lds, MF_VC(2), fmul(a2, m2));
+      mf_put2(lds, MF_VC(3), fmul(fadd(a0, a1), fadd(m0, m1)));
+      mf_put2(lds, MF_VC(4), fmul(fadd(a1, a2), fadd(m1, m2)));
     } else if (w == 1) {
-      const fp2_t m4 = mf_get2(lds, MF_LC(2 * k + 1, 0)), m5 = mf_get2(lds, MF_LC(2 * k + 1, 1));
-      const fp2_t b0 = mf_get2(lds, MF_FC(3)), b1 = mf_get2(lds, MF_FC(4));
-      mf_put2(lds, MF_VC(5), fp2_mul(fp2_add(mf_get2(lds, MF_FC(0)), mf_get2(lds, MF_FC(2))), fp2_add(m0, m2)));
-      mf_put2(lds, MF_VC(6), fp2_mul(b0, m4));
-      mf_put2(lds, MF_VC(7), fp2_mul(b1, m5));
-      mf_put2(lds, MF_VC(8), fp2_mul(fp2_add(b0, b1), fp2_add(m4, m5)));
+      const F m4 = mf_get2<F>(lds, MF_LC(2 * k + 1, 0)), m5 = mf_get2<F>(lds, MF_LC(2 * k + 1, 1));
+      const F b0 = mf_get2<F>(lds, MF_FC(3)), b1 = mf_get2<F>(lds, MF_FC(4));
+      mf_put2(lds, MF_VC(5), fmul(fadd(mf_get2<F>(lds, MF_FC(0)), mf_get2<F>(lds, MF_FC(2))), fadd(m0, m2)));
+      mf_put2(lds, MF_VC(6), fmul(b0, m4));
+      mf_put2(lds, MF_VC(7), fmul(b1, m5));
+      mf_put2(lds, MF_VC(8), fmul(fadd(b0, b1), fadd(m4, m5)));
     } else if (w == 2) {
-      const fp2_t m4 = mf_get2(lds, MF_LC(2 * k + 1, 0)), m5 = mf_get2(lds, MF_LC(2 * k + 1, 1));
-      const fp2_t b2 = mf_get2(lds, MF_FC(5));
-      mf_put2(lds, MF_VC(9), fp2_mul(b2, m4));
-      mf_put2(lds, MF_VC(10), fp2_mul(b2, m5));
-      const fp2_t s0 = fp2_add(mf_get2(lds, MF_FC(0)), mf_get2(lds, MF_FC(3)));
-      const fp2_t s1 = fp2_add(mf_get2(lds, MF_FC(1)), mf_get2(lds, MF_FC(4)));
-      mf_put2(lds, MF_VC(11), fp2_mul(s0, m0));
-      mf_put2(lds, MF_VC(12), fp2_mul(s1, fp2_add(m1, m4)));
+      const F m4 = mf_get2<F>(lds, MF_LC(2 * k + 1, 0)), m5 = mf_get2<F>(lds, MF_LC(2 * k + 1, 1));
+      const F b2 = mf_get2<F>(lds, MF_FC(5));
+      mf_put2(lds, MF_VC(9), fmul(b2, m4));
+      mf_put2(lds, MF_VC(10), fmul(b2, m5));
+      const F s0 = fadd(mf_get2<F>(lds, MF_FC(0)), mf_get2<F>(lds, MF_FC(3)));
+      const F s1 = fadd(mf_get2<F>(lds, MF_FC(1)), mf_get2<F>(lds, MF_FC(4)));
+      mf_put2(lds, MF_VC(11), fmul(s0, m0));
+      mf_put2(lds, MF_VC(12), fmul(s1, fadd(m1, m4)));
     } else {
-      const fp2_t m4 = mf_get2(lds, MF_LC(2 * k + 1, 0)), m5 = mf_get2(lds, MF_LC(2 * k + 1, 1));
-      const fp2_t s0 = fp2_add(mf_get2(lds, MF_FC(0)), mf_get2(lds, MF_FC(3)));
-      const fp2_t s1 = fp2_add(mf_get2(lds, MF_FC(1)), mf_get2(lds, MF_FC(4)));
-      const fp2_t s2 = fp2_add(mf_get2(lds, MF_FC(2)), mf_get2(lds, MF_FC(5)));
-      const fp2_t q1 = fp2_add(m1, m4), q2 = fp2_add(m2, m5);
-      mf_put2(lds, MF_VC(13), fp2_mul(s2, q2));
-      mf_put2(lds, MF_VC(14), fp2_mul(fp2_add(s0, s1), fp2_add(m0, q1)));
-      mf_put2(lds, MF_VC(15), fp2_mul(fp2_add(s1, s2), fp2_add(q1, q2)));
-      mf_put2(lds, MF_VC(16), fp2_mul(fp2_add(s0, s2), fp2_add(m0, q2)));
+      const F m4 = mf_get2<F>(lds, MF_LC(2 * k + 1, 0)), m5 = mf_get2<F>(lds, MF_LC(2 * k + 1, 1));
+      const F s0 = fadd(mf_get2<F>(lds, MF_FC(0)), mf_get2<F>(lds, MF_FC(3)));
+      const F s1 = fadd(mf_get2<F>(lds, MF_FC(1)), mf_get2<F>(lds, MF_FC(4)));
+      const F s2 = fadd(mf_get2<F>(lds, MF_FC(2)), mf_get2<F>(lds, MF_FC(5)));
+      const F q1 = fadd(m1, m4), q2 = fadd(m2, m5);
+      mf_put2(lds, MF_VC(13), fmul(s2, q2));
+      mf_put2(lds, MF_VC(14), fmul(fadd(s0, s1), fadd(m0, q1)));
+      mf_put2(lds, MF_VC(15), fmul(fadd(s1, s2), fadd(q1, q2)));
+      mf_put2(lds, MF_VC(16), fmul(fadd(s0, s2), fadd(m0, q2)));
     }
   }
   __syncthreads();
-  auto V = [&](int p) { return mf_get2(lds, MF_VC(p)); };
-  fp2_t o0, o1;
+  auto V = [&](int p) { return mf_get2<F>(lds, MF_VC(p)); };
+  F o0, o1;
   int j0, j1 = -1;
   if (w == 0) {
     o0 = mfc_mul<0>(V);
@@ -240,61 +281,62 @@
   __syncthreads();
 }
 
-#ifndef LSG_MF_STAGED
-#define LSG_MF_STAGED 1
-#endif
-LSG_DEVI void mf_put_line(uint32_t* lds, int wl, bool use, const fp2_t& l00, const fp2_t& l01P, const fp2_t& l11P) {
-  mf_put2(lds, MF_LC(wl, 0), fp2_select(use, l00, fp2_one()));
-  mf_put2(lds, MF_LC(wl, 1), fp2_select(use, l01P, fp2_zero()));
-  mf_put2(lds, MF_LC(wl, 2), fp2_select(use, l11P, fp2_zero()));
-}
+template <class F>
+LSG_DEVI void mf_put_line(uint32_t* lds, int wl, bool use, const F& l00, const F& l01P, const F& l11P) {
+  mf_put2(lds, MF_LC(wl, 0), fselect(use, l00, mf_layout<F>::one()));
+  mf_put2(lds, MF_LC(wl, 1), fselect(use, l01P, fzero<F>()));
+  mf_put2(lds, MF_LC(wl, 2), fselect(use, l11P, fzero<F>()));
+}
+template <class F>
 LSG_DEVI void mf_dbl_line(uint32_t* lds, int wl, bool use, const uint32_t* __restrict__ P, size_t sl) {
   const int tb = MF_T + 6 * wl;
-  fp2_t t0, t1, t2, v1;
-  {
-    const fp2_t X = mf_get2(lds, tb), Y = mf_get2(lds, tb + 2), Z = mf_get2(lds, tb + 4);
-    t0 = fp2_sqr(Y);
-    t1 = fp2_mul(Y, Z);
-    t2 = fp2_mul_b3(fp2_sqr(Z));
-    const fp2_t XX = fp2_sqr(X);
-    v1 = fp2_mul(X, Y);
+  F t0, t1, t2, v1;
+  {
+    const F X = mf_get2<F>(lds, tb), Y = mf_get2<F>(lds, tb + 2), Z = mf_get2<F>(lds, tb + 4);
+    t0 = fsqr(Y);
+    t1 = fmul(Y, Z);
+    t2 = fmul_b3(fsqr(Z));
+    const F XX = fsqr(X);
+    v1 = fmul(X, Y);
     const g1a_t Pk = lane_load<g1a_t>(P, sl);
-    mf_put_line(lds, wl, use, fp2_sub(t2, t0), fp2_mul_fp(fp2_mulk<3>(XX), Pk.x),
-                fp2_mul_fp((-fp2s(t1)).carry_mul<2>(), Pk.y));
-  }
-  fp2_t Z3 = fp2_mulk<8>(t0);
-  fp2_t X3 = fp2_mul(t2, Z3);
-  fp2_t Y3 = fp2_add(t0, t2);
-  mf_put2(lds, tb + 4, fp2_mul(t1, Z3));
-  const fp2_t s0 = (fp2s(t0) - fp2s_mulk<3>(fp2s(t2))).carry();
-  Y3 = fp2_mul(s0, Y3);
-  mf_put2(lds, tb + 2, fp2_add(X3, Y3));
-  X3 = fp2_mul(s0, v1);
-  mf_put2(lds, tb, fp2_mulk<2>(X3));
-}
+    mf_put_line(lds, wl, use, fsub(t2, t0), fmul_fp(fmulk<3>(XX), mf_layout<F>::fp_in(Pk.x)),
+                fmul_fp((-fsum(t1)).template carry_mul<2>(), mf_layout<F>::fp_in(Pk.y)));
+  }
+  F Z3 = fmulk<8>(t0);
+  F X3 = fmul(t2, Z3);
+  F Y3 = fadd(t0, t2);
+  mf_put2(lds, tb + 4, fmul(t1, Z3));
+  const F s0 = (fsum(t0) - fsum_mulk<3>(fsum(t2))).carry();
+  Y3 = fmul(s0, Y3);
+  mf_put2(lds, tb + 2, fadd(X3, Y3));
+  X3 = fmul(s0, v1);
+  mf_put2(lds, tb, fmulk<2>(X3));
+}
+template <class F>
 LSG_DEVI void mf_add_line(uint32_t* lds, int wl, bool use, const uint32_t* __restrict__ P, const uint32_t* __restrict__ H,
                           size_t sl) {
   const int tb = MF_T + 6 * wl;
-  fp2_t theta, delta;
-  {
-    const g2a_t Q = lane_load<g2a_t>(H, sl);
-    const fp2_t Z = mf_get2(lds, tb + 4);
-    theta = fp2_sub(mf_get2(lds, tb + 2), fp2_mul(Q.y, Z));
-    delta = fp2_sub(mf_get2(lds, tb), fp2_mul(Q.x, Z));
-    const fp2_t l00 = fp2_sub(fp2_mul(delta, Q.y), fp2_mul(theta, Q.x));
+  F theta, delta;
+  {
+    const aff_t<F> Q = g2_layout<F>::in(lane_load<g2a_t>(H, sl));
+    const F Z = mf_get2<F>(lds, tb + 4);
+    theta = fsub(mf_get2<F>(lds, tb + 2), fmul(Q.y, Z));
+    delta = fsub(mf_get2<F>(lds, tb), fmul(Q.x, Z));
+    const F l00 = fsub(fmul(delta, Q.y), fmul(theta, Q.x));
     const g1a_t Pk = lane_load<g1a_t>(P, sl);
-    mf_put_line(lds, wl, use, l00, fp2_mul_fp(theta, Pk.x), fp2_mul_fp(fp2_neg(delta), Pk.y));
-  }
-  const fp2_t C = fp2_sqr(theta);
-  const fp2_t D = fp2_sqr(delta);
-  const fp2_t E = fp2_mul(D, delta);
-  const fp2_t F = fp2_mul(mf_get2(lds, tb + 4), C);
-  const fp2_t G = fp2_mul(mf_get2(lds, tb), D);
-  const fp2_t Hs = (fp2s(E) + F - fp2s_mulk<2>(fp2s(G))).carry();
-  mf_put2(lds, tb, fp2_mul(delta, Hs));
-  const fp2_t Y3 = fp2_sub(fp2_mul(theta, fp2_sub(G, Hs)), fp2_mul(E, mf_get2(lds, tb + 2)));
+    mf_put_line(lds, wl, use, l00, fmul_fp(theta, mf_layout<F>::fp_in(Pk.x)),
+                fmul_fp(fneg(delta), mf_layout<F>::fp_in(Pk.y)));
+  }
+  const F C = fsqr(theta);
+  const F D = fsqr(delta);
+  const F E = fmul(D, delta);
+  const F Fz = fmul(mf_get2<F>(lds, tb + 4), C);
+  const F G = fmul(mf_get2<F>(lds, tb), D);
+  const F Hs = (fsum(E) + Fz - fsum_mulk<2>(fsum(G))).carry();
+  mf_put2(lds, tb, fmul(delta, Hs));
+  const F Y3 = fsub(fmul(theta, fsub(G, Hs)), fmul(E, mf_get2<F>(lds, tb + 2)));
   mf_put2(lds, tb + 2, Y3);
-  mf_put2(lds, tb + 4, fp2_mul(E, mf_get2(lds, tb + 4)));
+  mf_put2(lds, tb + 4, fmul(E, mf_get2<F>(lds, tb + 4)));
 }
 
 #ifndef LSG_MF_PRIO
@@ -303,11 +345,12 @@
 #ifndef LSG_MF_WAVES
 #define LSG_MF_WAVES 2
 #endif
-__global__ void __launch_bounds__(256) __attribute__((amdgpu_waves_per_eu(LSG_MF_WAVES)))
-k_miller_fused(int n_items, const int32_t* __restrict__ item_first, const int32_t* __restrict__ item_cnt,
-               const uint32_t* __restrict__ P, const uint8_t* __restrict__ pinf, const uint8_t* __restrict__ hinf,
-               const int32_t* __restrict__ err, const uint32_t* __restrict__ H, uint32_t* __restrict__ f_out) {
-  extern __shared__ uint32_t lds[];
+#define MF_KERNEL_PARAMS                                                                                        \
+  int n_items, const int32_t *__restrict__ item_first, const int32_t *__restrict__ item_cnt,                   \
+      const uint32_t *__restrict__ P, const uint8_t *__restrict__ pinf, const uint8_t *__restrict__ hinf,      \
+      const int32_t *__restrict__ err, const uint32_t *__restrict__ H, uint32_t *__restrict__ f_out
+template <class F>
+LSG_DEVI void mf_body(uint32_t* lds, MF_KERNEL_PARAMS) {
 #if LSG_MF_PRIO
   __builtin_amdgcn_s_setprio(LSG_MF_PRIO);
 #endif
@@ -319,7 +362,7 @@
   const int si = first + (w < cnt ? w : cnt - 1);
   const uint64_t use_mask = __ballot(live && w < cnt && err[si] == 0 && !pinf[si] && !hinf[si]);
   {
-    const g2p_t T = proj_from_aff(lane_load<g2a_t>(H, (size_t)si));
+    const proj_t<F> T = proj_from_aff(g2_layout<F>::in(lane_load<g2a_t>(H, (size_t)si)));
     mf_put2(lds, MF_T + 6 * w, T.X);
     mf_put2(lds, MF_T + 6 * w + 2, T.Y);
     mf_put2(lds, MF_T + 6 * w + 4, T.Z);
@@ -327,44 +370,29 @@
   auto line_phase = [&](bool add) {
     int wl = w, sl = si;
     asm volatile("" : "+s"(wl), "+v"(sl));
-#if LSG_MF_STAGED
     const bool use = (use_mask >> __lane_id()) & 1u;
     if (add)
-      mf_add_line(lds, wl, use, P, H, (size_t)sl);
+      mf_add_line<F>(lds, wl, use, P, H, (size_t)sl);
     else
-      mf_dbl_line(lds, wl, use, P, (size_t)sl);
-#else
-    g2p_t T;
-    T.X = mf_get2(lds, MF_T + 6 * wl);
-    T.Y = mf_get2(lds, MF_T + 6 * wl + 2);
-    T.Z = mf_get2(lds, MF_T + 6 * wl + 4);
-    line_t L = add ? ml_add_step_raw(T, lane_load<g2a_t>(H, (size_t)sl)) : ml_dbl_step_raw(T);
-    mf_put2(lds, MF_T + 6 * wl, T.X);
-    mf_put2(lds, MF_T + 6 * wl + 2, T.Y);
-    mf_put2(lds, MF_T + 6 * wl + 4, T.Z);
-    const g1a_t Pk = lane_load<g1a_t>(P, (size_t)sl);
-    L = line_eval(L, Pk.x, Pk.y);
-    const bool use = (use_mask >> __lane_id()) & 1u;
-    mf_put2(lds, MF_LC(wl, 0), fp2_select(use, L.l00, fp2_one()));
-    mf_put2(lds, MF_LC(wl, 1), fp2_select(use, L.l01, fp2_zero()));
-    mf_put2(lds, MF_LC(wl, 2), fp2_select(use, L.l11, fp2_zero()));
-#endif
+      mf_dbl_line<F>(lds, wl, use, P, (size_t)sl);
     __syncthreads();
-    mf_pair_lines(lds, wl);
+    mf_pair_lines<F>(lds, wl);
 #pragma unroll 1
-    for (int k = 0; k < 2; k++) mf_mul_pair(lds, wl, k);
+    for (int k = 0; k < 2; k++) mf_mul_pair<F>(lds, wl, k);
   };
   if (w < 2) {
-    mf_put2(lds, MF_FC(3 * w), w == 0 ? fp2_one() : fp2_zero());
-    mf_put2(lds, MF_FC(3 * w + 1), fp2_zero());
-    mf_put2(lds, MF_FC(3 * w + 2), fp2_zero());
+    mf_put2(lds, MF_FC(3 * w), w == 0 ? fone<F>() : fzero<F>());
+    mf_put2(lds, MF_FC(3 * w + 1), fzero<F>());
+    mf_put2(lds, MF_FC(3 * w + 2), fzero<F>());
   }
   const uint64_t xa = ((uint64_t)LSG_X_ABS_HI << 32) | LSG_X_ABS_LO;
   line_phase(false);
   line_phase(true);
 #pragma unroll 1
   for (int b = 61; b >= 0; b--) {
-    mf_sqr(lds, w);
+    int ws = w;
+    asm volatile("" : "+s"(ws));
+    mf_sqr<F>(lds, ws);
     line_phase(false);
     if ((xa >> b) & 1u) line_phase(true);
   }
@@ -373,25 +401,56 @@
 #pragma unroll
     for (int j = 0; j < 3; j++) {
       const int c = 3 * w + j;
-      fp_t v = mf_get(lds, MF_F + c);
+      fp_t v = mf_layout<F>::fp_out(lds, MF_F + c);
       if (c >= 6) v = fp_neg(v);
 #pragma unroll
       for (int k = 0; k < LSG_PL; k++) o[(7 * c + k) * LSG_GROUP] = v.l[k];
     }
   }
 }
+#define MF_KERNEL_ATTR __launch_bounds__(256) __attribute__((amdgpu_waves_per_eu(LSG_MF_WAVES)))
+#define MF_KERNEL_ARGS n_items, item_first, item_cnt, P, pinf, hinf, err, H, f_out
+#ifdef LSG_FP2_LANES
+__global__ void MF_KERNEL_ATTR k_miller_fused(MF_KERNEL_PARAMS) {
+  extern __shared__ uint32_t lds[];
+  mf_body<fp2v_t>(lds, MF_KERNEL_ARGS);
+}
+__global__ void MF_KERNEL_ATTR k_miller_fused_pair(MF_KERNEL_PARAMS) {
+  extern __shared__ uint32_t lds[];
+  mf_body<fp2_t>(lds, MF_KERNEL_ARGS);
+}
+#else
+__global__ void MF_KERNEL_ATTR k_miller_fused(MF_KERNEL_PARAMS) {
+  extern __shared__ uint32_t lds[];
+  mf_body<fp2_t>(lds, MF_KERNEL_ARGS);
+}
+#endif
 
 namespace lsgk {
+template <class K>
+static hipError_t mf_launch(K kernel, hipError_t attr, hipStream_t st, int n_items, const int32_t* item_first,
+                            const int32_t* item_cnt, const uint32_t* P, const uint8_t* pinf, const uint8_t* hinf,
+                            const int32_t* err, const uint32_t* H, uint32_t* f) {
+  if (attr != hipSuccess) return attr;
+  hipLaunchKernelGGL(kernel, dim3((n_items + MF_ITEMS - 1) / MF_ITEMS), dim3(256), MF_LDS_BYTES, st, n_items, item_first,
+                     item_cnt, P, pinf, hinf, err, H, f);
+  return hipGetLastError();
+}
 hipError_t miller_fused(hipStream_t st, int n_items, const int32_t* item_first, const int32_t* item_cnt,
                         const uint32_t* P, const uint8_t* pinf, const uint8_t* hinf, const int32_t* err,
-                        const uint32_t* H, uint32_t* f) {
+                        const uint32_t* H, uint32_t* f, bool pair_form) {
   if (n_items <= 0) return hipSuccess;
+#ifdef LSG_FP2_LANES
+  if (pair_form) {
+    static const hipError_t attr_pair = hipFuncSetAttribute(
+        (const void*)k_miller_fused_pair, hipFuncAttributeMaxDynamicSharedMemorySize, (int)MF_LDS_BYTES);
+    return mf_launch(k_miller_fused_pair, attr_pair, st, n_items, item_first, item_cnt, P, pinf, hinf, err, H, f);
+  }
+#endif
+  (void)pair_form;
   static const hipError_t attr = hipFuncSetAttribute((const void*)k_miller_fused,
                                                      hipFuncAttributeMaxDynamicSharedMemorySize, (int)MF_LDS_BYTES);
-  if (attr != hipSuccess) return attr;
-  hipLaunchKernelGGL(k_miller_fused, dim3((n_items + MF_ITEMS - 1) / MF_ITEMS), dim3(256), MF_LDS_BYTES, st, n_items, item_first,
-                     item_cnt, P, pinf, hinf, err, H, f);
-  return hipGetLastError();
+  return mf_launch(k_miller_fused, attr, st, n_items, item_first, item_cnt, P, pinf, hinf, err, H, f);
 }
 hipError_t miller_lines_list(hipStream_t st, int n, const int32_t* list, const uint32_t* H, uint32_t* lines) {
   LSG_LAUNCH_ITEMS(k_miller_lines_list, n, st, n, list, H, lines);
diff --git a/lodestar_amd/csrc/lsg_k_reduce.hip b/lodestar_amd/csrc/lsg_k_reduce.hip
--- a/lodestar_amd/csrc/lsg_k_reduce.hip
+++ b/lodestar_amd/csrc/lsg_k_reduce.hip
@@ -324,6 +324,37 @@
   putv(jac_add_proj(Jv, g2v_from_pair(Q)));
   putp(jac_add_proj(J, Q));
 }
+__global__ void LSG_KERNEL_ATTR k_check_mf_lanes(int n, const uint32_t* __restrict__ in, uint32_t* __restrict__ out) {
+  LANE_ITEM(n);
+  (void)lead;
+  auto el2 = [&](int j) {
+    return fp2_t(lane_load<fp_t>(in, (size_t)lsgk::CHECK_LANES_IN * item + 2 * j),
+                 lane_load<fp_t>(in, (size_t)lsgk::CHECK_LANES_IN * item + 2 * j + 1));
+  };
+  int o = 0;
+  auto put2 = [&](const fp2_t& w) {
+    lane_store(out, (size_t)lsgk::CHECK_LANES_OUT * item + (size_t)o, w.c0);
+    lane_store(out, (size_t)lsgk::CHECK_LANES_OUT * item + (size_t)o + 1, w.c1);
+    o += 2;
+  };
+  auto put = [&](const fp2v_t& v) { put2(fp2v_to_pair(v)); };
+  const fp2_t Ap = el2(0), Bp = el2(1), Cp = el2(2);
+  const fp2v_t A = fp2v_from_pair(Ap), B = fp2v_from_pair(Bp), C = fp2v_from_pair(Cp);
+  const fpv_t k = fpv_from_pair(Bp.c0);
+  put(fmul_fp(A, k));
+  put2(fp2_mul_fp(Ap, Bp.c0));
+  put(fmul_xi(A));
+  put2(fp2_mul_xi(Ap));
+  put((fsum(A) + fsum_mul_xi(fsum(B) - C)).carry());
+  put2((fp2s(Ap) + fp2s_mul_xi(fp2s(Bp) - Cp)).carry());
+  const fp6v_t v = fp6_mul_v(fp6_make(A, B, C));
+  put(v.c0);
+  put(v.c1);
+  put(v.c2);
+  put(fone<fp2v_t>());
+  put(fzero<fp2v_t>());
+  lane_store(out + (size_t)lsgk::CHECK_LANES_OUT * lsgl::W_FP * item + (size_t)o * lsgl::W_FP, 0, k);
+}
 #endif
 
 constexpr int LSG_CHECK_CANON_OUT = lsgk::CHECK_CANON_OUT;
@@ -446,7 +477,11 @@
 hipError_t check_g2_lanes(hipStream_t st, int n, const uint32_t* in, uint32_t* out) {
   LSG_LAUNCH_ITEMS(k_check_g2_lanes, n, st, n, in, out);
 }
+hipError_t check_mf_lanes(hipStream_t st, int n, const uint32_t* in, uint32_t* out) {
+  LSG_LAUNCH_ITEMS(k_check_mf_lanes, n, st, n, in, out);
+}
 #else
+hipError_t check_mf_lanes(hipStream_t, int, const uint32_t*, uint32_t*) { return hipErrorNotSupported; }
 hipError_t check_fp2_lanes(hipStream_t, int, const uint32_t*, uint32_t*) { return hipErrorNotSupported; }
 hipError_t check_g2_lanes(hipStream_t, int, const uint32_t*, uint32_t*) { return hipErrorNotSupported; }
 #endif
diff --git a/lodestar_amd/csrc/lsg_launch.h b/lodestar_amd/csrc/lsg_launch.h
--- a/lodestar_amd/csrc/lsg_launch.h
+++ b/lodestar_amd/csrc/lsg_launch.h
@@ -96,7 +96,7 @@
 
 hipError_t miller_fused(hipStream_t st, int n_items, const int32_t* item_first, const int32_t* item_cnt,
                         const uint32_t* P, const uint8_t* pinf, const uint8_t* hinf, const int32_t* err,
-                        const uint32_t* H, uint32_t* f);
+                        const uint32_t* H, uint32_t* f, bool pair_form = false);
 hipError_t miller_lines(hipStream_t st, int n, const uint32_t* H, uint32_t* lines);
 hipError_t miller_lines_list(hipStream_t st, int n, const int32_t* list, const uint32_t* H, uint32_t* lines);
 hipError_t miller_accum_list(hipStream_t st, int n, const int32_t* list, const uint32_t* P, const uint8_t* pinf,
@@ -123,6 +123,7 @@
 constexpr int CHECK_LANES_IN = 12, CHECK_LANES_OUT = 24, CHECK_G2L_IN = 12, CHECK_G2L_OUT = 24;
 hipError_t check_fp2_lanes(hipStream_t st, int n, const uint32_t* in, uint32_t* out);
 hipError_t check_g2_lanes(hipStream_t st, int n, const uint32_t* in, uint32_t* out);
+hipError_t check_mf_lanes(hipStream_t st, int n, const uint32_t* in, uint32_t* out);
 constexpr int CHECK_CANON_OUT = 54, CHECK_ROOTS_OUT = 58;
 hipError_t check_canon(hipStream_t st, int n, const uint32_t* in, uint32_t* out);
 hipError_t check_from_bytes(hipStream_t st, int n, const uint8_t* in48, uint32_t* out);
diff --git a/lodestar_amd/csrc/lsg_pairing.hpp b/lodestar_amd/csrc/lsg_pairing.hpp
--- a/lodestar_amd/csrc/lsg_pairing.hpp
+++ b/lodestar_amd/csrc/lsg_pairing.hpp
@@ -58,7 +58,7 @@
 }
 
 template <int J, class G>
-LSG_INL fp2_t mfc_sqr(const G& V) {
+LSG_INL auto mfc_sqr(const G& V) {
   if constexpr (J == 0) {
     return fp6_kar_s0(V(0), V(1), V(2), V(3)).template carry_mul<2>();
   } else if constexpr (J == 1) {
@@ -66,54 +66,54 @@
   } else if constexpr (J == 2) {
     return fp6_kar_s2(V(0), V(1), V(2), V(5)).template carry_mul<2>();
   } else if constexpr (J == 3) {
-    const fp2_t d = (fp6_kar_s0(V(6), V(7), V(8), V(9)) - fp6_kar_s0(V(0), V(1), V(2), V(3))).carry();
-    const fp2_t t2 = fp6_kar_s2(V(0), V(1), V(2), V(5)).carry();
-    return (fp2s(d) - fp2s_mul_xi(t2)).carry();
+    const auto e = ((fsum(V(9)) - V(7) - V(8)) - (fsum(V(3)) - V(1) - V(2))).carry();
+    const auto g = (fsum(e) - fp6_kar_s2(V(0), V(1), V(2), V(5))).carry();
+    return (fsum(V(6)) - V(0) + fsum_mul_xi(g)).carry();
   } else if constexpr (J == 4) {
-    const fp2_t d = ((fp2s(V(10)) - V(6) - V(7)) - (fp2s(V(4)) - V(0) - V(1))).carry();
-    const fp2_t e = (fp2s(d) + fp2s_mul_xi(fp2s(V(8)) - V(2))).carry();
-    return (fp2s(e) - fp6_kar_s0(V(0), V(1), V(2), V(3))).carry();
+    const auto d = ((fsum(V(10)) - V(6) - V(7)) - (fsum(V(4)) - V(0) - V(1))).carry();
+    const auto e = (fsum(d) + fsum_mul_xi(fsum(V(8)) - V(2))).carry();
+    return (fsum(e) - fp6_kar_s0(V(0), V(1), V(2), V(3))).carry();
   } else {
-    const fp2_t d = ((fp2s(V(11)) - V(6) - V(8)) - (fp2s(V(5)) - V(0) - V(2))).carry();
-    const fp2_t t1 = fp6_kar_s1(V(0), V(1), V(2), V(4)).carry();
-    return (fp2s(d) + V(7) - V(1) - t1).carry();
+    const auto d = ((fsum(V(11)) - V(6) - V(8)) - (fsum(V(5)) - V(0) - V(2))).carry();
+    const auto t1 = fp6_kar_s1(V(0), V(1), V(2), V(4)).carry();
+    return (fsum(d) + V(7) - V(1) - t1).carry();
   }
 }
 template <int J, class G>
-LSG_INL fp2_t mfc_pair(const G& V) {
+LSG_INL auto mfc_pair(const G& V) {
   if constexpr (J == 0) {
-    return (fp2s(V(0)) + fp2s_mul_xi(V(1))).carry();
+    return (fsum(V(0)) + fsum_mul_xi(V(1))).carry();
   } else if constexpr (J == 1) {
-    return fp2_sub2(V(3), V(0), V(2));
+    return fsub2(V(3), V(0), V(2));
   } else if constexpr (J == 2) {
-    return fp2_sub2(V(4), V(0), V(1));
+    return fsub2(V(4), V(0), V(1));
   } else {
-    return fp2_sub2(V(5), V(2), V(1));
+    return fsub2(V(5), V(2), V(1));
   }
 }
 template <int J, class G>
-LSG_INL fp2_t mfc_mul(const G& V) {
+LSG_INL auto mfc_mul(const G& V) {
   if constexpr (J == 0) {
-    const fp2_t g = (fp2s(V(4)) - V(1) - V(2) + V(8)).carry();
-    const fp2_t h = (fp2s(g) - V(6) - V(7)).carry();
-    return (fp2s(V(0)) + fp2s_mul_xi(h)).carry();
+    const auto g = (fsum(V(4)) - V(1) - V(2) + V(8)).carry();
+    const auto h = (fsum(g) - V(6) - V(7)).carry();
+    return (fsum(V(0)) + fsum_mul_xi(h)).carry();
   } else if constexpr (J == 1) {
-    const fp2_t h = (fp2s(V(2)) + V(7) + V(9)).carry();
-    return ((fp2s(V(3)) - V(0) - V(1)) + fp2s_mul_xi(h)).carry();
+    const auto h = (fsum(V(2)) + V(7) + V(9)).carry();
+    return ((fsum(V(3)) - V(0) - V(1)) + fsum_mul_xi(h)).carry();
   } else if constexpr (J == 2) {
-    const fp2_t n0 = (fp2s(V(6)) + fp2s_mul_xi(V(10))).carry();
-    return (fp2s(V(5)) - V(0) - V(2) + V(1) + n0).carry();
+    const auto n0 = (fsum(V(6)) + fsum_mul_xi(V(10))).carry();
+    return (fsum(V(5)) - V(0) - V(2) + V(1) + n0).carry();
   } else if constexpr (J == 3) {
-    const fp2_t g = (fp2s(V(15)) - V(12) - V(13) + V(1) + V(2)).carry();
-    const fp2_t h = (fp2s(g) - V(4) - V(7) - V(9)).carry();
-    return (fp2s(V(11)) - V(0) + fp2s_mul_xi(h)).carry();
+    const auto g = (fsum(V(15)) - V(12) - V(13) + V(1) + V(2)).carry();
+    const auto h = (fsum(g) - V(4) - V(7) - V(9)).carry();
+    return (fsum(V(11)) - V(0) + fsum_mul_xi(h)).carry();
   } else if constexpr (J == 4) {
-    const fp2_t a = ((fp2s(V(14)) - V(11) - V(12)) - (fp2s(V(3)) - V(0) - V(1))).carry();
-    const fp2_t b = fp2_sub2(V(13), V(2), V(10));
-    return (fp2s(a) - V(6) + fp2s_mul_xi(b)).carry();
+    const auto a = ((fsum(V(14)) - V(11) - V(12)) - (fsum(V(3)) - V(0) - V(1))).carry();
+    const auto b = fsub2(V(13), V(2), V(10));
+    return (fsum(a) - V(6) + fsum_mul_xi(b)).carry();
   } else {
-    const fp2_t g = (fp2s(V(11)) + V(13) + V(5) - V(16) - V(12) - V(0)).carry();
-    return (fp2s(V(2)) + V(6) + V(7) - V(1) - V(8) - g).carry();
+    const auto g = (fsum(V(11)) + V(13) + V(5) - V(16) - V(12) - V(0)).carry();
+    return (fsum(V(2)) + V(6) + V(7) - V(1) - V(8) - g).carry();
   }
 }
 
```

Result: faster. 3.801 million (median of 6 runs) (+3.1%).
